# safe-autonomous-systems/fluidgym

Measured on AMD Instinct MI355X. Metric: env-steps/sec (batched) + pressure-Poisson HBM GB/s vs roofline, 1/2/4/8 GPUs, higher is better.
Workload: dtype f32; 1 GPU; ChannelJet2D-v0 (2D channel stand-in for 'cylinder Re=100 256x128'), 64 envs/GPU, 25 PISO steps/env step, random jets, stirred by a body force N(0,2.0) redrawn every env step; global_batch=64, parallelism=env-sharded x1, 1 bcast + 1 all_gather per step (RCCL), lanes_per_gpu=2, workload_modified=True, capped_solves=0, floor_released_solves=0, advection_solver_form=two-brick, velocity_solver=on-chip Jacobi sweeps (policy advection_jacobi; 11972 solves settled by

## Files before the change

### fluidgym_amd/_lib.py

```python
from __future__ import annotations

import ctypes
import os
from ctypes import POINTER, Structure, c_char_p, c_float, c_int, c_int32, c_int64, c_void_p

_HERE = os.path.dirname(os.path.abspath(__file__))
LIB_PATH = os.environ.get("FLUIDGYM_AMD_LIB") or os.path.join(_HERE, "libfluidgym_hip.so")
LIB_F64_PATH = os.environ.get("FLUIDGYM_AMD_LIB_F64") or os.path.join(_HERE, "libfluidgym_hip_f64.so")

FG_MAX_SCALARS = 4
FG_FIELD_SUMMARY_WORK_BYTES = 128
FG_OK = 0
FG_ERR_NOT_CONVERGED = -5
FG_ERR_NOT_FINITE = -6
FG_ERR_FLUX_BALANCE = -7
FG_PERIODIC, FG_FIXED = 0, 1
FG_DIRICHLET, FG_NEUMANN = 0, 1
FG_VELOCITY, FG_PRESSURE, FG_SCALAR, FG_VELOCITY_SOURCE, FG_VISCOSITY_FIELD = 0, 1, 2, 3, 4
FG_BOUND_VELOCITY, FG_BOUND_SCALAR = 8, 16
FG_SOLVER_CG, FG_SOLVER_JACOBI, FG_SOLVER_RBGS, FG_SOLVER_MGCG, FG_SOLVER_FDCG = 0, 1, 2, 3, 4
(FG_BUF_A, FG_BUF_C_OFF, FG_BUF_ADV_RHS, FG_BUF_VEL_RESULT, FG_BUF_H, FG_BUF_DIV, FG_BUF_P_RESULT,
 FG_BUF_SCALAR_RESULT) = range(8)
FG_ERR_UNSUPPORTED = -4
FG_ERR_INVALID_ARG = -1
# ... 79 lines not shown
        ("pressure_use_bicgstab", c_int32),
        ("pressure_warm_start", c_int32),
        ("pressure_project_mean", c_int32),
        ("pressure_stall_accept", c_float),
        ("solver_double_fallback", c_int32),
        ("bicg_precondition_fallback", c_int32),
    ]


class FgMbSimOptions(Structure):
    _fields_ = [
        ("step", FgMbStepOptions),
        ("time_step", c_float),
        ("cfl", c_float),
        ("adaptive", c_int32),
        ("substeps", c_int32),
        ("flux_balance_tol", c_float),
        ("outflow_slot0", c_int32),
        ("outflow_count", c_int32),
        ("outflow_velm", c_float * 3),
        ("outflow_tol", c_float),
        ("max_substeps", c_int32),
        ("outflow_slot0_b", c_int32),
        ("outflow_count_b", c_int32),
    ]


(FG_MB_BUF_A, FG_MB_BUF_C_OFF, FG_MB_BUF_RHS, FG_MB_BUF_H, FG_MB_BUF_DIV, FG_MB_BUF_P_DIAG, FG_MB_BUF_P_OFF,
 FG_MB_BUF_VELOCITY_RESULT) = range(8)
FG_MB_BUF_KRYLOV0 = 8


class FgSimOptions(Structure):
    _fields_ = [
        ("step", FgStepOptions),
        ("time_step", c_float),
        ("cfl", c_float),
        ("adaptive", c_int32),
        ("substeps", c_int32),
        ("flux_balance_tol", c_float),
        ("outflow_mask", c_int32),
        ("outflow_velm", c_float * 3),
        ("outflow_tol", c_float),
        ("max_substeps", c_int32),
    ]


SIGNATURES = {
    "fg_abi_version": (c_int, []),
    "fg_last_error": (c_char_p, []),
    "fg_create": (c_int, [POINTER(FgConfig), POINTER(c_float), POINTER(c_float), POINTER(c_float), POINTER(c_void_p)]),
    "fg_destroy": (c_int, [c_void_p]),
    "fg_bind": (c_int, [c_void_p, c_int, c_void_p]),
    "fg_set_viscosity": (c_int, [c_void_p, c_float]),
    "fg_set_scalar_viscosity": (c_int, [c_void_p, c_int, c_float]),
    "fg_set_viscosity_batch": (c_int, [c_void_p, c_void_p]),
    "fg_set_scalar_viscosity_batch": (c_int, [c_void_p, c_int, c_void_p]),
    "fg_set_fd_preconditioner": (c_int, [c_void_p] + [POINTER(c_float)] * 7),
    "fg_max_velocity": (c_int, [c_void_p, c_void_p, c_void_p]),
    "fg_set_fd_fast_transform": (c_int, [c_void_p, c_int, c_float]),
    "fg_set_return_best": (c_int, [c_void_p, c_int]),
    "fg_set_cg_reset_steps": (c_int, [c_void_p, c_int]),
    "fg_set_advection_start": (c_int, [c_void_p, c_int]),
    "fg_set_wall_stress_forcing": (c_int, [c_void_p, c_int, c_float, c_float]),
    "fg_boundary_flux_balance": (c_int, [c_void_p, c_void_p, c_void_p]),
    "fg_step_diagnostics": (c_int, [c_void_p, POINTER(c_float), c_void_p]),
    "fg_update_advective_boundary": (c_int, [c_void_p, c_int, POINTER(c_float), c_void_p, c_void_p]),
    "fg_balance_boundary_fluxes": (c_int, [c_void_p, c_int, c_float, c_void_p, c_void_p]),
    "fg_setup_advection": (c_int, [c_void_p, c_void_p, c_int, c_int, c_void_p]),
    "fg_solve_advection": (c_int, [c_void_p, c_int, c_int, c_float, c_int, POINTER(FgSolveInfo), c_void_p]),
    "fg_copy_scalar_result_to_blocks": (c_int, [c_void_p, c_int, c_void_p]),
    "fg_setup_pressure_matrix": (c_int, [c_void_p, c_void_p]),
    "fg_setup_pressure_rhs": (c_int, [c_void_p, c_void_p, c_void_p]),
    "fg_solve_pressure": (c_int, [c_void_p, c_int, c_float, c_int, c_int, POINTER(FgSolveInfo), c_void_p]),
    "fg_correct_velocity": (c_int, [c_void_p, c_void_p]),
    "fg_copy_velocity_result_to_blocks": (c_int, [c_void_p, c_void_p]),
    "fg_copy_velocity_result_from_blocks": (c_int, [c_void_p, c_void_p]),
    "fg_piso_step": (c_int, [c_void_p, c_void_p, POINTER(FgStepOptions), POINTER(c_int32), c_void_p]),
    "fg_single_step": (c_int, [c_void_p, POINTER(FgSimOptions), POINTER(c_int32), POINTER(c_float), c_void_p]),
    "fg_multi_step": (c_int, [c_void_p, POINTER(FgSimOptions), c_int32, POINTER(c_void_p), POINTER(c_int32), POINTER(c_float), POINTER(c_int32), c_void_p]),
    "fg_make_divergence_free": (c_int, [c_void_p, c_float, c_int, POINTER(FgSolveInfo), c_void_p]),
    "fg_reset_solver_state": (c_int, [c_void_p, c_void_p]),
    "fg_solver_hints": (c_int, [c_void_p, POINTER(c_int32), c_int32]),
    "fg_env_restore_field": (c_int, [c_void_p, c_int, c_void_p, c_int32, POINTER(FgEnvSel), c_int32, c_int32, c_void_p]),
    "fg_env_reset_solver_state": (c_int, [c_void_p, POINTER(FgEnvSel), c_int32, c_void_p]),
    "fg_mb_env_restore_field": (c_int, [c_void_p, c_int, c_void_p, c_int32, POINTER(FgEnvSel), c_int32, c_int32, c_void_p]),
    "fg_mb_env_reset_solver_state": (c_int, [c_void_p, POINTER(FgEnvSel), c_int32, c_void_p]),
    "fg_set_pressure_refinement": (c_int, [c_void_p, c_int32, c_float, c_float]),
    "fg_get_buffer": (c_int, [c_void_p, c_int, POINTER(c_void_p), POINTER(c_int64)]),
    "fg_read_buffer": (c_int, [c_void_p, c_int, c_void_p, c_void_p]),
    "fg_poisson_apply": (c_int, [c_void_p, c_void_p, c_void_p, c_void_p, c_void_p]),
    "fg_poisson_jacobi": (c_int, [c_void_p, c_void_p, c_void_p, c_void_p, c_int, c_float, c_void_p]),
    "fg_poisson_rbgs": (c_int, [c_void_p, c_void_p, c_void_p, c_void_p, c_int, c_float, c_void_p]),
    "fg_poisson_cg": (c_int, [c_void_p, c_void_p, c_void_p, c_void_p, c_float, c_int, c_int, POINTER(FgSolveInfo),
                              c_void_p]),
    "fg_poisson_fdcg": (c_int, [c_void_p, c_void_p, c_void_p, c_void_p, c_float, c_int, c_int, POINTER(FgSolveInfo),
                                c_void_p]),
    "fg_sparse_apply_ell": (c_int, [c_void_p, c_void_p, c_int32, c_int32, c_void_p, c_int64, c_int32, c_void_p, c_void_p]),
    "fg_sparse_apply_csr": (c_int, [c_void_p, c_void_p, c_void_p, c_int32, c_void_p, c_int64, c_int32, c_void_p, c_void_p]),
    "fg_stream_triad": (c_int, [c_void_p, c_void_p, c_void_p, c_float, c_int64, c_int32, POINTER(c_float), c_void_p]),
    "fg_mb_multilevel_status": (c_int, [c_void_p, POINTER(c_int32)]),
    "fg_mb_multilevel_apply": (c_int, [c_void_p, c_void_p, c_void_p, c_void_p]),
    "fg_mb_debug_ilu_apply": (c_int, [c_void_p, c_void_p, c_void_p, c_void_p]),
    "fg_mb_debug_pressure_cg": (c_int, [c_void_p, c_float, c_int32, c_int32, POINTER(c_int32), POINTER(c_int32), POINTER(ctypes.c_double), c_void_p]),
    "fg_mb_wall_forces": (c_int, [c_void_p, c_void_p, c_void_p, c_void_p, c_int32, c_int32, c_float, c_float, c_void_p, c_void_p]),
    "fg_mb_wall_forces_batch": (c_int, [c_void_p, c_void_p, c_void_p, c_void_p, c_int32, c_int32, c_float, c_float, c_void_p, c_void_p, c_void_p]),
    "fg_mb_debug_bicgstab": (c_int, [c_void_p, c_float, c_int32, c_int32, POINTER(c_int64), POINTER(ctypes.c_double), POINTER(c_float), c_void_p]),
    "fg_dacc_host_sum": (c_int, [POINTER(ctypes.c_double), c_int64, ctypes.c_double, POINTER(ctypes.c_double)]),
    "fg_dacc_device_sum": (c_int, [POINTER(ctypes.c_double), c_int64, ctypes.c_double, c_int32, POINTER(ctypes.c_double), c_void_p]),
    "fg_field_summary": (c_int, [c_void_p, c_int32, c_int32, c_int64, c_int32, c_void_p, c_void_p, c_void_p, ctypes.c_double, ctypes.c_double,
                                 c_int32, c_void_p, c_void_p]),
    "fg_plane_moments": (c_int, [POINTER(c_void_p), POINTER(c_int64), c_int32, c_int32, c_int32, c_int32, c_int32, c_int32, c_void_p, c_void_p,
                                 c_void_p, c_void_p, c_void_p]),
    "fg_plane_budgets": (c_int, [POINTER(c_void_p), POINTER(c_int64), c_int32, c_int32, c_int32, c_int32, c_int32, c_void_p, c_void_p, c_void_p,
                                 c_int32, c_int32, c_void_p, c_void_p, c_void_p, c_void_p, c_void_p]),
    "fg_plane_timecorr": (c_int, [POINTER(c_void_p), POINTER(c_int64), c_int32, c_int32, c_int32, c_int32, c_int32, c_int32, c_int32,
                                  POINTER(c_int32), c_void_p, c_void_p, c_void_p, c_void_p]),
    "fg_mb_cell_moments": (c_int, [c_void_p, c_void_p, c_int32, c_int32, c_int64, POINTER(c_int64), c_int32, c_int64, c_void_p, c_void_p,
                                   c_void_p]),
    "fg_mb_cell_moments_widths": (c_int, [c_void_p, c_void_p, c_int64, POINTER(c_int64), c_int32, c_void_p, c_void_p, POINTER(c_int32)]),
    "fg_plane_spectra": (c_int, [POINTER(c_void_p), POINTER(c_int64), c_int32, c_int32, c_int32, c_int32, c_int32, POINTER(c_int32), c_int32,
                                 c_void_p, c_void_p, c_void_p]),
    "fg_coherence_litmus": (c_int, [c_int32, c_int32, c_int32, c_int32, POINTER(c_int64), POINTER(ctypes.c_double), c_void_p]),
    "fg_profile_enable": (c_int, [c_void_p, c_int]),
    "fg_profile_kinds": (c_int, []),
    "fg_profile_kind_name": (ctypes.c_char_p, [c_int]),
    "fg_profile_read": (c_int, [c_void_p, c_int, POINTER(ctypes.c_double), POINTER(c_int64), POINTER(ctypes.c_double),
                                POINTER(ctypes.c_double), POINTER(ctypes.c_double), POINTER(ctypes.c_double),
                                POINTER(c_int64), POINTER(c_int64), POINTER(ctypes.c_double), POINTER(c_int64)]),
    "fg_coords_to_transforms": (c_int, [c_void_p, c_void_p, c_int, c_int, c_int, c_int, c_void_p]),
    "fg_resampler_create": (c_int, [c_int, POINTER(ctypes.c_int32), POINTER(ctypes.c_int32), POINTER(ctypes.c_int32),
                                    POINTER(ctypes.c_float), c_int, c_int, POINTER(c_void_p)]),
    "fg_resampler_destroy": (c_int, [c_void_p]),
    "fg_resample": (c_int, [c_void_p, c_void_p, c_int, c_int, c_void_p, c_int, c_void_p]),
    "fg_envglue_jet_schedule": (c_int, [c_void_p, c_void_p, c_void_p, c_void_p, c_int32, c_int32, c_int32, c_void_p, c_void_p, c_void_p]),
    "fg_envglue_channel_observe": (c_int, [c_void_p, c_void_p, c_void_p, c_int32, c_int32, c_int32, c_int32, c_float, c_float, c_void_p,
                                           c_void_p, c_void_p, c_void_p, c_void_p, c_void_p]),
    "fg_envglue_channel_observe_batch": (c_int, [c_void_p, c_void_p, c_void_p, c_int32, c_int32, c_int32, c_int32, c_void_p, c_float, c_void_p,
                                                 c_void_p, c_void_p, c_void_p, c_void_p, c_void_p]),
    "fg_mb_create": (c_int, [c_int32, c_int32, c_int32, POINTER(c_void_p)]),
    "fg_mb_destroy": (c_int, [c_void_p]),
    "fg_config_dump": (c_int, [c_void_p, ctypes.c_char_p, c_int]),
    "fg_mb_config_dump": (c_int, [c_void_p, ctypes.c_char_p, c_int]),
    "fg_mb_add_block": (c_int, [c_void_p, POINTER(c_float), c_int32, c_int32, c_int32, POINTER(c_int32)]),
    "fg_mb_connect": (c_int, [c_void_p, c_int32, c_int32, c_int32, c_int32, c_int32, c_int32]),
    "fg_mb_make_periodic": (c_int, [c_void_p, c_int32, c_int32]),
    "fg_mb_set_reference_quirks": (c_int, [c_void_p, c_int32, c_int32]),
    "fg_mb_set_nonortho_flags": (c_int, [c_void_p, c_int32]),
    "fg_mb_finalize": (c_int, [c_void_p]),
    "fg_mb_sizes": (c_int, [c_void_p, POINTER(c_int32), POINTER(c_int32)]),
    "fg_mb_block_info": (c_int, [c_void_p, c_int32, POINTER(c_int32), POINTER(c_int32)]),
    "fg_mb_get_host_table": (c_int, [c_void_p, c_int32, c_void_p, POINTER(c_int64)]),
    "fg_mb_get_neighbors": (c_int, [c_void_p, POINTER(c_int32)]),
    "fg_mb_bind": (c_int, [c_void_p, c_void_p, c_void_p, c_void_p, c_void_p]),
    "fg_mb_set_viscosity": (c_int, [c_void_p, c_float]),
    "fg_mb_set_viscosity_batch": (c_int, [c_void_p, c_void_p]),
    "fg_mb_piso_step": (c_int, [c_void_p, c_void_p, POINTER(FgMbStepOptions), POINTER(c_int32), c_void_p]),
    "fg_mb_max_velocity": (c_int, [c_void_p, POINTER(c_float), c_void_p]),
    "fg_mb_set_residual_projection": (c_int, [c_void_p, POINTER(c_float)]),
    "fg_mb_set_stall_limit": (c_int, [c_void_p, c_int32]),
    "fg_mb_set_advection_start": (c_int, [c_void_p, c_int]),
    "fg_mb_set_advection_jacobi": (c_int, [c_void_p, c_int]),
    "fg_mb_advection_jacobi_counts": (c_int, [c_void_p, POINTER(c_int64)]),
    "fg_mb_set_multilevel": (c_int, [c_void_p, c_int32, c_int32, POINTER(c_int32), POINTER(c_int32), POINTER(c_int32), POINTER(c_float),
                                     POINTER(c_float), c_float, c_int32]),
    "fg_mb_env_status": (c_int, [c_void_p, POINTER(c_int32)]),
# ... 133 lines not shown
```

### fluidgym_amd/csrc/fg_api.hip

```cpp
#include <stdio.h>
#include <string.h>

#include <cmath>
#include <string>
#include <vector>

#include <stdlib.h>

#include "fg_internal.h"

static thread_local std::string g_last_error;
void fg_set_error(const std::string& msg) { g_last_error = msg; }

extern "C" int fg_abi_version(void) { return FG_ABI_VERSION; }
extern "C" const char* fg_last_error(void) { return g_last_error.c_str(); }

static FgBounds make_bounds(const fg_state* s, int channel) {
    FgBounds b;
    for (int f = 0; f < 6; ++f) {
        b.vel[f] = s->bvel[f];
        b.scal[f] = s->bscal[f];
        b.scalar_bc[f] = s->cfg.scalar_bc[f][channel < 0 ? 0 : channel];
    }
    return b;
}

static int check_bound(const fg_state* s, bool need_scalar) {
    FG_REQUIRE(s->velocity && s->pressure, FG_ERR_NOT_BOUND, "velocity/pressure not bound (fg_bind)");
    for (int f = 0; f < 2 * s->grid.dims; ++f) {
        if (!s->grid.fixed[f]) continue;
        FG_REQUIRE(s->bvel[f], FG_ERR_NOT_BOUND, "boundary velocity of a FIXED face not bound");
        if (need_scalar) FG_REQUIRE(s->bscal[f], FG_ERR_NOT_BOUND, "boundary scalar of a FIXED face not bound");
    }
    if (need_scalar) FG_REQUIRE(s->scalar, FG_ERR_NOT_BOUND, "passive scalar not bound");
    return FG_OK;
}

extern "C" int fg_create(const fg_config* cfg, const fg_real* hx, const fg_real* hy, const fg_real* hz, fg_handle* out) {
    FG_REQUIRE(cfg && out && hx && hy, FG_ERR_INVALID_ARG, "fg_create: null argument");
    FG_REQUIRE(cfg->dims == 2 || cfg->dims == 3, FG_ERR_INVALID_ARG, "dims must be 2 or 3");
    FG_REQUIRE(cfg->dims == 2 || hz, FG_ERR_INVALID_ARG, "hz required in 3-D");
    FG_REQUIRE(cfg->nx >= 3 && cfg->ny >= 3 && (cfg->dims == 2 ? cfg->nz == 1 : cfg->nz >= 3), FG_ERR_INVALID_ARG,
               "block needs >= 3 cells per axis (nz = 1 in 2-D)");
    FG_REQUIRE(cfg->batch >= 1, FG_ERR_INVALID_ARG, "batch must be >= 1");
    FG_REQUIRE(cfg->n_scalars >= 0 && cfg->n_scalars <= FG_MAX_SCALARS, FG_ERR_INVALID_ARG, "bad n_scalars");
    for (int a = 0; a < cfg->dims; ++a)
        FG_REQUIRE(cfg->face_type[2 * a] == cfg->face_type[2 * a + 1], FG_ERR_INVALID_ARG,
                   "a FIXED face needs a FIXED partner (CloseBoundary closes both, domain_structs.cpp:1981-2002)");
    FG_REQUIRE((long long)cfg->nx * cfg->ny * cfg->nz * cfg->batch * 6 < (1LL << 31), FG_ERR_UNSUPPORTED,
               "index space exceeds int32 (reference index_t is int32 as well)");
    FG_HIP_CHECK(hipSetDevice(cfg->device));

    fg_state* s = new fg_state();
    memset(s, 0, sizeof(*s));
    s->cfg = *cfg;
    FgGrid& g = s->grid;
    g.dims = cfg->dims; g.nx = cfg->nx; g.ny = cfg->ny; g.nz = cfg->nz;
    g.n = cfg->nx * cfg->ny * cfg->nz; g.B = cfg->batch;
    for (int f = 0; f < 6; ++f) g.fixed[f] = (f < 2 * cfg->dims) ? (cfg->face_type[f] == FG_FIXED) : 0;
    s->vec = (!FG_F64 && cfg->nx % 4 == 0) ? 4 : 1;
    s->viscosity = 0.f;

    const fg_real* hsrc[3] = {hx, hy, hz};
    const int hn[3] = {cfg->nx, cfg->ny, cfg->nz};
    for (int a = 0; a < 3; ++a) {
        std::vector<fg_real> h(hn[a], 1.f), rh(hn[a], 1.f);
        if (a < cfg->dims)
            for (int i = 0; i < hn[a]; ++i) {
                if (!(hsrc[a][i] > 0.f)) { delete s; fg_set_error("cell widths must be positive"); return FG_ERR_INVALID_ARG; }
                h[i] = hsrc[a][i]; rh[i] = 1.f / hsrc[a][i];
            }
        FG_HIP_CHECK(hipMalloc(&s->d_h[a], sizeof(fg_real) * hn[a]));
        FG_HIP_CHECK(hipMalloc(&s->d_rh[a], sizeof(fg_real) * hn[a]));
        FG_HIP_CHECK(hipMemcpy(s->d_h[a], h.data(), sizeof(fg_real) * hn[a], hipMemcpyHostToDevice));
        FG_HIP_CHECK(hipMemcpy(s->d_rh[a], rh.data(), sizeof(fg_real) * hn[a], hipMemcpyHostToDevice));
        g.h[a] = s->d_h[a]; g.rh[a] = s->d_rh[a];
    }
    const size_t BN = (size_t)g.B * g.n, d = g.dims;
    auto alloc = [&](fg_real** p, size_t count) -> hipError_t {
        hipError_t e = hipMalloc(p, sizeof(fg_real) * count);
        if (e == hipSuccess) e = hipMemset(*p, 0, sizeof(fg_real) * count);
        return e;
    };
    FG_HIP_CHECK(alloc(&s->A, BN));
    FG_HIP_CHECK(alloc(&s->rA, BN));
    FG_HIP_CHECK(alloc(&s->Coff, BN * 2 * d));
    FG_HIP_CHECK(alloc(&s->adv_rhs, BN * d));
    FG_HIP_CHECK(alloc(&s->vel_result, BN * d));
    FG_HIP_CHECK(alloc(&s->hvec, BN * d));
    FG_HIP_CHECK(alloc(&s->div, BN));
    FG_HIP_CHECK(alloc(&s->p_result, BN));
    FG_HIP_CHECK(alloc(&s->scal_result, BN));
    for (int i = 0; i < 8; ++i) FG_HIP_CHECK(alloc(&s->w[i], BN * d));
    const size_t nsys = (size_t)g.B * d;
    FG_HIP_CHECK(hipMalloc(&s->acc, sizeof(FgDacc) * nsys * FG_ACC_DOUBLES));
    FG_HIP_CHECK(hipMemset(s->acc, 0, sizeof(FgDacc) * nsys * FG_ACC_DOUBLES));
    FG_HIP_CHECK(hipMalloc(&s->flags, sizeof(int32_t) * nsys));
    FG_HIP_CHECK(hipMalloc(&s->info_dev, sizeof(fg_solve_info) * nsys));
    FG_HIP_CHECK(hipHostMalloc(&s->info_pinned, sizeof(fg_solve_info) * nsys));
    FG_HIP_CHECK(hipHostMalloc(&s->flags_pinned, sizeof(int32_t) * nsys));
    FG_HIP_CHECK(alloc(&s->scratch_B, (size_t)g.B * (4 + 2 * d)));
    FG_HIP_CHECK(hipMalloc(&s->d_bvel_ptrs, sizeof(fg_real*) * 6));
    FG_HIP_CHECK(hipMemset(s->d_bvel_ptrs, 0, sizeof(fg_real*) * 6));
    FG_HIP_CHECK(hipHostMalloc(&s->diag_pinned, sizeof(fg_real) * 2 * g.B));
    FG_HIP_CHECK(hipHostMalloc(&s->dt_pinned, sizeof(fg_real) * g.B));
    FG_HIP_CHECK(alloc(&s->dt_dev, g.B));
    FG_HIP_CHECK(hipMalloc(&s->env_sel_dev, sizeof(fg_env_sel) * g.B));
    s->t_rem_dev = nullptr;
#if !FG_F64
    FG_HIP_CHECK(hipMalloc(&s->t_rem_dev, sizeof(double) * g.B));
    FG_HIP_CHECK(hipMemset(s->t_rem_dev, 0, sizeof(double) * g.B));
#endif
    if (int rc = fg_poll_create(&s->poll, (int)(nsys > 2 * (size_t)g.B ? nsys : 2 * (size_t)g.B))) return rc;
    for (int k = 0; k < 4; ++k) { s->pred_bicg[k] = 2; s->pred_cg[k] = 1; }
    s->wall_forcing_axis = -1;
    s->ref64_inner = 1e-4f;
    s->cg_wgs_per_slot = 256;
    { const char* ev = getenv("FG_BICG3"); s->bicg3_force = ev ? atoi(ev) : -1; }
    { const char* ev = getenv("FG_BICG3_BXL"); s->bicg3_bxl = ev ? atoi(ev) : 0; }
    { const char* ev = getenv("FG_BICG_SUB"); s->bicg_sub = ev ? atoi(ev) : -1; }
    { const char* ev = getenv("FG_REDUCE_WGS"); s->reduce_wgs = ev ? atoi(ev) : 0; }
    { const char* ev = getenv("FG_BICG3_MIX"); s->bicg3_mix = ev ? atoi(ev) : 3; }
    { const char* ev = getenv("FG_BICG_FUSED"); s->bicg_fused = ev ? atoi(ev) : 1; }
    s->tridiag_cb = 64;
    s->helm_cb_pref = 32;
    { const char* ev = getenv("FG_HELM_ROWFORM"); s->helm_rowform_off = (ev && atoi(ev) == 0) ? 1 : 0; }
    { const char* ev = getenv("FG_FD_FACFUSE"); s->fd_facfuse = ev ? atoi(ev) : 1; }
    { const char* ev = getenv("FG_DEV_DT"); s->dev_dt = ev ? atoi(ev) : 1; }
    { const char* ev = getenv("FG_ADV_LINESWEEP"); s->adv_linesweep = ev ? atoi(ev) : 0; }
    { const char* ev = getenv("FG_FD_ROWMEAN"); s->fd_rowmean = ev ? atoi(ev) : 1; }
    s->fd_row_epoch = -1; s->rA_epoch = 0; s->fd_row_part_epoch = -1;
    { const char* ev = getenv("FG_CG_FUSED"); s->cg_fused = ev ? atoi(ev) : 1; }
    { const char* ev = getenv("FG_BICG_PFUSED"); s->bicg_pfused = ev ? atoi(ev) : 1; }
    { const char* ev = getenv("FG_ADV_JACOBI"); s->adv_jacobi = ev ? atoi(ev) : 0; s->adv_jacobi_env = ev ? 1 : 0; }
    for (int k = 0; k < 4; ++k) s->jac_hist[k] = FgJacHist{0, 0, 0};
    s->jac_solves = s->jac_fallbacks = 0;
    FG_HIP_CHECK(hipHostMalloc(&s->jac_prev, sizeof(float) * 4 * nsys));
    s->jac_rA_epoch = -1;
    FG_HIP_CHECK(hipMalloc(&s->fcg_alpha, sizeof(double) * 2 * (size_t)g.B));
    FG_HIP_CHECK(hipMemset(s->fcg_alpha, 0, sizeof(double) * 2 * (size_t)g.B));
    FG_HIP_CHECK(hipMalloc(&s->fcg_xsum, sizeof(FgDacc) * 2 * (size_t)g.B));
    FG_HIP_CHECK(hipMemset(s->fcg_xsum, 0, sizeof(FgDacc) * 2 * (size_t)g.B));
    FG_HIP_CHECK(hipMalloc(&s->fcg_lazy, sizeof(int32_t) * (size_t)g.B));
    FG_HIP_CHECK(hipMemset(s->fcg_lazy, 0, sizeof(int32_t) * (size_t)g.B));
    { const char* e = getenv("FG_FCG_FIRST"); s->fcg_first = (e && atoi(e) == 0) ? 0 : 1; }
    { const char* e = getenv("FG_JAC_SPEC"); s->jac_spec = (e && atoi(e) == 0) ? 0 : 1; }
    { const char* e = getenv("FG_FCG_SPEC"); s->fcg_spec = (e && atoi(e) == 0) ? 0 : 1; }
    { const char* e = getenv("FG_JAC_PREFACTOR"); s->jac_prefactor = (e && atoi(e) == 0) ? 0 : 1; }
    { const char* e = getenv("FG_JAC_WARM"); s->jac_warm = e ? (atoi(e) != 0 ? 1 : 0) : -1; }
    s->cg_return_best = 1;
    s->cg_reset_steps = 100;
    s->adv_from_result = 1;
    FG_HIP_CHECK(hipMalloc(&s->cg_acc, sizeof(FgDacc) * (size_t)g.B * 8 * 64));
    FG_HIP_CHECK(hipMemset(s->cg_acc, 0, sizeof(FgDacc) * (size_t)g.B * 8 * 64));
    FG_HIP_CHECK(hipMalloc(&s->cg_best.best_crit, sizeof(fg_real) * g.B));
    FG_HIP_CHECK(hipMalloc(&s->cg_best.saved_crit, sizeof(fg_real) * g.B));
    FG_HIP_CHECK(hipMalloc(&s->cg_best.save_at, sizeof(int32_t) * g.B));
    FG_HIP_CHECK(alloc(&s->cg_best.best_x, BN));
    *out = s;
    return FG_OK;
}

extern "C" int fg_destroy(fg_handle s) {
    if (!s) return FG_OK;
    for (int a = 0; a < 3; ++a) { (void)hipFree(s->d_h[a]); (void)hipFree(s->d_rh[a]); }
    fg_real* owned[] = {s->A, s->rA, s->Coff, s->adv_rhs, s->vel_result, s->hvec, s->div, s->p_result, s->scal_result,
                      s->scratch_B};
    for (fg_real* p : owned) (void)hipFree(p);
    for (int i = 0; i < 8; ++i) (void)hipFree(s->w[i]);
    (void)hipFree(s->acc); (void)hipFree(s->flags); (void)hipFree(s->info_dev);
    (void)hipHostFree(s->info_pinned); (void)hipHostFree(s->flags_pinned);
    fg_prof_destroy(s);
    fg_poll_destroy(&s->poll);
    (void)hipFree(s->d_bvel_ptrs); (void)hipHostFree(s->diag_pinned); (void)hipHostFree(s->dt_pinned); (void)hipFree(s->dt_dev); (void)hipFree(s->t_rem_dev); (void)hipFree(s->env_sel_dev);
    float* fd[] = {s->fd_Qx, s->fd_QxT, s->fd_Qz, s->fd_QzT, s->fd_lower, s->fd_inv, s->fd_cp};
    for (float* p : fd) if (p) (void)hipFree(p);
    if (s->fd_dct_tw) { (void)hipFree(s->fd_dct_tw); (void)hipFree(s->fd_dct_rot); }
    (void)hipFree(s->cg_acc); (void)hipFree(s->fcg_alpha); (void)hipFree(s->fcg_xsum); (void)hipFree(s->fcg_lazy);
    if (s->jac_prev) (void)hipHostFree(s->jac_prev);
    (void)hipFree(s->fd_row_part); (void)hipFree(s->fd_lam_x); (void)hipFree(s->fd_row_inv); (void)hipFree(s->fd_row_cp); (void)hipFree(s->fd_row_lower);
    (void)hipFree(s->line_inv); (void)hipFree(s->line_cp); (void)hipFree(s->ilu_d);
    (void)hipFree(s->r64_buf); (void)hipFree(s->r64_acc); (void)hipFree(s->ref64_x); (void)hipFree(s->force_uniform);
    (void)hipFree(s->fd_lam); (void)hipFree(s->helm_diag); (void)hipFree(s->helm_lower); (void)hipFree(s->helm_upper); (void)hipFree(s->helm_tmp); (void)hipFree(s->helm_lower_row); (void)hipFree(s->helm_lower_row2); (void)hipFree(s->line_inv2); (void)hipFree(s->line_cp2);
    (void)hipFree(s->cg_best.best_crit); (void)hipFree(s->cg_best.saved_crit); (void)hipFree(s->cg_best.save_at); (void)hipFree(s->cg_best.best_x);
    delete s;
    return FG_OK;
}

static int sync_bvel_ptrs(fg_state* s);
extern "C" int fg_bind(fg_handle s, int field, fg_real* ptr) {
    FG_REQUIRE(s, FG_ERR_INVALID_ARG, "null handle");
    if (field == FG_VELOCITY) s->velocity = ptr;
    else if (field == FG_PRESSURE) s->pressure = ptr;
    else if (field == FG_SCALAR) s->scalar = ptr;
    else if (field == FG_VELOCITY_SOURCE) s->velocity_source = ptr;
    else if (field == FG_VISCOSITY_FIELD) s->visc_field = ptr;
    else if (field >= FG_BOUND_VELOCITY && field < FG_BOUND_VELOCITY + 6) {
        s->bvel[field - FG_BOUND_VELOCITY] = ptr;
        return sync_bvel_ptrs(s);
    }
    else if (field >= FG_BOUND_SCALAR && field < FG_BOUND_SCALAR + 6) s->bscal[field - FG_BOUND_SCALAR] = ptr;
    else FG_REQUIRE(false, FG_ERR_INVALID_ARG, "fg_bind: unknown field id");
    return FG_OK;
}

extern "C" int fg_set_viscosity(fg_handle s, fg_real v) {
    FG_REQUIRE(s, FG_ERR_INVALID_ARG, "null handle");
    s->viscosity = v;
    return FG_OK;
}
extern "C" int fg_set_scalar_viscosity(fg_handle s, int ch, fg_real v) {
    FG_REQUIRE(s && ch >= 0 && ch < FG_MAX_SCALARS, FG_ERR_INVALID_ARG, "bad channel");
    s->scalar_viscosity[ch] = v;
    s->scalar_viscosity_set = true;
    return FG_OK;
}
extern "C" int fg_set_viscosity_batch(fg_handle s, const fg_real* nu_B) {
    FG_REQUIRE(s, FG_ERR_INVALID_ARG, "null handle");
    s->viscosity_B = nu_B;
    s->helm_pre_mask = 0;
    return FG_OK;
}
extern "C" int fg_set_scalar_viscosity_batch(fg_handle s, int ch, const fg_real* k_B) {
    FG_REQUIRE(s && ch >= 0 && ch < FG_MAX_SCALARS, FG_ERR_INVALID_ARG, "bad channel");
    s->scalar_viscosity_B[ch] = k_B;
    s->helm_pre_mask = 0;
    return FG_OK;
}

extern "C" int fg_set_fd_preconditioner(fg_handle s, const float* Qx, const float* QxT, const float* Qz, const float* QzT,
// ... 267 lines not shown
    if (for_scalar) {
        a.scal = s->scalar + (size_t)channel * s->grid.n;
        a.scal_env_stride = (long)s->cfg.n_scalars * s->grid.n;
        a.nu = fg_nu(s, 1, channel);
    } else {
        a.source = s->velocity_source;
        if (s->wall_forcing_axis >= 0)
            if (int rc = fg_launch_wall_forcing(s, (hipStream_t)stream)) return rc;
        a.force = s->wall_forcing_axis >= 0 ? s->force_uniform : nullptr;
        a.visc = s->visc_field;
        a.nu = fg_nu(s);
        a.rA = s->rA;
        s->adv_last_dt = dt_B;
        s->rA_epoch++;
        s->jac_rA_epoch = s->rA_epoch;
#if !FG_F64
        if (fg_fd_rowmean_ok(s) && s->vec == 4 && (s->grid.nx & 63) == 0) {
            if (!s->fd_row_part) FG_HIP_CHECK(hipMalloc(&s->fd_row_part, sizeof(float) * (size_t)s->grid.B * s->grid.ny * (s->grid.nx / 64)));
            a.row_part = s->fd_row_part;
            s->fd_row_part_epoch = s->rA_epoch;
        }
#endif
        if (buoy_axis >= 0) {
            a.buoy_T = s->scalar; a.buoy_stride = (long)s->cfg.n_scalars * s->grid.n; a.buoy_axis = buoy_axis; a.buoy_factor = buoy_factor;
            a.source_w = s->velocity_source;
        }
    }
    return fg_launch_adv_build(s, make_bounds(s, channel), a, (hipStream_t)stream);
}

static int advection_solve(fg_state* s, FgBicgArgs a, fg_solve_info* info, hipStream_t st, int for_scalar = 0, int channel = 0, bool* spec_ran = nullptr);

extern "C" int fg_solve_advection(fg_handle s, int for_scalar, int channel, fg_real tol, int max_iterations,
                                  fg_solve_info* info_host, void* stream) {
    FG_REQUIRE(s, FG_ERR_INVALID_ARG, "null handle");
    FgBicgArgs a;
    a.diag = s->A; a.off = s->Coff; a.rhs = s->adv_rhs;
    a.dt = s->cur_dt;
    a.tol = tol; a.max_iterations = max_iterations;
    if (for_scalar) { a.x = s->scal_result; a.nc = 1; a.use_x0 = 0; a.kind = 0; }
    else { a.x = s->vel_result; a.nc = s->grid.dims; a.use_x0 = s->adv_from_result; }
    return advection_solve(s, a, info_host, (hipStream_t)stream, for_scalar, channel);
}

extern "C" int fg_copy_scalar_result_to_blocks(fg_handle s, int channel, void* stream) {
    FG_REQUIRE(s && s->scalar, FG_ERR_NOT_BOUND, "scalar not bound");
    const int n = s->grid.n;
    if (s->cfg.n_scalars == 1) return fg_launch_copy_active(s, s->cur_dt, s->scal_result, s->scalar, 1, (hipStream_t)stream);
    FG_HIP_CHECK(hipMemcpy2DAsync(s->scalar + (size_t)channel * n, sizeof(fg_real) * n * s->cfg.n_scalars, s->scal_result,
                                  sizeof(fg_real) * n, sizeof(fg_real) * n, s->grid.B, hipMemcpyDeviceToDevice,
                                  (hipStream_t)stream));
    return FG_OK;
}

extern "C" int fg_setup_pressure_matrix(fg_handle s, void* stream) {
    FG_REQUIRE(s, FG_ERR_INVALID_ARG, "null handle");
    s->rA_epoch++;
    return fg_launch_pressure_setup(s, s->cur_dt, (hipStream_t)stream);
}

extern "C" int fg_setup_pressure_rhs(fg_handle s, const fg_real* dt_B, void* stream) {
    FG_REQUIRE(s && dt_B, FG_ERR_INVALID_ARG, "null argument");
    if (int rc = check_bound(s, false)) return rc;
    hipStream_t st = (hipStream_t)stream;
    if (int rc = fg_launch_h(s, dt_B, s->vel_result, st)) return rc;
    return fg_launch_div(s, make_bounds(s, 0), dt_B, s->hvec, s->div, st);
}

struct SpecH { fg_state* s; const fg_real* dt; const fg_step_options* opt; hipStream_t st; };
static int spec_h(void* p) {
    const SpecH* c = static_cast<const SpecH*>(p);
    fg_state* s = c->s;
    if (int rc = fg_launch_h(s, c->dt, s->vel_result, c->st)) return rc;
    return fg_launch_div(s, make_bounds(s, 0), c->dt, s->hvec, s->div, c->st, !c->opt->pressure_warm_start,
                         c->opt->pressure_method == FG_SOLVER_FDCG && s->fd_Qx != nullptr);
}

static int launch_corrector(fg_state* s, const fg_real* dt, const FgCgOutcome& o, bool last, hipStream_t st) {
    const bool mean_folded = last && o.mean_ready;
    FG_REQUIRE(!o.lazy_z || !last || mean_folded, FG_ERR_UNSUPPORTED, "fg_piso_step: an unmaterialised pressure without its folded mean");
    if (last && !mean_folded)
        if (int rc = fg_launch_mean_sub(s, dt, s->p_result, s->pressure, st)) return rc;
    const FgMeanRef mean = {s->fcg_xsum, s->info_dev, s->pressure, o.marks_valid ? s->fcg_lazy : nullptr, s->fcg_alpha};
    const FgLazyRef lazy = {s->fcg_lazy, s->fcg_alpha, last ? s->p_result : nullptr};
    const fg_real* p = o.lazy_z ? o.lazy_z : ((last && !mean_folded) ? s->pressure : s->p_result);
    return fg_launch_correct(s, dt, s->rA, s->hvec, p, s->vel_result, st, last ? s->velocity : nullptr, mean_folded ? &mean : nullptr, o.lazy_z ? &lazy : nullptr);
}

struct SpecCorrect { fg_state* s; const fg_real* dt; bool last; hipStream_t st; };
static int spec_correct(void* p, const FgCgOutcome& o) {
    const SpecCorrect* c = static_cast<const SpecCorrect*>(p);
    return launch_corrector(c->s, c->dt, o, c->last, c->st);
}

static int solve_pressure(fg_state* s, const fg_real* dt, int method, fg_real tol, int max_iterations, int use_previous,
                          fg_solve_info* info_host, hipStream_t st, bool finalize = true, int kind = 2, FgCgOutcome* out = nullptr,
                          FgCgSpec spec = FgCgSpec{}) {
    int rc = FG_OK;
    FgCgOutcome own;
    if (!out) out = &own;
    if (method == FG_SOLVER_CG || method == FG_SOLVER_FDCG) {
        FgCgArgs a;
        a.rA = s->rA; a.b = s->div; a.x = s->p_result;
        a.r = s->w[0]; a.p = s->w[1]; a.Ap = s->w[2];
        a.dt = dt; a.tol = tol; a.max_iterations = max_iterations; a.use_x0 = use_previous;
        a.reset_steps = s->cg_reset_steps;
        a.precond = (method == FG_SOLVER_FDCG);
        a.kind = kind;
        a.check_every = a.precond ? 2 : 16;
        a.lazy_ok = finalize ? 0 : 1;
        a.spec = spec;
#if !FG_F64
        if (s->ref64_outer > 0) a.lazy_ok = 0;
#endif
        rc = fg_cg_solve(s, a, info_host, st, out);
#if !FG_F64
        if (s->ref64_outer > 0 && (rc == FG_OK || rc == FG_ERR_NOT_CONVERGED)) rc = fg_refine64_pressure(s, a, info_host, st, out);
        if (s->double_fallback && (rc == FG_ERR_NOT_FINITE || (s->ladder_force & 2))) {
            std::vector<fg_solve_info> tmp;
            fg_solve_info* info = info_host;
            if (!info) { tmp.assign(s->info_pinned, s->info_pinned + s->grid.B); info = tmp.data(); }
            s->rung_count[2] += 1;
            rc = fg_rung64_cg(s, a, info, (s->ladder_force & 2) != 0, st, out);
        }
#endif
    } else {
        fg_set_error("fg_solve_pressure: only FG_SOLVER_CG drives the PISO step (Jacobi/RBGS are smoothers)");
        return FG_ERR_UNSUPPORTED;
    }
    if (rc != FG_OK && rc != FG_ERR_NOT_CONVERGED) return rc;
    if (finalize)
        if (int rc2 = fg_launch_mean_sub(s, dt, s->p_result, s->pressure, st)) return rc2;
    return rc;
}

extern "C" int fg_solve_pressure(fg_handle s, int method, fg_real tol, int max_iterations, int use_previous,
                                 fg_solve_info* info_host, void* stream) {
    FG_REQUIRE(s, FG_ERR_INVALID_ARG, "null handle");
    if (int rc = check_bound(s, false)) return rc;
    return solve_pressure(s, s->cur_dt, method, tol, max_iterations, use_previous, info_host, (hipStream_t)stream);
}

extern "C" int fg_set_pressure_refinement(fg_handle s, int32_t max_corrections, fg_real target_tol, fg_real inner_relative_tol) {
    FG_REQUIRE(s, FG_ERR_INVALID_ARG, "null handle");
    FG_REQUIRE(!FG_F64 || max_corrections <= 0, FG_ERR_UNSUPPORTED, "fg_set_pressure_refinement: the fp64 build solves in fp64 already");
    FG_REQUIRE(max_corrections <= 0 || (target_tol > 0 && inner_relative_tol > 0 && inner_relative_tol < 1), FG_ERR_INVALID_ARG,
               "fg_set_pressure_refinement: tolerances must be positive, the relative one below 1");
    s->ref64_outer = max_corrections > 0 ? max_corrections : 0;
    s->ref64_tol = (float)target_tol; s->ref64_inner = (float)inner_relative_tol;
    return FG_OK;
}

extern "C" int fg_correct_velocity(fg_handle s, void* stream) {
    FG_REQUIRE(s, FG_ERR_INVALID_ARG, "null handle");
    if (int rc = check_bound(s, false)) return rc;
    return fg_launch_correct(s, s->cur_dt, s->rA, s->hvec, s->pressure, s->vel_result, (hipStream_t)stream);
}

extern "C" int fg_copy_velocity_result_to_blocks(fg_handle s, void* stream) {
    FG_REQUIRE(s && s->velocity, FG_ERR_NOT_BOUND, "velocity not bound");
    return fg_launch_copy_active(s, s->cur_dt, s->vel_result, s->velocity, s->grid.dims, (hipStream_t)stream);
}
extern "C" int fg_copy_velocity_result_from_blocks(fg_handle s, void* stream) {
    FG_REQUIRE(s && s->velocity, FG_ERR_NOT_BOUND, "velocity not bound");
    return fg_launch_copy_active(s, nullptr, s->velocity, s->vel_result, s->grid.dims, (hipStream_t)stream);
}

static int max_iters(const fg_solve_info* info, int n) {
    int m = -1;
    for (int i = 0; i < n; ++i) m = info[i].used_iterations > m ? info[i].used_iterations : m;
    return m;
}

static int advection_solve(fg_state* s, FgBicgArgs a, fg_solve_info* info, hipStream_t st, int for_scalar, int channel, bool* spec_ran) {
    a.precond = (s->adv_precond == 1) ? 1 : (s->adv_precond == 3 ? 2 : (s->adv_precond == 4 ? 3 : 0));
    if (a.precond == 2 && !for_scalar && s->visc_field) a.precond = 0;
    if (a.precond == 2) {
        a.nu = fg_nu(s, for_scalar, channel);
        a.wall_lo = for_scalar ? (s->cfg.scalar_bc[2][channel] == FG_DIRICHLET) : 1;
        a.wall_hi = for_scalar ? (s->cfg.scalar_bc[3][channel] == FG_DIRICHLET) : 1;
    }
    const int nsys = s->grid.B * a.nc;
    std::vector<fg_solve_info> info_own;
    if (!info) { info_own.resize(nsys); info = info_own.data(); }
    int rc = fg_bicgstab_solve(s, a, info, st, spec_ran);
    bool failed = (rc == FG_ERR_NOT_CONVERGED || rc == FG_ERR_NOT_FINITE) || (s->ladder_force & 1);
#if !FG_F64
    if (failed && s->double_fallback && rc != FG_ERR_HIP) {
        s->rung_count[0] += 1;
        rc = fg_rung64_bicgstab(s, a, info, (s->ladder_force & 1) != 0, st);
        if (rc != FG_OK && rc != FG_ERR_NOT_CONVERGED && rc != FG_ERR_NOT_FINITE) return rc;
        failed = (rc != FG_OK) || (s->ladder_force & 4);
    }
#endif
    if (failed && (s->adv_precond == 2 || s->adv_precond == 5)) {
        s->line_retries += 1;
        s->rung_count[1] += 1;
        a.precond = s->adv_precond == 5 ? 3 : 1; a.use_x0 = 0;
        rc = fg_bicgstab_solve(s, a, info, st);
    }
    (void)nsys;
    return rc;
}

extern "C" int fg_piso_step(fg_handle s, const fg_real* dt_B, const fg_step_options* opt, int32_t* stats_host,
                            void* stream) {
    FG_REQUIRE(s && dt_B && opt, FG_ERR_INVALID_ARG, "null argument");
    const bool scalar = opt->advect_scalar && s->cfg.n_scalars > 0;
    if (int rc = check_bound(s, scalar)) return rc;
    FG_REQUIRE(opt->buoyancy_axis < s->grid.dims, FG_ERR_INVALID_ARG, "bad buoyancy axis");
    FG_REQUIRE(opt->buoyancy_axis < 0 || (s->velocity_source && s->scalar), FG_ERR_NOT_BOUND,
               "buoyancy needs velocity source and scalar bound");
    hipStream_t st = (hipStream_t)stream;
    const int B = s->grid.B, d = s->grid.dims;
    std::vector<fg_solve_info> info((size_t)B * d);
    int32_t stats[4] = {-1, -1, -1, -1};
    struct DropHelmRecord { fg_state* s; ~DropHelmRecord() { s->helm_pre_mask = 0; } } drop_helm_record{s};
    int status = FG_OK;
    auto soft = [&](int rc) {
        if (rc == FG_ERR_NOT_CONVERGED) { status = rc; return FG_OK; }
        return rc;
    };
#if !FG_F64
    const bool sweeps_first = s->adv_linesweep && s->grid.dims == 2 && s->jac_hist[0].skip == 0 && s->jac_hist[1].skip == 0;
    if (scalar && s->cfg.n_scalars == 1 && s->adv_precond == 3 && s->fd_lam && !s->visc_field && !sweeps_first) {
        const FgNu nu2[2] = {fg_nu(s, 1, 0), fg_nu(s)};
        const int wlo[2] = {s->cfg.scalar_bc[2][0] == FG_DIRICHLET, 1}, whi[2] = {s->cfg.scalar_bc[3][0] == FG_DIRICHLET, 1};
        if (int rc = fg_helm_factor_pair(s, dt_B, nu2, wlo, whi, st)) return rc;
    }
#endif
    if (scalar) {
        FgRange range_scalar("scalar_advection");
        for (int ch = 0; ch < s->cfg.n_scalars; ++ch) {
            if (int rc = fg_setup_advection(s, dt_B, 1, ch, stream)) return rc;
            FgBicgArgs a;
            a.diag = s->A; a.off = s->Coff; a.rhs = s->adv_rhs; a.x = s->scal_result; a.nc = 1;
            a.dt = dt_B; a.tol = opt->advection_tol; a.max_iterations = opt->max_iterations; a.use_x0 = 0; a.kind = 0;
            if (int rc = soft(advection_solve(s, a, info.data(), st, 1, ch))) return rc;
            const int m = max_iters(info.data(), B);
            stats[0] = m > stats[0] ? m : stats[0];
            s->ctr.add(0, info.data(), B);
            const int n = s->grid.n;
            if (s->cfg.n_scalars == 1) {
                if (int rc = fg_launch_copy_active(s, dt_B, s->scal_result, s->scalar, 1, st)) return rc;
            } else {
                (void)n;
                fg_set_error("multi-channel scalar copy with inactive envs not implemented");
                return FG_ERR_UNSUPPORTED;
            }
        }
    }
    fg_range_push("velocity_assembly_and_solve");
    struct PopOnce { bool armed = true; void fire() { if (armed) { fg_range_pop(); armed = false; } } ~PopOnce() { fire(); } } range_velocity;
    if (int rc = setup_advection(s, dt_B, 0, 0, stream, opt->buoyancy_axis, opt->buoyancy_factor)) return rc;
    bool h_div_ran = false;
    {
        FgBicgArgs a;
        a.diag = s->A; a.off = s->Coff; a.rhs = s->adv_rhs; a.x = s->vel_result; a.nc = d;
        a.dt = dt_B; a.tol = opt->advection_tol; a.max_iterations = opt->max_iterations; a.use_x0 = s->adv_from_result;
        SpecH spec_h_ctx = {s, dt_B, opt, st};
        if (opt->corrector_steps > 0) a.spec = FgSpecHook{spec_h, &spec_h_ctx};
        if (int rc = soft(advection_solve(s, a, info.data(), st, 0, 0, &h_div_ran))) return rc;
        stats[1] = max_iters(info.data(), B * d);
        s->ctr.add(1, info.data(), B * d);
    }
    range_velocity.fire();
    for (int c = 0; c < opt->corrector_steps; ++c) {
        FgRange range_corr(c == 0 ? "pressure_corrector_0" : "pressure_corrector_1+");
        const bool last = (c + 1 == opt->corrector_steps);
        if (!(c == 0 && h_div_ran)) {
            if (int rc = fg_launch_h(s, dt_B, s->vel_result, st)) return rc;
            if (int rc = fg_launch_div(s, make_bounds(s, 0), dt_B, s->hvec, s->div, st, !opt->pressure_warm_start,
                                       opt->pressure_method == FG_SOLVER_FDCG && s->fd_Qx != nullptr))
                return rc;
        }
        SpecCorrect spec_ctx = {s, dt_B, last, st};
        FgCgOutcome outcome;
        if (int rc = soft(solve_pressure(s, dt_B, opt->pressure_method, opt->pressure_tol, opt->max_iterations, opt->pressure_warm_start ? 1 : 0,
                                         info.data(), st, false, c == 0 ? 0 : 1, &outcome, FgCgSpec{spec_correct, &spec_ctx})))
            return rc;
        if (c < 2) { stats[2 + c] = max_iters(info.data(), B); s->ctr.add(2 + c, info.data(), B); }
        if (!outcome.spec_done)
            if (int rc = launch_corrector(s, dt_B, outcome, last, st)) return rc;
    }
    if (opt->corrector_steps <= 0)
        if (int rc = fg_launch_copy_active(s, dt_B, s->vel_result, s->velocity, d, st)) return rc;
    if (stats_host) memcpy(stats_host, stats, sizeof(stats));
    s->ctr.piso_steps += 1;
    return status;
}

extern "C" int fg_config_dump(fg_handle s, char* buf, int n) {
    FG_REQUIRE(s && buf && n > 0, FG_ERR_INVALID_ARG, "fg_config_dump: bad argument");
    char tmp[3072];
    const int len = snprintf(tmp, sizeof(tmp),
        "{\"build\": \"%s\", \"FG_CG_FUSED\": %d, \"FG_BICG_PFUSED\": %d, \"FG_BICG_FUSED\": %d, \"FG_BICG_SUB\": %d, \"FG_BICG3\": %d, "
        "\"FG_BICG3_BXL\": %d, \"FG_BICG3_MIX\": %d, \"FG_REDUCE_WGS\": %d, \"FG_CG_WGS_PER_SLOT\": %d, \"FG_TRIDIAG_CB\": %d, \"FG_HELM_CB\": %d, "
        "\"FG_HELM_ROWFORM\": %d, \"FG_FD_ROWMEAN\": %d, \"FG_POLL_SPIN\": %d, \"FG_PROF_PERIOD\": %d, \"fast_transform_x\": %d, \"fd_preconditioner\": %d, "
        "\"helmholtz\": %d, \"advection_preconditioner\": %d, \"advection_from_result\": %d, \"return_best\": %d, \"cg_reset_steps\": %d, "
        "\"double_fallback\": %d, \"wall_forcing_axis\": %d, \"FG_ADV_JACOBI\": %d, \"FG_FCG_FIRST\": %d, \"FG_JAC_WARM\": %d, \"first_iterate_polls\": %ld, \"unstored_pressure_solves\": %ld, \"FG_JAC_SPEC\": %d, \"FG_FCG_SPEC\": %d, \"jacobi_speculation_misses\": %ld, \"jacobi_floor_released\": %ld, \"pressure_refinement_corrections\": %ld}",
        FG_F64 ? "f64" : "f32", s->cg_fused, s->bicg_pfused, s->bicg_fused, s->bicg_sub, s->bicg3_force, s->bicg3_bxl, s->bicg3_mix, s->reduce_wgs,
        s->cg_wgs_per_slot, s->tridiag_cb, s->helm_cb_pref, s->helm_rowform_off ? 0 : 1, s->fd_rowmean, s->poll.spin, s->prof.period, s->fd_dct_x, s->fd_Qx ? 1 : 0,
        s->fd_lam ? 1 : 0, s->adv_precond, s->adv_from_result, s->cg_return_best, s->cg_reset_steps, s->double_fallback, s->wall_forcing_axis, s->adv_jacobi, s->fcg_first, s->jac_warm,
        s->fcg_first_polls, s->fcg_unstored, s->jac_spec, s->fcg_spec, s->jac_spec_missed, s->jac_floor_released, s->ref64_corrections);
    if (len >= n) return len + 1;
    memcpy(buf, tmp, (size_t)len + 1);
    return FG_OK;
}

extern "C" int fg_solver_unconverged(fg_handle s, int64_t* out4) {
    FG_REQUIRE(s != nullptr && out4 != nullptr, FG_ERR_INVALID_ARG, "fg_solver_unconverged: bad argument");
    for (int k = 0; k < 4; ++k) out4[k] = s->ctr.unconv[k];
    return FG_OK;
}

extern "C" int fg_solver_counters(fg_handle s, int64_t* out13, int32_t reset) {
    FG_REQUIRE(s != nullptr, FG_ERR_INVALID_ARG, "fg_solver_counters: null handle");
    if (out13) s->ctr.write(out13);
    if (reset) s->ctr.reset();
    return FG_OK;
}

extern "C" int fg_single_step(fg_handle s, const fg_sim_options* o, int32_t* out, fg_real* flux_host, void* stream);
extern "C" int fg_multi_step(fg_handle s, const fg_sim_options* o, int32_t n, const fg_real* const* bvel_schedule, int32_t* out_6n,
                             fg_real* flux_host, int32_t* steps_done, void* stream) {
    FG_REQUIRE(s && o && out_6n && n >= 0, FG_ERR_INVALID_ARG, "fg_multi_step: bad argument");
    if (steps_done) *steps_done = 0;
    for (int k = 0; k < n; ++k) {
        if (bvel_schedule)
            for (int f = 0; f < 2 * s->grid.dims; ++f)
                if (const fg_real* p = bvel_schedule[(size_t)k * 6 + f])
                    if (int rc = fg_bind(s, FG_BOUND_VELOCITY + f, const_cast<fg_real*>(p))) return rc;
        if (int rc = fg_single_step(s, o, out_6n + 6 * (size_t)k, flux_host, stream)) return rc;
        if (steps_done) *steps_done = k + 1;
        if (out_6n[6 * (size_t)k + 5] == 0 && !s->cg_return_best) break;
    }
    return FG_OK;
}

static inline bool is_close_zero(double a) { return std::fabs(a) <= 1e-8; }

extern "C" int fg_single_step(fg_handle s, const fg_sim_options* o, int32_t* out, fg_real* flux_host, void* stream) {
    fg_htrace("single_step_in");
    FgRange range_sim("fg_single_step");
    FG_REQUIRE(s && o && out, FG_ERR_INVALID_ARG, "null argument");
    if (int rc = check_bound(s, o->step.advect_scalar && s->cfg.n_scalars > 0)) return rc;
    hipStream_t st = (hipStream_t)stream;
    const int B = s->grid.B;
    const FgBounds bnd = make_bounds(s, 0);
    std::vector<double> t_rem(B, (double)o->time_step);
    int32_t stats[4] = {-1, -1, -1, -1};
    int substeps = 0, all_ok = 1;
    bool first = true;
    int fixed_left = o->adaptive ? 0 : (o->substeps > 0 ? o->substeps : 1);
    for (;;) {
        bool any = false;
        if (o->adaptive) {
            for (int b = 0; b < B; ++b) any = any || (t_rem[b] > 0 && !is_close_zero(t_rem[b]));
        } else {
            any = fixed_left > 0;
        }
        if (!any) break;
        auto advance = [&](int b, fg_real max_vel) -> fg_real {
            fg_real ts = 0.f;
            if (!o->adaptive) {
                ts = o->time_step;
            } else if (t_rem[b] > 0 && !is_close_zero(t_rem[b])) {
                const double mv = (double)max_vel;
                const double max_ts = is_close_zero(mv) ? t_rem[b] : (double)o->cfl / mv;
                double tsd;
                if (max_ts >= t_rem[b]) tsd = t_rem[b];
                else tsd = t_rem[b] / (double)(long long)std::ceil(t_rem[b] / max_ts);
                t_rem[b] -= tsd;
                ts = (fg_real)tsd;
            }
            return ts;
        };
        auto flux_guard = [&]() -> int {
            fg_real worst = 0.f;
            for (int b = 0; b < B; ++b) {
                if (flux_host) flux_host[b] = s->diag_pinned[b];
                const fg_real a = std::fabs(s->diag_pinned[b]);
                worst = (a > worst || a != a) ? a : worst;
            }
            if (!(worst <= o->flux_balance_tol)) {
                fg_set_error("Domain boundary fluxes not balanced, cannot proceed with simulation step.");
                return FG_ERR_FLUX_BALANCE;
// ... 11 lines not shown
                const FgDtRule rule = deferred ? FgDtRule{s->t_rem_dev, s->dt_dev, (float)o->cfl, (double)o->time_step, first ? 1 : 0}
                                               : FgDtRule{nullptr, nullptr, 0.f, 0.0, 0};
                if (int rc = fg_launch_max_velocity(s, bnd, s->scratch_B + B, st, s->diag_pinned + B, po.seq ? FgPollOut{po.seq + B, po.value, po.gran} : po,
                                                    first ? s->scratch_B : nullptr, first ? s->diag_pinned : nullptr, rule))
                    return rc;
            }
            fg_htrace("maxvel_launched");
            if (!deferred) {
                if (o->adaptive && po.gran) {
                    if (int rc = fg_poll_wait_words(&s->poll, po, 12 * B, first ? 2 * B : B, st)) return rc;
                    for (int b = 0; b < B; ++b) {
                        s->diag_pinned[B + b] = fg_poll_word_float(&s->poll, 12 * B + b);
                        if (first) s->diag_pinned[b] = fg_poll_word_float(&s->poll, 13 * B + b);
                    }
                } else if (int rc = fg_poll_wait(&s->poll, po, o->adaptive ? B : 0, o->adaptive ? 1 : B, st)) return rc;
                fg_htrace("maxvel_poll_done");
                if (first) if (int rc = flux_guard()) return rc;
            }
        }
        if (!deferred)
            for (int b = 0; b < B; ++b) s->dt_pinned[b] = advance(b, o->adaptive ? s->diag_pinned[B + b] : (fg_real)0);
        const bool folded = o->outflow_mask && fg_outflow_folds(s, o->outflow_mask);
        const bool dt_by_value = folded && B <= 64 && !deferred;
        if (!dt_by_value && !deferred) FG_HIP_CHECK(hipMemcpyAsync(s->dt_dev, s->dt_pinned, sizeof(fg_real) * B, hipMemcpyHostToDevice, st));
        if (o->outflow_mask) {
            for (int f = 0; f < 2 * s->grid.dims; ++f)
                if ((o->outflow_mask >> f) & 1) FG_REQUIRE(s->grid.fixed[f], FG_ERR_INVALID_ARG, "outflow face is not FIXED");
            if (!folded)
                for (int f = 0; f < 2 * s->grid.dims; ++f)
                    if ((o->outflow_mask >> f) & 1)
                        if (int rc = fg_launch_outflow(s, f, o->outflow_velm[f >> 1], s->dt_dev, st)) return rc;
            fg_real velm3[3] = {o->outflow_velm[0], o->outflow_velm[1], o->outflow_velm[2]};
            if (int rc = fg_launch_balance(s, bnd, o->outflow_mask, (fg_real)0.01 * o->outflow_tol, s->dt_dev, st, folded ? o->outflow_mask : 0, velm3,
                                           dt_by_value ? s->dt_pinned : nullptr))
                return rc;
        }
        int rc = fg_piso_step(s, s->dt_dev, &o->step, stats, stream);
        if (rc == FG_ERR_NOT_CONVERGED) all_ok = 0;
        else if (rc != FG_OK) return rc;
        if (deferred) {
            if (int rc2 = fg_poll_wait_words(&s->poll, po_cfl, 12 * B, first ? 2 * B : B, st)) return rc2;
            for (int b = 0; b < B; ++b) {
                s->diag_pinned[B + b] = fg_poll_word_float(&s->poll, 12 * B + b);
                if (first) s->diag_pinned[b] = fg_poll_word_float(&s->poll, 13 * B + b);
            }
            if (first) if (int rc2 = flux_guard()) return rc2;
            for (int b = 0; b < B; ++b) s->dt_pinned[b] = advance(b, s->diag_pinned[B + b]);
        }
        ++substeps;
        first = false;
        if (!o->adaptive) --fixed_left;
        if (substeps >= (o->max_substeps > 0 ? o->max_substeps : 100000)) break;
    }
    fg_htrace("single_step_out");
    for (int i = 0; i < 4; ++i) out[i] = stats[i];
    out[4] = substeps;
    out[5] = all_ok;
    return FG_OK;
}

extern "C" int fg_make_divergence_free(fg_handle s, fg_real tol, int max_iterations, fg_solve_info* info_host,
                                       void* stream) {
    FG_REQUIRE(s, FG_ERR_INVALID_ARG, "null handle");
    if (int rc = check_bound(s, false)) return rc;
    s->cur_dt = nullptr;
    hipStream_t st = (hipStream_t)stream;
    const size_t BN = (size_t)s->grid.B * s->grid.n;
    std::vector<fg_real> ones(BN, 1.f);
    FG_HIP_CHECK(hipMemcpyAsync(s->rA, ones.data(), sizeof(fg_real) * BN, hipMemcpyHostToDevice, st));
    s->rA_epoch++;
    FG_HIP_CHECK(hipStreamSynchronize(st));
    if (int rc = fg_launch_copy_active(s, nullptr, s->velocity, s->hvec, s->grid.dims, st)) return rc;
    if (int rc = fg_launch_div(s, make_bounds(s, 0), nullptr, s->hvec, s->div, st)) return rc;
    int rc = solve_pressure(s, nullptr, FG_SOLVER_CG, tol, max_iterations, 0, info_host, st);
    if (rc != FG_OK && rc != FG_ERR_NOT_CONVERGED) return rc;
    if (int rc2 = fg_launch_correct(s, nullptr, s->rA, s->hvec, s->pressure, s->vel_result, st)) return rc2;
    if (int rc2 = fg_launch_copy_active(s, nullptr, s->vel_result, s->velocity, s->grid.dims, st)) return rc2;
    return rc;
}

extern "C" int fg_reset_solver_state(fg_handle s, void* stream) {
    FG_REQUIRE(s && s->velocity, FG_ERR_NOT_BOUND, "velocity not bound");
    for (int k = 0; k < 4; ++k) s->jac_hist[k] = FgJacHist{0, 0, 0};
    FG_HIP_CHECK(hipMemsetAsync(s->p_result, 0, sizeof(fg_real) * (size_t)s->grid.B * s->grid.n, (hipStream_t)stream));
    return fg_launch_copy_active(s, nullptr, s->velocity, s->vel_result, s->grid.dims, (hipStream_t)stream);
}

extern "C" int fg_solver_hints(fg_handle s, int32_t* hints12, int32_t set) {
    FG_REQUIRE(s != nullptr && hints12 != nullptr, FG_ERR_INVALID_ARG, "fg_solver_hints: bad argument");
    for (int k = 0; k < 4; ++k) {
        FgJacHist& H = s->jac_hist[k];
        if (set) { H.sweeps = hints12[3 * k]; H.skip = hints12[3 * k + 1]; H.fails = hints12[3 * k + 2]; }
        else { hints12[3 * k] = H.sweeps; hints12[3 * k + 1] = H.skip; hints12[3 * k + 2] = H.fails; }
    }
    return FG_OK;
}

extern "C" int fg_get_buffer(fg_handle s, int which, fg_real** out_ptr, int64_t* out_count) {
    FG_REQUIRE(s && out_ptr && out_count, FG_ERR_INVALID_ARG, "null argument");
    const int64_t BN = (int64_t)s->grid.B * s->grid.n, d = s->grid.dims;
    switch (which) {
        case FG_BUF_A: *out_ptr = s->A; *out_count = BN; break;
        case FG_BUF_C_OFF: *out_ptr = s->Coff; *out_count = BN * 2 * d; break;
        case FG_BUF_ADV_RHS: *out_ptr = s->adv_rhs; *out_count = BN * d; break;
        case FG_BUF_VEL_RESULT: *out_ptr = s->vel_result; *out_count = BN * d; break;
        case FG_BUF_H: *out_ptr = s->hvec; *out_count = BN * d; break;
        case FG_BUF_DIV: *out_ptr = s->div; *out_count = BN; break;
        case FG_BUF_P_RESULT: *out_ptr = s->p_result; *out_count = BN; break;
        case FG_BUF_SCALAR_RESULT: *out_ptr = s->scal_result; *out_count = BN; break;
        default:
            if (which >= 100 && which < 108) { *out_ptr = s->w[which - 100]; *out_count = BN * d; break; }
            FG_REQUIRE(false, FG_ERR_INVALID_ARG, "unknown buffer id");
    }
    return FG_OK;
}

extern "C" int fg_read_buffer(fg_handle s, int which, fg_real* dst, void* stream) {
    fg_real* src = nullptr;
    int64_t count = 0;
    if (int rc = fg_get_buffer(s, which, &src, &count)) return rc;
    FG_REQUIRE(dst, FG_ERR_INVALID_ARG, "null destination");
    FG_HIP_CHECK(hipMemcpyAsync(dst, src, sizeof(fg_real) * count, hipMemcpyDeviceToDevice, (hipStream_t)stream));
    return FG_OK;
}

extern "C" int fg_poisson_apply(fg_handle s, const fg_real* rA, const fg_real* x, fg_real* y, void* stream) {
    FG_REQUIRE(s && rA && x && y, FG_ERR_INVALID_ARG, "null argument");
    return fg_poisson_apply_launch(s, rA, x, y, (hipStream_t)stream);
}

extern "C" int fg_poisson_jacobi(fg_handle s, const fg_real* rA, const fg_real* b, fg_real* x, int n_sweeps, fg_real omega,
                                 void* stream) {
    FG_REQUIRE(s && rA && b && x && n_sweeps >= 0, FG_ERR_INVALID_ARG, "bad argument");
    hipStream_t st = (hipStream_t)stream;
    fg_real* buf[2] = {x, s->w[5]};
    for (int i = 0; i < n_sweeps; ++i)
        if (int rc = fg_poisson_jacobi_launch(s, rA, b, buf[i & 1], buf[(i + 1) & 1], omega, st)) return rc;
    if (n_sweeps & 1)
        FG_HIP_CHECK(hipMemcpyAsync(x, s->w[5], sizeof(fg_real) * (size_t)s->grid.B * s->grid.n, hipMemcpyDeviceToDevice, st));
    return FG_OK;
}

extern "C" int fg_poisson_rbgs(fg_handle s, const fg_real* rA, const fg_real* b, fg_real* x, int n_sweeps, fg_real omega,
                               void* stream) {
    FG_REQUIRE(s && rA && b && x && n_sweeps >= 0, FG_ERR_INVALID_ARG, "bad argument");
    hipStream_t st = (hipStream_t)stream;
    for (int i = 0; i < n_sweeps; ++i) {
        if (int rc = fg_poisson_rbgs_launch(s, rA, b, x, omega, 0, st)) return rc;
        if (int rc = fg_poisson_rbgs_launch(s, rA, b, x, omega, 1, st)) return rc;
    }
    return FG_OK;
}

extern "C" int fg_poisson_cg(fg_handle s, const fg_real* rA, const fg_real* b, fg_real* x, fg_real tol, int max_iterations,
                             int use_x0, fg_solve_info* info_host, void* stream) {
    FG_REQUIRE(s && rA && b && x, FG_ERR_INVALID_ARG, "null argument");
    FgCgArgs a;
    a.rA = rA; a.b = b; a.x = x;
    a.r = s->w[0]; a.p = s->w[1]; a.Ap = s->w[2];
    a.dt = nullptr; a.tol = tol; a.max_iterations = max_iterations; a.use_x0 = use_x0;
    a.reset_steps = 100;
    a.precond = 0;
    a.check_every = (tol > 0.f) ? 16 : (1 << 30);
    return fg_cg_solve(s, a, info_host, (hipStream_t)stream);
}

// ... 24 lines not shown
```

### fluidgym_amd/csrc/fg_fftcg.h

```cpp
#pragma once
#include "fg_internal.h"
#include "fg_cg.h"

constexpr int FCG_DELTA = 3, FCG_GAMMA = 5;

struct FcgVectors {
    fg_real* z; fg_real* w;
    fg_real* p; fg_real* s;
    fg_real* x; fg_real* r; fg_real* t1;
};

struct FcgUpdArgs {
    const float* z; const float* w; float* p; float* s; float* x; float* r; float* t1;
    const float2* tw; const float2* rot; float fs0, fs;
    const int32_t* flags; FgDacc* acc; double* alpha; FgDacc* xsum; FgBest best;
    int ns, rows, it, first; long env_stride;
    const float* r0; int x_zero;
    const int32_t* lazy;
};
struct FcgInvArgs {
    const float* u; const float* r; const float* rA; float* z; float* w;
    const float2* tw; const float2* rot; float is0, is;
    const int32_t* flags; FgDacc* acc; int ns, rows, it; long env_stride;
    const float* hy; const float* rhy; const float* hx; const float* rhx; int fixed_x;
    FgDacc* xsum; int extras;
};

struct FcgDivArgs {
    const float* h; float* div; float* r; float* x; float* t1;
    const float* bvel[4];
    const float2* tw; const float2* rot; float fs0, fs;
    const float* dt; FgDacc* acc; int ns, rows; long n;
    const float* hx; const float* hy; int fixed_x;
};

#if !FG_F64
int fg_fcg_div_fwd(fg_state* s, const FgBounds& bnd, const fg_real* dt, const fg_real* hvec, fg_real* div, int ns, hipStream_t st);
bool fg_fcg_ok(const fg_state* s);
int fg_fcg_update_fwd(fg_state* s, const FcgVectors& v, int it, int first, int ns, hipStream_t st, bool marks_valid, const fg_real* r0 = nullptr);
int fg_fcg_inv_apply(fg_state* s, const FcgVectors& v, const fg_real* rA, int it, int ns, hipStream_t st, int extras = 0);
int fg_fcg_check0(fg_state* s, fg_real tol, int ns, hipStream_t st, FgPollOut poll, bool* marks_valid);
#endif
```

### fluidgym_amd/csrc/fg_fftcg.hip

```cpp
#include "fg_internal.h"
#include "fg_cg.h"
#include "fg_fftrow.h"
#include "fg_fftcg.h"

#if !FG_F64
namespace {

using fgfft::Map;

template <int N, bool PERIODIC>
__global__ __launch_bounds__(256) void k_fcg_update_fwd(FcgUpdArgs a) {
    constexpr int EPL = N / 64;
    __shared__ __attribute__((aligned(16))) float2 buf[2][4][N];
    __shared__ __attribute__((aligned(16))) float2 twl[N];
    __shared__ float red[8];
    const int b = blockIdx.y;
    const int lane = threadIdx.x & 63, wave = threadIdx.x >> 6;
    if (a.flags[b] != 0) {
        if (a.lazy && a.lazy[b] == 1) {
            const float alpha = (float)a.alpha[b * 2];
            const int row0 = 2 * (blockIdx.x * 4 + wave);
#pragma unroll
            for (int half = 0; half < 2; ++half) {
                const int row = row0 + half;
                if (row >= a.rows) continue;
                const size_t o = (size_t)b * a.env_stride + (size_t)row * N;
                float zv[EPL], xv[EPL];
                fgfft::load_row<N>(a.z + o, lane, zv);
                if (a.x_zero) {
#pragma unroll
                    for (int e = 0; e < EPL; ++e) xv[e] = 0.f;
                } else {
                    fgfft::load_row<N>(a.x + o, lane, xv);
                }
#pragma unroll
                for (int e = 0; e < EPL; ++e) xv[e] += alpha * zv[e];
                fgfft::store_row<N>(a.x + o, lane, xv);
            }
        } else if (a.x_zero && (a.flags[b] == 1 || a.flags[b] == 2)) {
            float z0[EPL];
#pragma unroll
            for (int e = 0; e < EPL; ++e) z0[e] = 0.f;
            const int r0 = 2 * (blockIdx.x * 4 + wave);
            if (r0 < a.rows) fgfft::store_row<N>(a.x + (size_t)b * a.env_stride + (size_t)r0 * N, lane, z0);
            if (r0 + 1 < a.rows) fgfft::store_row<N>(a.x + (size_t)b * a.env_stride + (size_t)(r0 + 1) * N, lane, z0);
        }
        return;
    }
    for (int k = threadIdx.x; k < N; k += 256) twl[k] = a.tw[k];
    const int it = a.it;
    const double g_new = fg_acc_total(fg_acc_ptr(a.acc, b, FCG_GAMMA + it % 3), a.ns);
    const double d_new = fg_acc_total(fg_acc_ptr(a.acc, b, FCG_DELTA + (it & 1)), a.ns);
    double beta = 0.0, denom = d_new;
    if (!a.first) {
        const double g_old = fg_acc_total(fg_acc_ptr(a.acc, b, FCG_GAMMA + (it + 2) % 3), a.ns);
        const double al_old = a.alpha[b * 2 + ((it + 1) & 1)];
        beta = g_new / g_old;
        denom = d_new - beta * g_new / al_old;
    }
    const double alpha_d = g_new / denom;
    const float alpha = (float)alpha_d, betaf = (float)beta;
    const bool save = a.best.save_at[b] == it;
    if (blockIdx.x == 0 && threadIdx.x < 64) {
        fg_acc_zero(fg_acc_ptr(a.acc, b, FCG_GAMMA + (it + 1) % 3), a.ns);
        fg_acc_zero(fg_acc_ptr(a.acc, b, FCG_DELTA + ((it + 1) & 1)), a.ns);
        if (threadIdx.x == 0) {
            a.alpha[b * 2 + (it & 1)] = alpha_d;
            acc_st(a.xsum + (b * 2 + ((it + 1) & 1)), 0.0);
        }
    }
    const int row0 = 2 * (blockIdx.x * 4 + wave), row1 = row0 + 1;
    const bool live0 = row0 < a.rows, live1 = row1 < a.rows;
    const size_t o0 = (size_t)b * a.env_stride + (size_t)(live0 ? row0 : 0) * N;
    const size_t o1 = (size_t)b * a.env_stride + (size_t)(live1 ? row1 : 0) * N;
    float pa[EPL], pb[EPL], sa[EPL], sb[EPL], xa[EPL], xb[EPL], ra[EPL], rb[EPL];
    {
        float za[EPL], zb[EPL], wa[EPL], wb[EPL];
        fgfft::load_row<N>(a.z + o0, lane, za); fgfft::load_row<N>(a.z + o1, lane, zb);
        fgfft::load_row<N>(a.w + o0, lane, wa); fgfft::load_row<N>(a.w + o1, lane, wb);
        if (!a.first) {
            fgfft::load_row<N>(a.p + o0, lane, pa); fgfft::load_row<N>(a.p + o1, lane, pb);
            fgfft::load_row<N>(a.s + o0, lane, sa); fgfft::load_row<N>(a.s + o1, lane, sb);
        }
        if (a.x_zero) {
#pragma unroll
            for (int e = 0; e < EPL; ++e) { xa[e] = 0.f; xb[e] = 0.f; }
        } else {
            fgfft::load_row<N>(a.x + o0, lane, xa); fgfft::load_row<N>(a.x + o1, lane, xb);
        }
        const float* rsrc = a.r0 ? a.r0 : a.r;
        fgfft::load_row<N>(rsrc + o0, lane, ra); fgfft::load_row<N>(rsrc + o1, lane, rb);
        if (save) {
            if (live0) fgfft::store_row<N>(a.best.best_x + o0, lane, xa);
            if (live1) fgfft::store_row<N>(a.best.best_x + o1, lane, xb);
        }
        if (a.first) {
#pragma unroll
            for (int e = 0; e < EPL; ++e) { pa[e] = za[e]; pb[e] = zb[e]; sa[e] = wa[e]; sb[e] = wb[e]; }
        } else {
#pragma unroll
            for (int e = 0; e < EPL; ++e) {
                pa[e] = za[e] + betaf * pa[e]; pb[e] = zb[e] + betaf * pb[e];
                sa[e] = wa[e] + betaf * sa[e]; sb[e] = wb[e] + betaf * sb[e];
            }
        }
    }
    float part[2] = {0.f, 0.f};
#pragma unroll
    for (int e = 0; e < EPL; ++e) {
        xa[e] += alpha * pa[e]; ra[e] -= alpha * sa[e];
        xb[e] += alpha * pb[e]; rb[e] -= alpha * sb[e];
        if (!live0) { xa[e] = 0.f; ra[e] = 0.f; }
        if (!live1) { xb[e] = 0.f; rb[e] = 0.f; }
        part[0] += ra[e] * ra[e] + rb[e] * rb[e];
        part[1] += xa[e] + xb[e];
    }
    if (live0) {
        if (!a.first) { fgfft::store_row<N>(a.p + o0, lane, pa); fgfft::store_row<N>(a.s + o0, lane, sa); }
        fgfft::store_row<N>(a.x + o0, lane, xa); fgfft::store_row<N>(a.r + o0, lane, ra);
    }
    if (live1) {
        if (!a.first) { fgfft::store_row<N>(a.p + o1, lane, pb); fgfft::store_row<N>(a.s + o1, lane, sb); }
// ... 229 lines not shown
            if (at_lo) fgfft::ldv<VW>(a.bvel[2] + ((size_t)b * 2 + 1) * N + i0, bl);
            if (at_hi) fgfft::ldv<VW>(a.bvel[3] + ((size_t)b * 2 + 1) * N + i0, bh);
            const float hl = sr[(i0 == 0) ? N - 1 : i0 - 1], hr = sr[(i0 + VW == N) ? 0 : i0 + VW];
            const bool xlo = (i0 == 0) && a.fixed_x, xhi = (i0 + VW == N) && a.fixed_x;
#pragma unroll
            for (int e = 0; e < VW; ++e) {
                const float h_l = (e == 0) ? hl : hc[e > 0 ? e - 1 : 0], h_r = (e == VW - 1) ? hr : hc[e < VW - 1 ? e + 1 : VW - 1];
                float acc = 0.f;
                {
                    const float area = hy;
                    const float F_hi = (e == VW - 1 && xhi) ? a.bvel[1][((size_t)b * 2 + 0) * a.rows + jc] * area : 0.5f * (hc[e] + h_r) * area;
                    const float F_lo = (e == 0 && xlo) ? a.bvel[0][((size_t)b * 2 + 0) * a.rows + jc] * area : 0.5f * (hc[e] + h_l) * area;
                    acc += F_hi - F_lo;
                }
                {
                    const float area = hx[e];
                    const float F_hi = at_hi ? bh[e] * area : 0.5f * (v1[e] + vd[e]) * area;
                    const float F_lo = at_lo ? bl[e] * area : 0.5f * (v1[e] + vu[e]) * area;
                    acc += F_hi - F_lo;
                }
                out[q * VW + e] = live ? acc : 0.f;
            }
        }
        if (live) {
#pragma unroll
            for (int e = 0; e < EPL; ++e) part[0] += out[e] * out[e];
            const size_t o = (size_t)b * a.n + (size_t)j * N;
            fgfft::store_row<N>(a.div + o, lane, half ? db : da);
        }
    }
    __syncthreads();
    float oa[EPL], ob[EPL];
    fgfft::forward_rows<N, PERIODIC>(da, db, oa, ob, buf[0][wave], buf[1][wave], twl, a.rot, fgfft::Scales{a.fs0, a.fs}, lane);
    if (row0 < a.rows) fgfft::store_row<N>(a.t1 + (size_t)b * a.n + (size_t)row0 * N, lane, oa);
    if (row0 + 1 < a.rows) fgfft::store_row<N>(a.t1 + (size_t)b * a.n + (size_t)(row0 + 1) * N, lane, ob);
    fg_block_sum<1>(part, red);
    if (threadIdx.x == 0) fg_acc_add(fg_acc_ptr(a.acc, b, 0), a.ns, blockIdx.x, (double)part[0]);
}

template <bool PERIODIC>
int launch_upd(const fg_state* s, int slot, int n, const FcgUpdArgs& a, dim3 grid, hipStream_t st) {
    switch (n) {
        case 64: FG_LAUNCH_P(s, slot, (k_fcg_update_fwd<64, PERIODIC>), grid, dim3(256), 0, st, a); break;
        case 128: FG_LAUNCH_P(s, slot, (k_fcg_update_fwd<128, PERIODIC>), grid, dim3(256), 0, st, a); break;
        case 256: FG_LAUNCH_P(s, slot, (k_fcg_update_fwd<256, PERIODIC>), grid, dim3(256), 0, st, a); break;
        case 512: FG_LAUNCH_P(s, slot, (k_fcg_update_fwd<512, PERIODIC>), grid, dim3(256), 0, st, a); break;
        default: fg_set_error("fused CG: unsupported row length"); return FG_ERR_UNSUPPORTED;
    }
    return FG_OK;
}
template <bool PERIODIC>
int launch_inv(const fg_state* s, int slot, int n, const FcgInvArgs& a, dim3 grid, hipStream_t st) {
    switch (n) {
        case 64: FG_LAUNCH_P(s, slot, (k_fcg_inv_apply<64, PERIODIC>), grid, dim3(320), 0, st, a); break;
        case 128: FG_LAUNCH_P(s, slot, (k_fcg_inv_apply<128, PERIODIC>), grid, dim3(320), 0, st, a); break;
        case 256: FG_LAUNCH_P(s, slot, (k_fcg_inv_apply<256, PERIODIC>), grid, dim3(320), 0, st, a); break;
        case 512: FG_LAUNCH_P(s, slot, (k_fcg_inv_apply<512, PERIODIC>), grid, dim3(320), 0, st, a); break;
        default: fg_set_error("fused CG: unsupported row length"); return FG_ERR_UNSUPPORTED;
    }
    return FG_OK;
}

template <bool PERIODIC>
int launch_div(const fg_state* s, int n, const FcgDivArgs& a, dim3 grid, hipStream_t st) {
    const int slot = fg_prof_slot(s, FG_PK_DIV, nullptr, s->grid.B, 28.0 * (double)s->grid.n, (8.0 + 5.0 * log2((double)n)) * (double)s->grid.n, st);
    switch (n) {
        case 64: FG_LAUNCH_P(s, slot, (k_fcg_div_fwd<64, PERIODIC>), grid, dim3(256), 0, st, a); break;
        case 128: FG_LAUNCH_P(s, slot, (k_fcg_div_fwd<128, PERIODIC>), grid, dim3(256), 0, st, a); break;
        case 256: FG_LAUNCH_P(s, slot, (k_fcg_div_fwd<256, PERIODIC>), grid, dim3(256), 0, st, a); break;
        case 512: FG_LAUNCH_P(s, slot, (k_fcg_div_fwd<512, PERIODIC>), grid, dim3(256), 0, st, a); break;
        default: fg_set_error("fused CG: unsupported row length"); return FG_ERR_UNSUPPORTED;
    }
    return FG_OK;
}

}

bool fg_fcg_ok(const fg_state* s) {
    const FgGrid& G = s->grid;
    return s->cg_fused && s->fd_dct_x != 0 && G.dims == 2 && fg_fd_dct_supported(G.nx) && G.fixed[2] && G.fixed[3] && G.ny >= 3 &&
           s->fcg_alpha != nullptr;
}

int fg_fcg_update_fwd(fg_state* s, const FcgVectors& v, int it, int first, int ns, hipStream_t st, bool marks_valid, const fg_real* r0) {
    const FgGrid& G = s->grid;
    FcgUpdArgs a = {};
    a.r0 = r0; a.x_zero = r0 ? 1 : 0;
    a.lazy = (it == 0 && marks_valid) ? s->fcg_lazy : nullptr;
    a.z = v.z; a.w = v.w; a.p = v.p; a.s = v.s; a.x = v.x; a.r = v.r; a.t1 = v.t1;
    a.tw = s->fd_dct_tw; a.rot = s->fd_dct_rot; a.fs0 = s->fd_dct_fwd[0]; a.fs = s->fd_dct_fwd[1];
    a.flags = s->flags; a.acc = s->cg_acc; a.alpha = s->fcg_alpha; a.xsum = s->fcg_xsum; a.best = s->cg_best;
    a.ns = ns; a.rows = G.ny; a.it = it; a.first = first; a.env_stride = G.n;
    const dim3 grid((G.ny + 7) / 8, G.B);
    const int slot = fg_prof_slot(s, FG_PK_FCG_UPD, s->flags, G.B, (first ? (r0 ? 24.0 : 28.0) : 44.0) * G.n, (10.0 + 5.0 * log2((double)G.nx)) * G.n, st);
    if (int rc = (s->fd_dct_x == 2 ? launch_upd<true>(s, slot, G.nx, a, grid, st) : launch_upd<false>(s, slot, G.nx, a, grid, st))) return rc;
    FG_HIP_CHECK(hipGetLastError());
    return FG_OK;
}

int fg_fcg_inv_apply(fg_state* s, const FcgVectors& v, const fg_real* rA, int it, int ns, hipStream_t st, int extras) {
    const FgGrid& G = s->grid;
    FcgInvArgs a = {};
    a.u = v.t1; a.r = v.r; a.rA = rA; a.z = v.z; a.w = v.w;
    a.tw = s->fd_dct_tw; a.rot = s->fd_dct_rot; a.is0 = s->fd_dct_inv[0]; a.is = s->fd_dct_inv[1];
    a.flags = s->flags; a.acc = s->cg_acc; a.ns = ns; a.rows = G.ny; a.it = it; a.env_stride = G.n;
    a.xsum = s->fcg_xsum; a.extras = (extras && it == 0) ? 1 : 0;
    a.hy = G.h[1]; a.rhy = G.rh[1]; a.hx = G.h[0]; a.rhx = G.rh[0]; a.fixed_x = G.fixed[0];
    const dim3 grid((G.ny + 7) / 8, G.B);
    const int slot = fg_prof_slot(s, FG_PK_FCG_INV, s->flags, G.B, 20.0 * G.n, (14.0 + 5.0 * log2((double)G.nx)) * G.n, st);
    if (int rc = (s->fd_dct_x == 2 ? launch_inv<true>(s, slot, G.nx, a, grid, st) : launch_inv<false>(s, slot, G.nx, a, grid, st))) return rc;
    FG_HIP_CHECK(hipGetLastError());
    return FG_OK;
}
int fg_fcg_check0(fg_state* s, fg_real tol, int ns, hipStream_t st, FgPollOut poll, bool* marks_valid) {
    const FgGrid& G = s->grid;
    hipLaunchKernelGGL(k_fcg_check0, dim3((G.B + CHECK_WAVES - 1) / CHECK_WAVES), dim3(64 * CHECK_WAVES), 0, st, s->cg_acc, s->flags, s->info_dev, s->info_pinned, s->fcg_alpha, s->fcg_lazy,
                       tol, G.n, G.B, ns, poll);
    FG_HIP_CHECK(hipGetLastError());
    *marks_valid = true;
    return FG_OK;
}
int fg_fcg_div_fwd(fg_state* s, const FgBounds& bnd, const fg_real* dt, const fg_real* hvec, fg_real* div, int ns, hipStream_t st) {
    const FgGrid& G = s->grid;
    FcgDivArgs a = {};
    a.h = hvec; a.div = div; a.r = s->w[0]; a.x = s->p_result; a.t1 = s->w[3];
    for (int f = 0; f < 4; ++f) a.bvel[f] = bnd.vel[f];
    a.tw = s->fd_dct_tw; a.rot = s->fd_dct_rot; a.fs0 = s->fd_dct_fwd[0]; a.fs = s->fd_dct_fwd[1];
    a.dt = dt; a.acc = s->cg_acc; a.ns = ns; a.rows = G.ny; a.n = G.n;
    a.hx = G.h[0]; a.hy = G.h[1]; a.fixed_x = G.fixed[0];
    const dim3 grid((G.ny + 7) / 8, G.B);
    if (int rc = (s->fd_dct_x == 2 ? launch_div<true>(s, G.nx, a, grid, st) : launch_div<false>(s, G.nx, a, grid, st))) return rc;
    FG_HIP_CHECK(hipGetLastError());
    return FG_OK;
}
#endif
```

### fluidgym_amd/csrc/fg_internal.h

```cpp
#pragma once
#include <hip/hip_runtime.h>
#include <hip/hip_ext.h>
#include <math.h>
#include <stdint.h>
#include <cstring>
#include <string>
#include <type_traits>

#include "../../include/fluidgym_hip.h"

#ifdef FG_REAL_DOUBLE
struct alignas(16) fg_real4 { double x, y, z, w; };
__host__ __device__ __forceinline__ fg_real4 make_fg_real4(double x, double y, double z, double w) { fg_real4 r; r.x = x; r.y = y; r.z = z; r.w = w; return r; }
#define FG_F64 1
#define FG_FMAX fmax
#define FG_FABS fabs
#define FG_SQRT sqrt
#else
typedef float4 fg_real4;
#define make_fg_real4 make_float4
#define FG_F64 0
#define FG_FMAX fmaxf
#define FG_FABS fabsf
#define FG_SQRT sqrtf
// ... 533 lines not shown
            if (!info[i].converged) unconv[kind] += 1;
        }
    }
    void reset() { *this = FgCounters(); }
    void write(int64_t* out) const {
        for (int k = 0; k < 4; ++k) { out[k] = sum[k]; out[4 + k] = n[k]; out[8 + k] = max[k]; }
        out[12] = piso_steps;
    }
};

struct FgPrepared {
    int bicg_nc; const fg_real* bicg_dt;
    int cg_ns, cg_best; const fg_real* cg_dt;
    int cg_start;
    void clear() { *this = FgPrepared{}; }
    void set_bicg(int nc, const fg_real* dt) { clear(); bicg_nc = nc; bicg_dt = dt; }
    void set_cg(int ns, int best, const fg_real* dt) { clear(); cg_ns = ns; cg_best = best; cg_dt = dt; }
    bool cg_for(const fg_real* dt) const { return cg_ns > 0 && cg_dt == dt; }
    void set_cg_start(int form) { cg_start = form; }
    bool take_bicg(int nc, const fg_real* dt) { const bool ready = bicg_nc == nc && bicg_dt == dt; clear(); return ready; }
    int take_cg(int ns, int best, const fg_real* dt) {
        const int got = (cg_ns == ns && cg_best == best && cg_dt == dt) ? cg_start : -1; clear(); return got;
    }
};

struct FgNu {
    fg_real v = 0; const fg_real* per_env = nullptr;
#ifdef __HIPCC__
    __device__ __forceinline__ fg_real at(int b) const { return per_env ? per_env[b] : v; }
#endif
    bool same(const FgNu& o) const { return v == o.v && per_env == o.per_env; }
};

struct fg_state {
    fg_config cfg;
    FgGrid grid;
    int vec;
    fg_real viscosity;
    fg_real scalar_viscosity[FG_MAX_SCALARS];
    bool scalar_viscosity_set;
    const fg_real* viscosity_B;
    const fg_real* scalar_viscosity_B[FG_MAX_SCALARS];
    fg_real* d_h[3];
    fg_real* d_rh[3];
    fg_real* velocity;
    fg_real* pressure;
    fg_real* scalar;
    fg_real* velocity_source;
    fg_real* visc_field;
    fg_real* bvel[6];
    fg_real* bscal[6];
    fg_real* A;
    fg_real* rA;
    fg_real* Coff;
    fg_real* adv_rhs;
    fg_real* vel_result;
    fg_real* hvec;
    fg_real* div;
    fg_real* p_result;
    fg_real* scal_result;
    fg_real* w[8];
    FgDacc* acc;
    int32_t* flags;
    fg_solve_info* info_dev;
    fg_solve_info* info_pinned;
    int32_t* flags_pinned;
    fg_real* scratch_B;
    FgProf prof;
    FgDacc* cg_acc;
    FgBest cg_best;
    int cg_return_best;
    int cg_reset_steps;
    int adv_from_result;
    int adv_precond; long long line_retries;
    int cg_wgs_per_slot;
    int wall_forcing_axis; fg_real wall_forcing_coef[2]; fg_real* force_uniform;
    int reduce_wgs;
    int bicg_sub;
    int bicg3_force, bicg3_bxl, bicg3_mix;
    int bicg_fused;
    int cg_fused, bicg_pfused; double* fcg_alpha; FgDacc* fcg_xsum;
    int32_t* fcg_lazy; int fcg_first;
    int fcg_spec;
    int jac_spec; long jac_spec_missed;
    long jac_floor_released = 0;
    int jac_prefactor;
    int jac_warm;
    long fcg_unstored, fcg_first_polls;
    fg_real* line_inv; fg_real* line_cp;
    fg_real* ilu_d;
    int double_fallback; int ladder_force; long long rung_count[4];
    double* r64_buf; FgDacc* r64_acc;
    int ref64_outer; float ref64_tol, ref64_inner; double* ref64_x; long ref64_corrections;
    float* fd_Qx; float* fd_QxT; float* fd_Qz; float* fd_QzT; float* fd_lower; float* fd_inv; float* fd_cp;
    float* fd_lam; float* helm_diag; float* helm_lower; float* helm_upper; float* helm_tmp;
    float* helm_lower_row; float helm_rs; int helm_cb, helm_rowform_off, helm_cb_pref;
    float* line_inv2; float* line_cp2; float* helm_lower_row2; int helm_pre_mask; const fg_real* helm_pre_dt; FgNu helm_pre_nu[2]; int helm_pre_walls[2][2]; int helm_set;
    int tridiag_cb;
    int fd_dct_x; float2* fd_dct_tw; float2* fd_dct_rot; float fd_dct_fwd[2]; float fd_dct_inv[2];
    float* fd_lam_x; float* fd_row_inv; float* fd_row_cp; float* fd_row_lower; int fd_rowmean; long fd_row_epoch; mutable long rA_epoch;
    int fd_facfuse;
    float* fd_row_part; long fd_row_part_epoch;
    int32_t* forms_rec;
    const fg_real* adv_last_dt;
    fg_real** d_bvel_ptrs;
    fg_real* diag_pinned;
    fg_real* dt_pinned;
    fg_real* dt_dev;
    double* t_rem_dev;
    int dev_dt;
    int pred_bicg[4], pred_cg[4];
    int adv_jacobi, adv_jacobi_env; FgJacHist jac_hist[4]; float* jac_prev;
    int adv_linesweep;
    long long jac_solves, jac_fallbacks;
    long jac_rA_epoch;
    FgCounters ctr;
    const fg_real* cur_dt;
    FgPoll poll;
    mutable int maxvel_clean;
    FgPrepared prepared;
    fg_env_sel* env_sel_dev;
    size_t n_cells() const { return (size_t)grid.n; }
};
inline FgNu fg_nu(const fg_state* s, int for_scalar = 0, int channel = 0) {
    FgNu n;
    if (for_scalar && s->scalar_viscosity_B[channel]) { n.v = s->scalar_viscosity[channel]; n.per_env = s->scalar_viscosity_B[channel]; }
    else if (for_scalar && s->scalar_viscosity_set) n.v = s->scalar_viscosity[channel];
    else { n.v = s->viscosity; n.per_env = s->viscosity_B; }
    return n;
}

void fg_set_error(const std::string& msg);
#define FG_REQUIRE(cond, code, msg)  \
    do {                             \
        if (!(cond)) {               \
            fg_set_error(msg);       \
            return code;             \
        }                            \
    } while (0)
#define FG_HIP_CHECK(expr)                                                                        \
    do {                                                                                          \
        hipError_t _e = (expr);                                                                   \
        if (_e != hipSuccess) {                                                                   \
            fg_set_error(std::string(#expr) + ": " + hipGetErrorString(_e));                      \
            return FG_ERR_HIP;                                                                    \
        }                                                                                         \
    } while (0)

#if FG_F64
#define FG_DISPATCH(s, ...)                                                       \
    do {                                                                          \
        if ((s)->grid.dims == 2) { constexpr int DIMS = 2, VEC = 1; __VA_ARGS__; } \
        else { constexpr int DIMS = 3, VEC = 1; __VA_ARGS__; }                    \
    } while (0)
#else
#define FG_DISPATCH(s, ...)                                                       \
    do {                                                                          \
        if ((s)->grid.dims == 2) {                                                \
            if ((s)->vec == 4) { constexpr int DIMS = 2, VEC = 4; __VA_ARGS__; }  \
            else { constexpr int DIMS = 2, VEC = 1; __VA_ARGS__; }                \
        } else {                                                                  \
            if ((s)->vec == 4) { constexpr int DIMS = 3, VEC = 4; __VA_ARGS__; }  \
            else { constexpr int DIMS = 3, VEC = 1; __VA_ARGS__; }                \
        }                                                                         \
    } while (0)
#endif

struct FgBicgBegin { FgDacc* acc; fg_real* sc; int32_t* flags; fg_solve_info* info; int nc; };
#ifdef __HIPCC__
__device__ __forceinline__ void fg_bicg_begin_sys(const FgBicgBegin& q, const fg_real* __restrict__ dt, int sys) {
    for (int k = 0; k < FG_ACC_DOUBLES; ++k) acc_st(q.acc + ((size_t)sys * FG_ACC_DOUBLES + k), 0.0);
    sc_st(q.sc + (sys * 2), 1.f); sc_st(q.sc + (sys * 2 + 1), 1.f);
    const bool active = (dt == nullptr) || (dt[sys / q.nc] > 0.f);
    flag_st(q.flags + (sys), active ? 0 : 3);
    q.info[sys].final_residual = 0.f;
    q.info[sys].used_iterations = -1;
    q.info[sys].converged = active ? 0 : 1;
    q.info[sys].is_finite = 1;
}
#endif
struct FgAdvArgs {
    const fg_real* vel;
    const fg_real* scal;
    long scal_env_stride;
    const fg_real* source;
    const fg_real* force;
    const fg_real* dt;
    FgNu nu;
    const fg_real* visc;
    int for_scalar;
    int channel, n_scalars;
    fg_real* A; fg_real* Coff; fg_real* rhs;
    fg_real* rA;
    FgBicgBegin begin;
    const fg_real* buoy_T; long buoy_stride; int buoy_axis; fg_real buoy_factor; fg_real* source_w;
    fg_real* row_part;
};
int fg_launch_adv_build(fg_state* s, const FgBounds& bnd, const FgAdvArgs& a, hipStream_t st);
int fg_launch_wall_forcing(const fg_state* s, hipStream_t st);
int fg_launch_sgs(const fg_state* s, const FgBounds& bnd, fg_real coefficient, fg_real* out, hipStream_t st);
int fg_launch_pressure_setup(const fg_state* s, const fg_real* dt, hipStream_t st);
int fg_launch_h(fg_state* s, const fg_real* dt, const fg_real* vel_result, hipStream_t st);
int fg_launch_div(fg_state* s, const FgBounds& bnd, const fg_real* dt, const fg_real* hvec, fg_real* div, hipStream_t st,
                  bool cg_from_zero = false,
                  bool fused_fwd = false);
struct FgMeanRef { const FgDacc* sums; const fg_solve_info* info; fg_real* p_copy; const int32_t* lazy; const double* alpha; };
struct FgLazyRef { const int32_t* lazy; const double* alpha; fg_real* p_res; };
int fg_launch_correct(const fg_state* s, const fg_real* dt, const fg_real* rA, const fg_real* hvec, const fg_real* p,
                      fg_real* vel_out, hipStream_t st, fg_real* vel_copy = nullptr, const FgMeanRef* mean = nullptr, const FgLazyRef* lazy = nullptr);
struct FgDtRule { double* t_rem; fg_real* dt_out; float cfl; double time_step; int reset; };
int fg_launch_max_velocity(const fg_state* s, const FgBounds& bnd, fg_real* out_B, hipStream_t st, fg_real* mirror_B = nullptr,
                           FgPollOut poll = FgPollOut{nullptr, 0}, fg_real* flux_B = nullptr, fg_real* flux_mirror = nullptr,
                           FgDtRule rule = FgDtRule{nullptr, nullptr, 0.f, 0.0, 0});
int fg_launch_flux_balance(const fg_state* s, const FgBounds& bnd, fg_real* out_B, hipStream_t st, FgPollOut poll = FgPollOut{nullptr, 0});
int fg_launch_copy_active(const fg_state* s, const fg_real* dt, const fg_real* src, fg_real* dst, int comps, hipStream_t st);
int fg_launch_buoyancy(const fg_state* s, const fg_real* dt, const fg_real* T, long t_env_stride, fg_real* source, int axis,
                       fg_real factor, hipStream_t st);
int fg_launch_outflow(const fg_state* s, int face, fg_real velm_axis, const fg_real* dt, hipStream_t st);
int fg_launch_balance(const fg_state* s, const FgBounds& bnd, int free_mask, fg_real atol, const fg_real* dt, hipStream_t st,
                      int outflow_mask = 0, const fg_real* outflow_velm = nullptr,
                      const fg_real* dt_host_values = nullptr);
bool fg_outflow_folds(const fg_state* s, int outflow_mask);
int fg_launch_mean_sub(const fg_state* s, const fg_real* active_dt, fg_real* p, fg_real* p_copy, hipStream_t st);

int fg_poisson_apply_launch(const fg_state* s, const fg_real* rA, const fg_real* x, fg_real* y, hipStream_t st);
int fg_poisson_jacobi_launch(const fg_state* s, const fg_real* rA, const fg_real* b, const fg_real* x, fg_real* xnew,
                             fg_real omega, hipStream_t st);
int fg_poisson_rbgs_launch(const fg_state* s, const fg_real* rA, const fg_real* b, fg_real* x, fg_real omega, int color,
                           hipStream_t st);
struct FgCgOutcome {
    const fg_real* lazy_z = nullptr;
    bool mean_ready = false;
    bool marks_valid = false;
    bool spec_done = false;
};
struct FgCgSpec { int (*fn)(void* ctx, const FgCgOutcome& o) = nullptr; void* ctx = nullptr; };
struct FgCgArgs {
    const fg_real* rA; const fg_real* b; fg_real* x;
    fg_real* r; fg_real* p; fg_real* Ap;
    const fg_real* dt;
    fg_real tol; int max_iterations; int use_x0; int reset_steps;
    int check_every;
    int precond;
    int kind = 2;
    int lazy_ok = 0;
    FgCgSpec spec;
};
int fg_cg_solve(fg_state* s, const FgCgArgs& a, fg_solve_info* info_host, hipStream_t st, FgCgOutcome* out = nullptr);

struct FgSpecHook { int (*fn)(void* ctx) = nullptr; void* ctx = nullptr; };
struct FgBicgArgs {
    const fg_real* diag; const fg_real* off;
    const fg_real* rhs; fg_real* x;
    int nc;
    const fg_real* dt;
    fg_real tol; int max_iterations; int use_x0;
    int precond = 0;
    FgNu nu; int wall_lo = 1, wall_hi = 1;
    int kind = 1;
    FgSpecHook spec;
};
int fg_bicgstab_solve(fg_state* s, const FgBicgArgs& a, fg_solve_info* info_host, hipStream_t st, bool* spec_ran = nullptr);
#if !FG_F64
enum FgSweepOutcome {
    FG_SWEEP_NOT_TRIED,
    FG_SWEEP_SOLVED,
    FG_SWEEP_SOLVED_SPEC,
    FG_SWEEP_GAVE_UP,
    FG_SWEEP_SPEC_MISSED,
};
bool fg_jacobi_ok(const fg_state* s, const FgBicgArgs& a);
bool fg_linesweep_ok(const fg_state* s, const FgBicgArgs& a);
int fg_linesweep_solve(fg_state* s, const FgBicgArgs& a, fg_solve_info* info_host, hipStream_t st, FgSweepOutcome* outcome);
int fg_jacobi_solve(fg_state* s, const FgBicgArgs& a, fg_solve_info* info_host, hipStream_t st, FgSweepOutcome* outcome);
#endif
int fg_rung64_bicgstab(fg_state* s, const FgBicgArgs& a, fg_solve_info* info_host, bool all_systems, hipStream_t st);
int fg_rung64_cg(fg_state* s, const FgCgArgs& a, fg_solve_info* info_host, bool all_envs, hipStream_t st, FgCgOutcome* out);

bool fg_zmarch_ok(const fg_state* s, int* zc_out);
int fg_zmarch_apply(const fg_state* s, const fg_real* rA, const fg_real* x, fg_real* y, int zc, hipStream_t st);
int fg_zmarch_relax(const fg_state* s, const fg_real* rA, const fg_real* b, const fg_real* x, fg_real* xnew, fg_real omega,
                    int color, int zc, hipStream_t st);
int fg_zmarch_cg_ap(const fg_state* s, const fg_real* rA, const fg_real* z, const fg_real* p_in, fg_real* p_out, fg_real* Ap,
                    FgDacc* acc, int32_t* flags, fg_solve_info* info, int prof_slot, fg_real tol, int it, int first,
                    int ns, int num_base, int zc, hipStream_t st);
#define FG_PROF_SELF ((const int32_t*)(uintptr_t)1)
int fg_prof_slot(const fg_state* s, int kind, const int32_t* flags, int nsys, double bytes_per_sys,
                 double flops_per_sys, hipStream_t st);
int fg_prof_collect(fg_state* s, hipStream_t st);
void fg_prof_prefetch(fg_state* s, hipStream_t st);
void fg_prof_destroy(fg_state* s);
bool fg_fd_dct_supported(int n);
struct FgCgJudge;
int fg_fd_dct_forward(fg_state* s, const fg_real* r, fg_real* out, hipStream_t st, int batch = 0, const FgCgJudge* judge = nullptr);
int fg_fd_dct_inverse(fg_state* s, const fg_real* u, fg_real* z, const fg_real* dot_with, FgDacc* dot_acc, int dot_stride,
                      int dot_ns, hipStream_t st, int batch = 0);
#define FG_LAUNCH_P(s, slot, kernel, grid, block, shmem, st, ...)                                              \
    do {                                                                                                       \
        const int slot__ = (slot);                                                                             \
        if (slot__ >= 0)                                                                                       \
            hipExtLaunchKernelGGL(kernel, grid, block, shmem, st, (s)->prof.ev[2 * slot__],                    \
                                  (s)->prof.ev[2 * slot__ + 1], 0, __VA_ARGS__);                               \
        else                                                                                                   \
            hipLaunchKernelGGL(kernel, grid, block, shmem, st, __VA_ARGS__);                                   \
    } while (0)
int fg_fd_apply(fg_state* s, const fg_real* r, fg_real* z, FgDacc* rz_acc, int rz_stride, int rz_ns, int expect_active,
                hipStream_t st, const FgCgJudge* judge = nullptr);
struct FgCgLead;
int fg_fd_tridiag(fg_state* s, float* cur, hipStream_t st, const FgCgLead* lead, bool use_rowmean = false, const float* factor_from = nullptr, const float* factor_dt = nullptr);
bool fg_fd_tridiag_can_factor(const fg_state* s);
bool fg_fd_rowmean_ok(const fg_state* s);
int fg_refine64_pressure(fg_state* s, const FgCgArgs& a0, fg_solve_info* info_host, hipStream_t st, FgCgOutcome* out);
int fg_fd_rowmean_factor(fg_state* s, const float* rA, const float* dt, hipStream_t st, const float* row_part = nullptr, int tiles_x = 0);
int fg_fd_rowmean_prefactor(fg_state* s, const fg_real* dt, hipStream_t st);
int fg_line_alloc(fg_state* s);
int fg_ilu_alloc(fg_state* s);
int fg_ilu_factor(fg_state* s, const fg_real* diag, const fg_real* off, hipStream_t st);
int fg_ilu_apply(fg_state* s, const fg_real* diag, const fg_real* off, int nc, const fg_real* r, fg_real* z, hipStream_t st);
int fg_helm_alloc(fg_state* s);
int fg_helm_factor(fg_state* s, const fg_real* dt, FgNu nu, int wall_lo, int wall_hi, int nc, hipStream_t st, int kind = -1);
int fg_helm_factor_pair(fg_state* s, const float* dt, const FgNu nu[2], const int wall_lo[2], const int wall_hi[2], hipStream_t st);
int fg_helm_apply(fg_state* s, int nc, const float* r, float* z, hipStream_t st);
int fg_fd_helmholtz_apply(fg_state* s, int nc, const fg_real* r, fg_real* z, hipStream_t st);
int fg_line_factor(fg_state* s, const fg_real* diag, const fg_real* off, int nc, hipStream_t st);
int fg_line_apply(fg_state* s, const fg_real* diag, const fg_real* off, int nc, const fg_real* r, fg_real* z, hipStream_t st);
int fg_metrics_launch(const float* coords, float* transforms, int dims, int nx, int ny, int nz, hipStream_t st);
```

### fluidgym_amd/csrc/fg_piso.hip

```cpp
#include "fg_internal.h"
#include "fg_cg.h"
#include "fg_fftcg.h"

namespace {

template <int VEC>
__device__ __forceinline__ fg_real fg_elem_mask(int e, fg_real lo_mask_or_hi, bool is_edge_elem) {
    return is_edge_elem ? lo_mask_or_hi : 1.f;
}

template <int DIMS, int VEC>
__device__ __forceinline__ int fg_slab_index(const FgGrid& g, const FgCtx<DIMS, VEC>& c, int a) {
    if (a == 0) return c.k * g.ny + c.j;
    if (a == 1) return c.k * g.nx + c.i0;
    return c.j * g.nx + c.i0;
}
__device__ __forceinline__ int fg_slab_size(const FgGrid& g, int a) {
    return (a == 0) ? g.ny * g.nz : (a == 1) ? g.nx * g.nz : g.nx * g.ny;
}

template <int DIMS, int VEC, bool SCALAR, bool VISC = false>
__global__ __launch_bounds__(FG_BLOCK) void k_adv_build(FgGrid g, FgBounds bnd, FgAdvArgs a, int tiles_x,
                                                         int tiles_y, int tiles) {
    const FgCtx<DIMS, VEC> c = fg_make_ctx<DIMS, VEC>(g, tiles_x, tiles_y, tiles);
// ... 193 lines not shown
    const FgVec<VEC> rA = fg_load<VEC>(rA_ + (size_t)c.b * N + c.idx);
    FgVec<VEC> off[2 * DIMS];
#pragma unroll
    for (int f = 0; f < 2 * DIMS; ++f) off[f] = fg_load<VEC>(Coff + ((size_t)c.b * 2 * DIMS + f) * N + c.idx);
#pragma unroll
    for (int q = 0; q < DIMS; ++q) {
        const size_t base = ((size_t)c.b * DIMS + q) * N;
        const FgNbr<DIMS, VEC> u = fg_gather<DIMS, VEC>(velr + base, c);
        const FgVec<VEC> r = fg_load<VEC>(rhs + base + c.idx);
        FgVec<VEC> out;
#pragma unroll
        for (int e = 0; e < VEC; ++e) {
            fg_real H = off[0].v[e] * u.xm.v[e] + off[1].v[e] * u.xp.v[e] + off[2].v[e] * u.ym.v[e] +
                      off[3].v[e] * u.yp.v[e];
            if constexpr (DIMS == 3) H += off[4].v[e] * u.zm.v[e] + off[5].v[e] * u.zp.v[e];
            out.v[e] = rA.v[e] * (r.v[e] - H);
        }
        fg_store<VEC>(hvec + base + c.idx, out);
    }
}

template <int DIMS, int VEC>
__global__ __launch_bounds__(FG_BLOCK) void k_div(FgGrid g, FgBounds bnd, const fg_real* __restrict__ dt,
                                                   const fg_real* __restrict__ hvec, fg_real* __restrict__ div, FgCgStart start,
                                                   int tiles_x, int tiles_y, int tiles) {
    const FgCtx<DIMS, VEC> c = fg_make_ctx<DIMS, VEC>(g, tiles_x, tiles_y, tiles);
    if (dt && !(dt[c.b] > 0.f)) return;
    if (!c.valid && !start.acc) return;
    const size_t N = g.n;
    const FgMetric<DIMS, VEC> m = fg_metrics<DIMS, VEC>(g, c);
    fg_real acc[VEC];
#pragma unroll
    for (int e = 0; e < VEC; ++e) acc[e] = 0.f;
#pragma unroll
    for (int ax = 0; ax < DIMS; ++ax) {
        FgVec<VEC> ctr, lo, hi;
        fg_gather_axis<DIMS, VEC>(hvec + ((size_t)c.b * DIMS + ax) * N, c, ax, ctr, lo, hi);
        const int slab = fg_slab_index<DIMS, VEC>(g, c, ax);
        const int slab_n = fg_slab_size(g, ax);
#pragma unroll
        for (int e = 0; e < VEC; ++e) {
            fg_real area, mask_lo, mask_hi;
            if (ax == 0) { area = m.hy * m.hz; mask_lo = (e == 0) ? c.mxm : 1.f; mask_hi = (e == VEC - 1) ? c.mxp : 1.f; }
            else if (ax == 1) { area = m.hx[e] * m.hz; mask_lo = c.mym; mask_hi = c.myp; }
            else { area = m.hx[e] * m.hy; mask_lo = c.mzm; mask_hi = c.mzp; }
            const int bi = slab + ((ax == 0) ? 0 : e);
            fg_real F_hi, F_lo;
            if (mask_hi != 0.f) F_hi = 0.5f * (ctr.v[e] + hi.v[e]) * area;
            else F_hi = bnd.vel[2 * ax + 1][((size_t)c.b * DIMS + ax) * slab_n + bi] * area;
            if (mask_lo != 0.f) F_lo = 0.5f * (ctr.v[e] + lo.v[e]) * area;
            else F_lo = bnd.vel[2 * ax][((size_t)c.b * DIMS + ax) * slab_n + bi] * area;
            acc[e] += F_hi - F_lo;
        }
    }
    FgVec<VEC> out;
#pragma unroll
    for (int e = 0; e < VEC; ++e) out.v[e] = acc[e];
    if (c.valid) fg_store<VEC>(div + (size_t)c.b * N + c.idx, out);
    if (start.acc) {
        __shared__ fg_real lds[4];
        fg_real part[1] = {0.f};
        if (c.valid) {
            FgVec<VEC> z;
#pragma unroll
            for (int e = 0; e < VEC; ++e) { z.v[e] = 0.f; part[0] += out.v[e] * out.v[e]; }
            fg_store<VEC>(start.x + (size_t)c.b * N + c.idx, z);
            fg_store<VEC>(start.r + (size_t)c.b * N + c.idx, out);
        }
        fg_block_sum<1>(part, lds);
        if (threadIdx.x == 0) {
            const unsigned tile = fg_xcd_remap(blockIdx.x, gridDim.x) % tiles;
            fg_acc_add(fg_acc_ptr(start.acc, c.b, 0), start.ns, tile, (double)part[0]);
        }
    }
}

template <int DIMS, int VEC>
__global__ __launch_bounds__(FG_BLOCK) void k_correct(FgGrid g, const fg_real* __restrict__ dt,
                                                       const fg_real* __restrict__ rA_, const fg_real* __restrict__ hvec,
                                                       const fg_real* __restrict__ p, fg_real* __restrict__ vel_out,
                                                       fg_real* __restrict__ vel_copy, FgMeanRef mean, FgLazyRef lazy, int tiles_x, int tiles_y, int tiles) {
    const FgCtx<DIMS, VEC> c = fg_make_ctx<DIMS, VEC>(g, tiles_x, tiles_y, tiles);
    if ((dt && !(dt[c.b] > 0.f)) || !c.valid) return;
    const size_t N = g.n;
    const FgMetric<DIMS, VEC> m = fg_metrics<DIMS, VEC>(g, c);
    const FgVec<VEC> rA = fg_load<VEC>(rA_ + (size_t)c.b * N + c.idx);
    FgNbr<DIMS, VEC> P = fg_gather<DIMS, VEC>(p + (size_t)c.b * N, c);
    if (lazy.lazy) {
        const bool on = lazy.lazy[c.b] == 1;
        const fg_real sc = on ? (fg_real)lazy.alpha[2 * c.b] : (fg_real)0;
        auto scale = [&](FgVec<VEC>& v) {
#pragma unroll
            for (int e = 0; e < VEC; ++e) v.v[e] = on ? sc * v.v[e] : (fg_real)0;
        };
        scale(P.c); scale(P.xm); scale(P.xp); scale(P.ym); scale(P.yp);
        if constexpr (DIMS == 3) { scale(P.zm); scale(P.zp); }
        if (lazy.p_res) fg_store<VEC>(lazy.p_res + (size_t)c.b * N + c.idx, P.c);
    }
    if (mean.sums) {
        const int used = mean.info[c.b].used_iterations;
        const bool first_only = mean.lazy && mean.lazy[c.b] == 1;
        const fg_real mu = first_only ? (fg_real)(mean.alpha[2 * c.b] * acc_ld(mean.sums + (2 * c.b + 1)) / (double)g.n)
                           : used < 0 ? (fg_real)0 : (fg_real)(acc_ld(mean.sums + (2 * c.b + (used & 1))) / (double)g.n);
        FgVec<VEC> pc;
#pragma unroll
        for (int e = 0; e < VEC; ++e) pc.v[e] = P.c.v[e] - mu;
        fg_store<VEC>(mean.p_copy + (size_t)c.b * N + c.idx, pc);
    }
#pragma unroll
    for (int q = 0; q < DIMS; ++q) {
        const size_t base = ((size_t)c.b * DIMS + q) * N;
        const FgVec<VEC> h = fg_load<VEC>(hvec + base + c.idx);
        FgVec<VEC> out;
#pragma unroll
        for (int e = 0; e < VEC; ++e) {
            fg_real lo, hi, fac, rh;
            if (q == 0) {
                lo = P.xm.v[e]; hi = P.xp.v[e]; rh = m.rhx[e];
                const fg_real ml = (e == 0) ? c.mxm : 1.f, mh = (e == VEC - 1) ? c.mxp : 1.f;
                fac = (ml == 0.f || mh == 0.f) ? 1.f : 0.5f;
            } else if (q == 1) {
                lo = P.ym.v[e]; hi = P.yp.v[e]; rh = m.rhy;
                fac = (c.mym == 0.f || c.myp == 0.f) ? 1.f : 0.5f;
            } else {
                lo = P.zm.v[e]; hi = P.zp.v[e]; rh = m.rhz;
                fac = (c.mzm == 0.f || c.mzp == 0.f) ? 1.f : 0.5f;
            }
            out.v[e] = h.v[e] - rA.v[e] * ((hi - lo) * fac * rh);
        }
        fg_store<VEC>(vel_out + base + c.idx, out);
        if (vel_copy) fg_store<VEC>(vel_copy + base + c.idx, out);
    }
}

#if FG_F64
typedef long long fg_bits;
__device__ __forceinline__ fg_bits fg_real_bits(fg_real v) { return __double_as_longlong(v); }
__device__ __forceinline__ fg_real fg_bits_real(fg_bits b) { return __longlong_as_double(b); }
#else
typedef int fg_bits;
__device__ __forceinline__ fg_bits fg_real_bits(fg_real v) { return __float_as_int(v); }
__device__ __forceinline__ fg_real fg_bits_real(fg_bits b) { return __int_as_float(b); }
#endif
template <int DIMS>
__device__ __forceinline__ double fg_flux_balance_block(const FgGrid& g, const FgBounds& bnd, int b) {
    double acc = 0.0;
    const int lane = threadIdx.x & 63, wave = threadIdx.x >> 6;
    for (int f = 0; f < 2 * DIMS; ++f) {
        if (!g.fixed[f]) continue;
        const int ax = f >> 1;
        const int slab_n = fg_slab_size(g, ax);
        const double sgn = (f & 1) ? 1.0 : -1.0;
        const int n0 = (ax == 0) ? g.ny : g.nx;
        const int n1 = (DIMS == 3) ? ((ax == 2) ? g.ny : g.nz) : 1;
        const fg_real* __restrict__ h0 = (ax == 0) ? g.h[1] : g.h[0];
        const fg_real* __restrict__ h1 = (DIMS == 3) ? ((ax == 2) ? g.h[1] : g.h[2]) : nullptr;
        const fg_real* __restrict__ v = bnd.vel[f] + ((size_t)b * DIMS + ax) * slab_n;
        constexpr int RU = 4, WV = FG_BLOCK / 64;
        for (int i1b = wave; i1b < n1; i1b += WV * RU) {
            for (int i0 = lane; i0 < n0; i0 += 64) {
                fg_real val[RU], a1[RU];
#pragma unroll
                for (int u = 0; u < RU; ++u) {
                    const int i1 = i1b + u * WV;
                    const bool ok = i1 < n1;
                    a1[u] = ok ? (h1 ? h1[i1] : (fg_real)1) : (fg_real)0;
                    val[u] = ok ? v[(size_t)i1 * n0 + i0] : (fg_real)0;
                }
                const fg_real w0 = h0[i0];
#pragma unroll
                for (int u = 0; u < RU; ++u) acc += sgn * (double)(val[u] * (w0 * a1[u]));
            }
// ... 478 lines not shown
        hi += (double)u[((size_t)k * g.ny + (g.ny - 1)) * g.nx + i];
    }
    __shared__ double lds[2][16];
#pragma unroll
    for (int o = 32; o > 0; o >>= 1) { lo += __shfl_down(lo, o, 64); hi += __shfl_down(hi, o, 64); }
    if ((threadIdx.x & 63) == 0) { lds[0][threadIdx.x >> 6] = lo; lds[1][threadIdx.x >> 6] = hi; }
    __syncthreads();
    if (threadIdx.x == 0) {
        double sl = 0.0, sh = 0.0;
        for (int w = 0; w < (int)(blockDim.x >> 6); ++w) { sl += lds[0][w]; sh += lds[1][w]; }
        const double n = (double)rows * g.nx;
        const fg_real tau_lo = coef_lo * (fg_real)(sl / n), tau_hi = coef_hi * (fg_real)(sh / n);
        for (int q = 0; q < dims; ++q) force[b * dims + q] = (q == axis) ? (fg_real)0.5 * (tau_lo + tau_hi) : (fg_real)0;
    }
}

int fg_launch_wall_forcing(const fg_state* s, hipStream_t st) {
    hipLaunchKernelGGL(k_wall_forcing, dim3(s->grid.B), dim3(1024), 0, st, s->grid, (const fg_real*)s->velocity, s->wall_forcing_axis,
                       s->wall_forcing_coef[0], s->wall_forcing_coef[1], s->force_uniform, s->grid.dims);
    FG_HIP_CHECK(hipGetLastError());
    return FG_OK;
}

int fg_launch_sgs(const fg_state* s, const FgBounds& bnd, fg_real coefficient, fg_real* out, hipStream_t st) {
    const dim3 grid((s->grid.n + FG_BLOCK - 1) / FG_BLOCK, s->grid.B);
    if (s->grid.dims == 2) hipLaunchKernelGGL(k_sgs_smagorinsky<2>, grid, dim3(FG_BLOCK), 0, st, s->grid, bnd, (const fg_real*)s->velocity, coefficient, out);
    else hipLaunchKernelGGL(k_sgs_smagorinsky<3>, grid, dim3(FG_BLOCK), 0, st, s->grid, bnd, (const fg_real*)s->velocity, coefficient, out);
    FG_HIP_CHECK(hipGetLastError());
    return FG_OK;
}

int fg_launch_pressure_setup(const fg_state* s, const fg_real* dt, hipStream_t st) {
    const int n = s->grid.n;
    hipLaunchKernelGGL(k_reciprocal, stride_grid(s, n), dim3(FG_BLOCK), 0, st, s->A, s->rA, dt, n, (n % 4 == 0) ? n / 4 : 0);
    FG_HIP_CHECK(hipGetLastError());
    return FG_OK;
}

int fg_launch_h(fg_state* s, const fg_real* dt, const fg_real* vel_result, hipStream_t st) {
    fg_htrace("h_launch_in");
    FgCgBegin begin;
    begin.acc = s->cg_acc; begin.flags = s->flags; begin.info = s->info_dev; begin.mean_sums = s->acc; begin.best = s->cg_best;
    begin.track_best = s->cg_return_best; begin.ns = fg_cg_slots(s); begin.xsum = s->fcg_xsum;
    s->prepared.set_cg(begin.ns, begin.track_best, dt);
    const int slot_h = fg_prof_slot(s, FG_PK_H, nullptr, s->grid.B, (s->grid.dims == 3 ? 68.0 : 52.0) * (double)s->grid.n, 6.0 * s->grid.dims * s->grid.dims * (double)s->grid.n, st);
    FG_DISPATCH(s, {
        const FgLaunch L = fg_launch_geometry<DIMS, VEC>(s->grid);
        FG_LAUNCH_P(s, slot_h, (k_h<DIMS, VEC>), L.grid, dim3(FG_BLOCK), 0, st, s->grid, dt, s->rA, s->Coff, s->adv_rhs,
                    vel_result, s->hvec, begin, L.tiles_x, L.tiles_y, L.tiles);
    });
    FG_HIP_CHECK(hipGetLastError());
    fg_htrace("h_launch_out");
    return FG_OK;
}

int fg_launch_div(fg_state* s, const FgBounds& bnd, const fg_real* dt, const fg_real* hvec, fg_real* div,
                  hipStream_t st, bool cg_from_zero, bool fused_fwd) {
    FgCgStart start = {nullptr, nullptr, nullptr, 1};
    s->prepared.set_cg_start(0);
    if (cg_from_zero && dt != nullptr && s->prepared.cg_for(dt) && div == s->div) {
#if !FG_F64
        if (fused_fwd && fg_fcg_ok(s)) {
            s->prepared.set_cg_start(2);
            return fg_fcg_div_fwd(s, bnd, dt, hvec, div, s->prepared.cg_ns, st);
        }
#endif
        start.acc = s->cg_acc; start.r = s->w[0]; start.x = s->p_result; start.ns = s->prepared.cg_ns;
        s->prepared.set_cg_start(1);
    }
    const int slot_d = fg_prof_slot(s, FG_PK_DIV, nullptr, s->grid.B, 28.0 * (double)s->grid.n, 4.0 * s->grid.dims * (double)s->grid.n, st);
    FG_DISPATCH(s, {
        const FgLaunch L = fg_launch_geometry<DIMS, VEC>(s->grid);
        FG_LAUNCH_P(s, slot_d, (k_div<DIMS, VEC>), L.grid, dim3(FG_BLOCK), 0, st, s->grid, bnd, dt, hvec, div, start, L.tiles_x,
                    L.tiles_y, L.tiles);
    });
    FG_HIP_CHECK(hipGetLastError());
    return FG_OK;
}

int fg_launch_correct(const fg_state* s, const fg_real* dt, const fg_real* rA, const fg_real* hvec, const fg_real* p,
                      fg_real* vel_out, hipStream_t st, fg_real* vel_copy, const FgMeanRef* mean, const FgLazyRef* lazy) {
    fg_htrace("correct_in");
    const FgMeanRef mr = mean ? *mean : FgMeanRef{nullptr, nullptr, nullptr, nullptr, nullptr};
    const FgLazyRef lz = lazy ? *lazy : FgLazyRef{nullptr, nullptr, nullptr};
    const double cb = (s->grid.dims == 3 ? 36.0 : 28.0) + (vel_copy ? 4.0 * s->grid.dims : 0.0) + ((mean && mean->sums) || (lazy && lazy->p_res) ? 4.0 : 0.0);
    const int slot_c = fg_prof_slot(s, FG_PK_CORRECT, nullptr, s->grid.B, cb * (double)s->grid.n, 5.0 * s->grid.dims * (double)s->grid.n, st);
    FG_DISPATCH(s, {
        const FgLaunch L = fg_launch_geometry<DIMS, VEC>(s->grid);
        FG_LAUNCH_P(s, slot_c, (k_correct<DIMS, VEC>), L.grid, dim3(FG_BLOCK), 0, st, s->grid, dt, rA, hvec, p, vel_out, vel_copy, mr, lz,
                    L.tiles_x, L.tiles_y, L.tiles);
    });
    FG_HIP_CHECK(hipGetLastError());
    fg_htrace("correct_out");
    return FG_OK;
}

int fg_launch_max_velocity(const fg_state* s, const FgBounds& bnd, fg_real* out_B, hipStream_t st, fg_real* mirror_B, FgPollOut poll,
                           fg_real* flux_B, fg_real* flux_mirror, FgDtRule rule) {
    FG_REQUIRE(!rule.t_rem || (poll.gran && mirror_B && !FG_F64), FG_ERR_INVALID_ARG, "the device-side sub-step rule needs the result-word form");
    FG_REQUIRE(!flux_B || (mirror_B && flux_mirror), FG_ERR_INVALID_ARG, "the flux balance rides in the mirrored form only");
    int32_t* done_B = reinterpret_cast<int32_t*>(out_B + s->grid.B);
    FG_REQUIRE(!mirror_B || out_B == s->scratch_B + s->grid.B, FG_ERR_INVALID_ARG, "mirror needs the scratch row as out_B");
    if (!mirror_B || !s->maxvel_clean)
        FG_HIP_CHECK(hipMemsetAsync(out_B, 0, mirror_B ? sizeof(fg_real) * s->grid.B + sizeof(int32_t) * (s->grid.B + 1) : sizeof(fg_real) * s->grid.B, st));
    s->maxvel_clean = mirror_B ? 1 : 0;
    if ((s->grid.nx & 3) == 0) {
        const int rows = s->grid.ny * s->grid.nz;
        int rpb = 4;
        while ((long)((rows + 2 * rpb - 1) / (2 * rpb)) * s->grid.B >= 2048) rpb *= 2;
        while ((rows + rpb - 1) / rpb > (int)fg_reduce_wgs(s)) rpb *= 2;
        dim3 grid((rows + rpb - 1) / rpb, s->grid.B);
        const int slot_m = fg_prof_slot(s, FG_PK_MAXVEL, nullptr, s->grid.B, 4.0 * s->grid.dims * (double)s->grid.n, 2.0 * s->grid.dims * (double)s->grid.n, st);
        if (s->grid.dims == 2)
            FG_LAUNCH_P(s, slot_m, k_max_velocity_rows<2>, grid, dim3(FG_BLOCK), 0, st, s->grid, bnd, s->velocity, out_B, done_B,
                        mirror_B, rpb, poll, flux_B, flux_mirror, rule);
        else
            FG_LAUNCH_P(s, slot_m, k_max_velocity_rows<3>, grid, dim3(FG_BLOCK), 0, st, s->grid, bnd, s->velocity, out_B, done_B,
                        mirror_B, rpb, poll, flux_B, flux_mirror, rule);
        FG_HIP_CHECK(hipGetLastError());
        return FG_OK;
    }
    dim3 grid = stride_grid(s, (long)s->grid.n * 4);
    if (s->grid.dims == 2)
        hipLaunchKernelGGL(k_max_velocity<2>, grid, dim3(FG_BLOCK), 0, st, s->grid, bnd, s->velocity, out_B, done_B, mirror_B, poll, flux_B, flux_mirror, rule);
    else
        hipLaunchKernelGGL(k_max_velocity<3>, grid, dim3(FG_BLOCK), 0, st, s->grid, bnd, s->velocity, out_B, done_B, mirror_B, poll, flux_B, flux_mirror, rule);
    FG_HIP_CHECK(hipGetLastError());
    return FG_OK;
}

int fg_launch_flux_balance(const fg_state* s, const FgBounds& bnd, fg_real* out_B, hipStream_t st, FgPollOut poll) {
    if (s->grid.dims == 2)
        hipLaunchKernelGGL(k_flux_balance<2>, dim3(s->grid.B), dim3(FG_BLOCK), 0, st, s->grid, bnd, out_B, poll);
    else
        hipLaunchKernelGGL(k_flux_balance<3>, dim3(s->grid.B), dim3(FG_BLOCK), 0, st, s->grid, bnd, out_B, poll);
    FG_HIP_CHECK(hipGetLastError());
    return FG_OK;
}

int fg_launch_copy_active(const fg_state* s, const fg_real* dt, const fg_real* src, fg_real* dst, int comps,
                          hipStream_t st) {
    const long per_env = (long)comps * s->grid.n;
    hipLaunchKernelGGL(k_copy_active, stride_grid(s, per_env), dim3(FG_BLOCK), 0, st, dt, src, dst, per_env);
    FG_HIP_CHECK(hipGetLastError());
    return FG_OK;
}

int fg_launch_buoyancy(const fg_state* s, const fg_real* dt, const fg_real* T, long t_env_stride, fg_real* source, int axis,
                       fg_real factor, hipStream_t st) {
    hipLaunchKernelGGL(k_buoyancy, stride_grid(s, (long)s->grid.n * 4), dim3(FG_BLOCK), 0, st, dt, T, t_env_stride,
                       source, s->grid.dims, s->grid.n, axis, factor);
    FG_HIP_CHECK(hipGetLastError());
    return FG_OK;
}

int fg_launch_mean_sub(const fg_state* s, const fg_real* dt, fg_real* p, fg_real* p_copy, hipStream_t st) {
    FgDacc* sums = s->acc;
    dim3 grid = stride_grid(s, (long)s->grid.n * 4);
    dim3 rgrid(grid.x > fg_reduce_wgs(s) ? fg_reduce_wgs(s) : grid.x, grid.y);
    hipLaunchKernelGGL(k_sum_env, rgrid, dim3(FG_BLOCK), 0, st, dt, p, sums, s->grid.n);
    hipLaunchKernelGGL(k_sub_mean, grid, dim3(FG_BLOCK), 0, st, dt, p, p_copy, sums, s->grid.n);
    FG_HIP_CHECK(hipGetLastError());
    return FG_OK;
}

int fg_launch_outflow(const fg_state* s, int face, fg_real velm_axis, const fg_real* dt, hipStream_t st) {
    const int slab_n = (face >> 1) == 0 ? s->grid.ny * s->grid.nz : (face >> 1) == 1 ? s->grid.nx * s->grid.nz : s->grid.nx * s->grid.ny;
// ... 45 lines not shown
```

### fluidgym_amd/csrc/fg_poisson.hip

```cpp
#include <math.h>
#include <cmath>
#include <vector>

#include "fg_internal.h"
#include "fg_cg.h"
#include "fg_rung64.h"
#include "fg_fftcg.h"

namespace {

template <int DIMS, int VEC>
struct FgCoef {
    fg_real xm[VEC], xp[VEC], ym[VEC], yp[VEC], zm[VEC], zp[VEC];
};

template <int DIMS, int VEC>
__device__ __forceinline__ FgCoef<DIMS, VEC> fg_poisson_coef(const FgCtx<DIMS, VEC>& c, const FgMetric<DIMS, VEC>& m,
                                                             const FgNbr<DIMS, VEC>& rA) {
    FgCoef<DIMS, VEC> k;
    const fg_real ayz = m.hy * m.hz;
#pragma unroll
    for (int e = 0; e < VEC; ++e) {
        const fg_real rh_lo = (e == 0) ? m.rhx_m : m.rhx[e > 0 ? e - 1 : 0];
        const fg_real rh_hi = (e == VEC - 1) ? m.rhx_p : m.rhx[e < VEC - 1 ? e + 1 : VEC - 1];
// ... 280 lines not shown
    const fg_real have = best.saved_crit[b];
    const bool worse = !(I.final_residual <= have);
    if (I.converged || !worse || !isfinite(have)) return;
    for (int i = blockIdx.x * blockDim.x + threadIdx.x; i < n; i += gridDim.x * blockDim.x)
        x[(size_t)b * n + i] = best.best_x[(size_t)b * n + i];
    if (blockIdx.x == 0 && threadIdx.x == 0) {
        mirror[b].final_residual = have;
        mirror[b].is_finite = 1;
    }
}

}


int fg_poisson_apply_launch(const fg_state* s, const fg_real* rA, const fg_real* x, fg_real* y, hipStream_t st) {
    int zc;
    if (fg_zmarch_ok(s, &zc)) return fg_zmarch_apply(s, rA, x, y, zc, st);
    FG_DISPATCH(s, {
        const FgLaunch L = fg_launch_geometry<DIMS, VEC>(s->grid);
        hipLaunchKernelGGL((k_poisson_apply<DIMS, VEC>), L.grid, dim3(FG_BLOCK), 0, st, s->grid, rA, x, y, L.tiles_x,
                           L.tiles_y, L.tiles);
    });
    FG_HIP_CHECK(hipGetLastError());
    return FG_OK;
}

int fg_poisson_jacobi_launch(const fg_state* s, const fg_real* rA, const fg_real* b, const fg_real* x, fg_real* xnew,
                             fg_real omega, hipStream_t st) {
    int zc;
    if (fg_zmarch_ok(s, &zc)) return fg_zmarch_relax(s, rA, b, x, xnew, omega, -1, zc, st);
    FG_DISPATCH(s, {
        const FgLaunch L = fg_launch_geometry<DIMS, VEC>(s->grid);
        hipLaunchKernelGGL((k_poisson_relax<DIMS, VEC, false>), L.grid, dim3(FG_BLOCK), 0, st, s->grid, rA, b, x, xnew,
                           omega, 0, L.tiles_x, L.tiles_y, L.tiles);
    });
    FG_HIP_CHECK(hipGetLastError());
    return FG_OK;
}

int fg_poisson_rbgs_launch(const fg_state* s, const fg_real* rA, const fg_real* b, fg_real* x, fg_real omega, int color,
                           hipStream_t st) {
    int zc;
    if (fg_zmarch_ok(s, &zc)) return fg_zmarch_relax(s, rA, b, x, x, omega, color, zc, st);
    FG_DISPATCH(s, {
        const FgLaunch L = fg_launch_geometry<DIMS, VEC>(s->grid);
        hipLaunchKernelGGL((k_poisson_relax<DIMS, VEC, true>), L.grid, dim3(FG_BLOCK), 0, st, s->grid, rA, b, x, x,
                           omega, color, L.tiles_x, L.tiles_y, L.tiles);
    });
    FG_HIP_CHECK(hipGetLastError());
    return FG_OK;
}

int fg_fd_rowmean_prefactor(fg_state* s, const fg_real* dt, hipStream_t st) {
#if !FG_F64
    if (!(s->fd_Qx && fg_fcg_ok(s) && fg_fd_rowmean_ok(s)) || s->fd_row_epoch == s->rA_epoch || dt == nullptr) return FG_OK;
    const bool parts = s->fd_row_part && s->fd_row_part_epoch == s->rA_epoch;
    if (parts && fg_fd_tridiag_can_factor(s)) return FG_OK;
    if (int rc = fg_fd_rowmean_factor(s, s->rA, dt, st, parts ? s->fd_row_part : nullptr, (s->grid.nx + 63) / 64)) return rc;
    s->fd_row_epoch = s->rA_epoch;
#else
    (void)s; (void)dt; (void)st;
#endif
    return FG_OK;
}

int fg_cg_slots(const fg_state* s) {
    int tiles_per_env = 1;
    FG_DISPATCH(s, { tiles_per_env = fg_launch_geometry<DIMS, VEC>(s->grid).tiles; });
    int ns = 1;
    while (ns < FG_CG_SLOTS && tiles_per_env / ns > s->cg_wgs_per_slot) ns *= 2;
    return ns;
}

namespace {
struct CgRun {
    int ns, nb, check_every, next_poll;
    fg_real* zvec;
    FgDacc* mean_sums;
    FgCgJudge judge;
    bool fused;
    bool start_ready = false;
    bool start_fwd = false;
    bool done = false, info_fresh = false;
};
}

static int cg_begin(fg_state* s, const FgCgArgs& a, CgRun& c, hipStream_t st) {
    const int B = s->grid.B, n = s->grid.n;
    const int ns = c.ns = fg_cg_slots(s);
    {
        const int prep = s->prepared.take_cg(ns, s->cg_return_best, a.dt);
        c.start_ready = prep > 0 && !a.use_x0 && a.b == s->div && a.r == s->w[0] && a.x == s->p_result;
        c.start_fwd = c.start_ready && prep == 2;
        if (prep < 0) {
            FgCgBegin q;
            q.acc = s->cg_acc; q.flags = s->flags; q.info = s->info_dev; q.mean_sums = s->acc; q.best = s->cg_best;
            q.track_best = s->cg_return_best; q.ns = ns; q.xsum = s->fcg_xsum;
            hipLaunchKernelGGL(k_cg_begin, dim3(B), dim3(64), 0, st, a.dt, q, B);
        }
    }
    if (!c.start_ready)
    FG_DISPATCH(s, {
        const FgLaunch L = fg_launch_geometry<DIMS, VEC>(s->grid);
        hipLaunchKernelGGL((k_cg_residual<DIMS, VEC>), L.grid, dim3(FG_BLOCK), 0, st, s->grid, a.rA, a.b, a.x, a.r,
                           s->cg_acc, s->flags, a.use_x0, 0, ns, L.tiles_x, L.tiles_y, L.tiles);
    });
    c.check_every = a.check_every > 0 ? a.check_every : 16;
    c.nb = a.precond ? 5 : 0;
    c.zvec = a.precond ? s->w[5] : a.r;
    c.judge.acc = s->cg_acc; c.judge.flags = s->flags; c.judge.info = s->info_dev; c.judge.tol = a.tol; c.judge.it = -1; c.judge.n = n; c.judge.ns = ns;
#if !FG_F64
    c.fused = a.precond && s->fd_Qx && fg_fcg_ok(s);
#else
    c.fused = false;
#endif
    if (a.precond && !c.fused) {
        if (!s->fd_Qx) { fg_set_error("preconditioned CG requested but fg_set_fd_preconditioner was not called"); return FG_ERR_INVALID_ARG; }
        if (int rc = fg_fd_apply(s, a.r, c.zvec, s->cg_acc + (size_t)(c.nb + 0) * FG_CG_SLOTS, FG_CG_NAMES * FG_CG_SLOTS, ns, B, st, &c.judge)) return rc;
    }
    c.next_poll = a.precond ? (s->pred_cg[a.kind & 3] + 1 > 1 ? s->pred_cg[a.kind & 3] + 1 : 1) : c.check_every;
    c.mean_sums = (!a.use_x0 && a.x == s->p_result && s->fcg_xsum) ? s->fcg_xsum : nullptr;
    return FG_OK;
}

#if !FG_F64
static int cg_iterate_fused(fg_state* s, const FgCgArgs& a, CgRun& c, FgCgOutcome& o, hipStream_t st) {
    const int B = s->grid.B, n = s->grid.n, ns = c.ns;
    FgCgJudge& judge = c.judge;
    FcgVectors v;
    v.x = a.x; v.r = a.r; v.t1 = s->w[3]; v.z = c.zvec; v.w = s->w[4]; v.p = a.p; v.s = a.Ap;
    FgCgLead lead;
    lead.best = s->cg_best;
    const bool rowm = fg_fd_rowmean_ok(s);
    const float* factor_from = nullptr;
    if (rowm && !(a.rA == s->rA && s->fd_row_epoch == s->rA_epoch)) {
        const bool parts = a.rA == s->rA && s->fd_row_part && s->fd_row_part_epoch == s->rA_epoch;
        if (parts && fg_fd_tridiag_can_factor(s)) factor_from = s->fd_row_part;
        else if (int rc = fg_fd_rowmean_factor(s, a.rA, a.dt, st, parts ? s->fd_row_part : nullptr, (s->grid.nx + 63) / 64)) return rc;
        s->fd_row_epoch = (a.rA == s->rA) ? s->rA_epoch : -1;
    }
    judge.it = -1;
    if (!c.start_fwd)
        if (int rc = fg_fd_dct_forward(s, a.r, v.t1, st, 0, &judge)) return rc;
    lead.judge = judge;
    if (int rc = fg_fd_tridiag(s, v.t1, st, &lead, rowm, factor_from, a.dt)) return rc;
    const fg_real* r0 = c.start_fwd ? a.b : nullptr;
    {
        FcgVectors v0 = v;
        if (r0) v0.r = const_cast<fg_real*>(r0);
        if (int rc = fg_fcg_inv_apply(s, v0, a.rA, 0, ns, st, s->fcg_first)) return rc;
    }
    if (s->fcg_first && a.max_iterations >= 1) {
        const bool poll0 = c.next_poll <= 1;
        const FgPollOut po = poll0 ? fg_poll_next(&s->poll) : FgPollOut{nullptr, 0};
        if (poll0) fg_prof_prefetch(s, st);
        if (int rc = fg_fcg_check0(s, a.tol, ns, st, po, &o.marks_valid)) return rc;
        bool spec = false;
        if (poll0 && s->fcg_spec && a.spec.fn && a.lazy_ok && r0 && c.mean_sums) {
            FgCgOutcome ahead;
            ahead.lazy_z = v.z; ahead.mean_ready = true; ahead.marks_valid = true;
            if (int rc = a.spec.fn(a.spec.ctx, ahead)) return rc;
            spec = true;
        }
        if (poll0) {
            fg_htrace("cg_check_launched");
            if (int rc = fg_poll_wait_infos(&s->poll, po, 0, B, s->info_pinned, st)) return rc;
            fg_htrace("cg_poll_done");
            c.info_fresh = true;
            s->fcg_first_polls += 1;
            bool all = true, all_ok = true;
            for (int b = 0; b < B; ++b) {
                all = all && (s->info_pinned[b].converged || !s->info_pinned[b].is_finite);
                all_ok = all_ok && s->info_pinned[b].converged && s->info_pinned[b].is_finite;
            }
            if (all) {
                if (a.lazy_ok && r0 && all_ok && c.mean_sums) {
                    o.lazy_z = v.z; s->fcg_unstored += 1; o.spec_done = spec;
                } else {
                    if (int rc = fg_fcg_update_fwd(s, v, 0, 1, ns, st, o.marks_valid, r0)) return rc;
                }
                c.done = true;
            } else {
                c.next_poll = 2;
            }
        }
    }
    int first = 1;
    const int fused_reset = (a.reset_steps > 0 && a.reset_steps < 10) ? a.reset_steps : 10;
    for (int it = 0; it < a.max_iterations && !c.done; ++it) {
        if (int rc = fg_fcg_update_fwd(s, v, it, first, ns, st, o.marks_valid, it == 0 ? r0 : nullptr)) return rc;
        if (first) {
            fg_real* t = v.p; v.p = v.z; v.z = t;
            t = v.s; v.s = v.w; v.w = t;
            first = 0;
        }
        const bool poll = (it + 1 >= c.next_poll || it + 1 == a.max_iterations);
        if (poll) {
            c.next_poll = it + 1 + c.check_every;
            const int final_pass = (it + 1 == a.max_iterations);
            fg_prof_prefetch(s, st);
            const FgPollOut po = fg_poll_next(&s->poll);
            hipLaunchKernelGGL(k_cg_check, dim3((B + CG_CHECK_WAVES - 1) / CG_CHECK_WAVES), dim3(64 * CG_CHECK_WAVES), 0, st, s->cg_acc, s->flags, s->info_dev, s->info_pinned, a.tol, it,
                               n, B, final_pass, ns, po);
            fg_htrace("cg_check_launched");
            if (int rc = fg_poll_wait_infos(&s->poll, po, 0, B, s->info_pinned, st)) return rc;
            fg_htrace("cg_poll_done");
            c.info_fresh = true;
            c.done = true;
            for (int b = 0; b < B; ++b) c.done = c.done && (s->info_pinned[b].converged || !s->info_pinned[b].is_finite);
            if (c.done) break;
        }
        if (it + 1 < a.max_iterations) {
            judge.it = it;
            if ((it + 2) % fused_reset == 0) {
                hipLaunchKernelGGL(k_zero_name, dim3(B), dim3(64), 0, st, s->cg_acc, (it + 1) % 3, B);
                FG_DISPATCH(s, {
                    const FgLaunch L = fg_launch_geometry<DIMS, VEC>(s->grid);
                    hipLaunchKernelGGL((k_cg_residual<DIMS, VEC>), L.grid, dim3(FG_BLOCK), 0, st, s->grid, a.rA, a.b, a.x,
                                       a.r, s->cg_acc, s->flags, 1, (it + 1) % 3, ns, L.tiles_x, L.tiles_y, L.tiles);
                });
                if (int rc = fg_fd_dct_forward(s, a.r, v.t1, st, 0, nullptr)) return rc;
                first = 1;
            }
            lead.judge = judge;
            if (int rc = fg_fd_tridiag(s, v.t1, st, &lead, rowm)) return rc;
            if (int rc = fg_fcg_inv_apply(s, v, a.rA, it + 1, ns, st)) return rc;
        }
    }
    o.mean_ready = !a.use_x0;
    return FG_OK;
}
#endif

static int cg_iterate_classic(fg_state* s, const FgCgArgs& a, CgRun& c, FgCgOutcome& o, hipStream_t st) {
    const int B = s->grid.B, n = s->grid.n, ns = c.ns, nb = c.nb;
    fg_real* pbuf[2] = {a.p, s->w[6]};
    int zc = 0;
    const bool zmarch = fg_zmarch_ok(s, &zc);
    int active_est = (B + 3) / 4;
    for (int it = 0; it < a.max_iterations && !c.done; ++it) {
        int first = (it == 0);
        if (a.reset_steps > 0 && it > 0 && (it + 1) % a.reset_steps == 0) {
            hipLaunchKernelGGL(k_zero_name, dim3(B), dim3(64), 0, st, s->cg_acc, it % 3, B);
            FG_DISPATCH(s, {
                const FgLaunch L = fg_launch_geometry<DIMS, VEC>(s->grid);
                hipLaunchKernelGGL((k_cg_residual<DIMS, VEC>), L.grid, dim3(FG_BLOCK), 0, st, s->grid, a.rA, a.b, a.x,
                                   a.r, s->cg_acc, s->flags, 1, it % 3, ns, L.tiles_x, L.tiles_y, L.tiles);
            });
            first = 1;
        }
        const fg_real* p_in = pbuf[(it + 1) & 1];
        fg_real* p_out = pbuf[it & 1];
        const int slot_ap = fg_prof_slot(s, FG_PK_CG_AP, FG_PROF_SELF, B, (double)n * (first ? 16.0 : 20.0),
                                         (double)n * (4.0 * s->grid.dims + 5.0), st);
        if (zmarch) {
            if (int rc = fg_zmarch_cg_ap(s, a.rA, c.zvec, p_in, p_out, a.Ap, s->cg_acc, s->flags, s->info_dev, slot_ap,
                                         a.tol, it, first, ns, nb, zc, st))
                return rc;
        } else {
            FG_DISPATCH(s, {
                const FgLaunch L = fg_launch_geometry<DIMS, VEC>(s->grid);
                FG_LAUNCH_P(s, slot_ap, (k_cg_ap<DIMS, VEC>), L.grid, dim3(FG_BLOCK), 0, st, s->grid, a.rA, c.zvec, p_in,
                            p_out, a.Ap, s->cg_acc, s->flags, s->info_dev,
                            slot_ap >= 0 ? s->prof.active_dev + slot_ap : nullptr, s->cg_best, a.tol, it, first, ns,
                            nb, L.tiles_x, L.tiles_y, L.tiles);
            });
        }
        const int slot_up = fg_prof_slot(s, FG_PK_CG_UPDATE, s->flags, B, (double)n * 24.0, (double)n * 6.0, st);
        FG_DISPATCH(s, {
            const FgLaunch L = fg_launch_geometry<DIMS, VEC>(s->grid);
            FG_LAUNCH_P(s, slot_up, (k_cg_update<DIMS, VEC>), L.grid, dim3(FG_BLOCK), 0, st, s->grid, p_out, a.Ap, a.x,
                        a.r, s->cg_acc, s->flags, s->cg_best, a.tol, it, ns, nb, c.mean_sums, L.tiles_x, L.tiles_y, L.tiles);
        });
        const bool poll = (it + 1 >= c.next_poll || it + 1 == a.max_iterations);
        if (poll) c.next_poll = it + 1 + c.check_every;
        if (poll) {
            const int final_pass = (it + 1 == a.max_iterations);
            fg_prof_prefetch(s, st);
            const FgPollOut po = fg_poll_next(&s->poll);
            hipLaunchKernelGGL(k_cg_check, dim3((B + CG_CHECK_WAVES - 1) / CG_CHECK_WAVES), dim3(64 * CG_CHECK_WAVES), 0, st, s->cg_acc, s->flags, s->info_dev, s->info_pinned, a.tol, it,
                               n, B, final_pass, ns, po);
            if (int rc = fg_poll_wait_infos(&s->poll, po, 0, B, s->info_pinned, st)) return rc;
            c.info_fresh = true;
            c.done = true;
            active_est = 0;
            for (int b = 0; b < B; ++b) {
                const bool fin = s->info_pinned[b].converged || !s->info_pinned[b].is_finite;
                c.done = c.done && fin;
                active_est += !fin;
            }
            if (active_est < 1) active_est = 1;
            if (c.done) break;
        }
        if (a.precond && it + 1 < a.max_iterations) {
            c.judge.it = it;
            if (int rc = fg_fd_apply(s, a.r, c.zvec, s->cg_acc + (size_t)(nb + (it + 1) % 3) * FG_CG_SLOTS, FG_CG_NAMES * FG_CG_SLOTS, ns, active_est, st, &c.judge))
                return rc;
        }
    }
    if (c.mean_sums) o.mean_ready = true;
    return FG_OK;
}

static int cg_finish(fg_state* s, const FgCgArgs& a, const CgRun& c, FgCgOutcome& o, fg_solve_info* info_host, hipStream_t st) {
    const int B = s->grid.B, n = s->grid.n;
    if (!c.info_fresh) {
        FG_HIP_CHECK(hipMemcpyAsync(s->info_pinned, s->info_dev, sizeof(fg_solve_info) * B, hipMemcpyDeviceToHost, st));
        FG_HIP_CHECK(hipStreamSynchronize(st));
    }
    if (int prc = fg_prof_collect(s, st)) return prc;
    bool failed = false;
    for (int b = 0; b < B; ++b) failed = failed || !s->info_pinned[b].converged;
    if (failed) {
        o.mean_ready = false;
        hipLaunchKernelGGL(k_cg_restore_best, dim3(32, B), dim3(FG_BLOCK), 0, st, a.x, s->info_dev, s->info_pinned, s->cg_best, n);
        FG_HIP_CHECK(hipStreamSynchronize(st));
    }
    int rc = FG_OK;
    if (a.precond) {
        int used_max = 0;
        for (int b = 0; b < B; ++b) used_max = s->info_pinned[b].used_iterations > used_max ? s->info_pinned[b].used_iterations : used_max;
        s->pred_cg[a.kind & 3] = used_max;
    }
    for (int b = 0; b < B; ++b) {
        if (info_host) info_host[b] = s->info_pinned[b];
        if (!s->info_pinned[b].is_finite) rc = FG_ERR_NOT_FINITE;
        else if (!s->info_pinned[b].converged && rc == FG_OK) rc = FG_ERR_NOT_CONVERGED;
    }
    FG_HIP_CHECK(hipGetLastError());
    return rc;
}

int fg_cg_solve(fg_state* s, const FgCgArgs& a, fg_solve_info* info_host, hipStream_t st, FgCgOutcome* out) {
    CgRun c;
    FgCgOutcome o;
    if (int rc = cg_begin(s, a, c, st)) return rc;
#if !FG_F64
    if (c.fused) { if (int rc = cg_iterate_fused(s, a, c, o, st)) return rc; }
    else
#endif
    if (int rc = cg_iterate_classic(s, a, c, o, st)) return rc;
    const int rc = cg_finish(s, a, c, o, info_host, st);
    if (out) *out = o;
    return rc;
}

#if !FG_F64
namespace {
template <int DIMS>
__global__ __launch_bounds__(FG_BLOCK) void k64_papply(FgGrid g, const float* __restrict__ rA_, const double* __restrict__ x, double* __restrict__ y,
                                                       int tiles_x, int tiles_y, int tiles) {
    const FgCtx<DIMS, 1> c = fg_make_ctx<DIMS, 1>(g, tiles_x, tiles_y, tiles);
    if (!c.valid) return;
    const FgMetric<DIMS, 1> m = fg_metrics<DIMS, 1>(g, c);
    const FgNbr<DIMS, 1> rA = fg_gather<DIMS, 1>(rA_, c);
    const FgCoef<DIMS, 1> k = fg_poisson_coef<DIMS, 1>(c, m, rA);
    const R64Nbr<DIMS> X = r64_gather<DIMS>(x, c);
    double v = (double)k.xm[0] * (X.xm - X.c) + (double)k.xp[0] * (X.xp - X.c) + (double)k.ym[0] * (X.ym - X.c) + (double)k.yp[0] * (X.yp - X.c);
    if constexpr (DIMS == 3) v += (double)k.zm[0] * (X.zm - X.c) + (double)k.zp[0] * (X.zp - X.c);
    y[c.idx] = v;
}
}

int fg_rung64_cg(fg_state* s, const FgCgArgs& a, fg_solve_info* info, bool all_envs, hipStream_t st, FgCgOutcome* out) {
    R64 w;
    if (int rc = w.init(s, st)) return rc;
    const int B = s->grid.B, n = s->grid.n, d = s->grid.dims;
    FgGrid g1 = s->grid; g1.B = 1;
    double *r = w.v[0], *p = w.v[1], *Ap = w.v[2], *x = w.v[3], *bb = w.v[4];
    auto apply = [&](int b, const double* in, double* out) {
        const float* rA = a.rA + (size_t)b * n;
        if (d == 2) { FgLaunch L = fg_launch_geometry<2, 1>(g1); hipLaunchKernelGGL((k64_papply<2>), L.grid, dim3(FG_BLOCK), 0, st, g1, rA, in, out, L.tiles_x, L.tiles_y, L.tiles); }
        else { FgLaunch L = fg_launch_geometry<3, 1>(g1); hipLaunchKernelGGL((k64_papply<3>), L.grid, dim3(FG_BLOCK), 0, st, g1, rA, in, out, L.tiles_x, L.tiles_y, L.tiles); }
    };
    auto rms = [&](double q) { return sqrt(q / (double)n); };
    std::vector<float> dt_host;
    if (a.dt) { dt_host.resize(B); FG_HIP_CHECK(hipMemcpyAsync(dt_host.data(), a.dt, sizeof(float) * B, hipMemcpyDeviceToHost, st)); FG_HIP_CHECK(hipStreamSynchronize(st)); }
    int rc_all = FG_OK;
    for (int b = 0; b < B; ++b) {
        if (a.dt && !(dt_host[b] > 0.f)) continue;
        fg_solve_info& I = info[b];
        if (!all_envs && I.is_finite) continue;
        w.load(bb, a.b + (size_t)b * n);
        w.zero(x);
        w.axpby(r, 1.0, bb, 0.0, bb);
        w.axpby(p, 1.0, r, 0.0, r);
        double rr = w.dot(r, r);
        I.used_iterations = -1; I.converged = 0; I.is_finite = 1; I.final_residual = (float)rms(rr);
        for (int it = 0; it < a.max_iterations; ++it) {
            if (!(rms(rr) >= (double)a.tol)) { I.converged = std::isfinite(rr) ? 1 : 0; break; }
            if (a.reset_steps > 0 && it > 0 && (it + 1) % a.reset_steps == 0) {
                apply(b, x, Ap);
                w.axpby(r, 1.0, bb, -1.0, Ap);
                w.axpby(p, 1.0, r, 0.0, r);
                rr = w.dot(r, r);
            }
            apply(b, p, Ap);
            const double pAp = w.dot(p, Ap);
            const double alpha = rr / pAp;
            w.axpby(x, 1.0, x, alpha, p);
            w.axpby(r, 1.0, r, -alpha, Ap);
            const double rr_new = w.dot(r, r);
            w.axpby(p, rr_new / rr, p, 1.0, r);
            rr = rr_new;
            I.used_iterations = it; I.final_residual = (float)rms(rr);
// ... 99 lines not shown
```

### include/fluidgym_hip.h

```cpp
#ifndef FLUIDGYM_HIP_H
#define FLUIDGYM_HIP_H

#include <stdint.h>

#ifdef __cplusplus
extern "C" {
#endif

#define FG_ABI_VERSION 1

#ifdef FG_REAL_DOUBLE
typedef double fg_real;
#else
typedef float fg_real;
#endif
#define FG_MAX_SCALARS 4

#define FG_OK 0
#define FG_ERR_INVALID_ARG (-1)
#define FG_ERR_NOT_BOUND (-2)
#define FG_ERR_HIP (-3)
#define FG_ERR_UNSUPPORTED (-4)
#define FG_ERR_NOT_CONVERGED (-5)
#define FG_ERR_NOT_FINITE (-6)
// ... 93 lines not shown
#define FG_FORM_GEMM_T64 2
#define FG_FORM_GEMM_T128 3
#define FG_FORM_GEMM_Z64 4
#define FG_FORM_DCT 5
#define FG_FORM_FFT 6
#define FG_FORM_F64 7
#define FG_FORM_TRI_STREAM 1
#define FG_FORM_TRI_LDS3 2
#define FG_FORM_TRI_LDS2 3
#define FG_FORM_TRI_LDS3_FAC 4
#define FG_FORM_TRI_LDS2_FAC 5
#define FG_FORM_TRI_F64 6
#define FG_FORM_FAC_GRID 1
#define FG_FORM_FAC_ROWMEAN 2
#define FG_FORM_FAC_MADE 3
#define FG_FORM_HELM_ARRAY 1
#define FG_FORM_HELM_ROW32 2
#define FG_FORM_HELM_ROW64 3
#define FG_FORM_LINE_LDS 1
#define FG_FORM_LINE_STREAM 2
int fg_set_fd_helmholtz(fg_handle h, const float* lam_host);
int fg_advection_retries(fg_handle h, int64_t* out, int32_t reset);
int fg_set_double_fallback(fg_handle h, int on);
int fg_set_advection_jacobi(fg_handle h, int on);
int fg_advection_jacobi_counts(fg_handle h, int64_t* out2);
int fg_ladder(fg_handle h, int64_t* out4, int32_t force_mask);
int fg_advection_solver_form(fg_handle h, int nc, int32_t* out);
int fg_copy_scalar_result_to_blocks(fg_handle h, int channel, void* stream);
int fg_setup_pressure_matrix(fg_handle h, void* stream);
int fg_setup_pressure_rhs(fg_handle h, const fg_real* dt_B, void* stream);
int fg_solve_pressure(fg_handle h, int method, fg_real tol, int max_iterations, int use_previous,
                      fg_solve_info* info_host, void* stream);
int fg_set_pressure_refinement(fg_handle h, int32_t max_corrections, fg_real target_tol, fg_real inner_relative_tol);
int fg_correct_velocity(fg_handle h, void* stream);
int fg_copy_velocity_result_to_blocks(fg_handle h, void* stream);
int fg_copy_velocity_result_from_blocks(fg_handle h, void* stream);

typedef struct fg_step_options {
    int32_t corrector_steps;
    int32_t advect_scalar;
    int32_t pressure_method;
    int32_t max_iterations;
    fg_real advection_tol;
    fg_real pressure_tol;
    int32_t buoyancy_axis;
    fg_real buoyancy_factor;
    int32_t pressure_warm_start;
} fg_step_options;
int fg_piso_step(fg_handle h, const fg_real* dt_B, const fg_step_options* opt, int32_t* stats_host,
                 void* stream);
int fg_solver_counters(fg_handle h, int64_t* out13_host, int32_t reset);
int fg_solver_unconverged(fg_handle h, int64_t* out4_host);
typedef struct fg_sim_options {
    fg_step_options step;
    fg_real time_step;
    fg_real cfl;
    int32_t adaptive;
    int32_t substeps;
    fg_real flux_balance_tol;
    int32_t outflow_mask;
    fg_real outflow_velm[3];
    fg_real outflow_tol;
    int32_t max_substeps;
} fg_sim_options;
int fg_single_step(fg_handle h, const fg_sim_options* opt, int32_t* out_host_6, fg_real* flux_balance_host,
                   void* stream);
int fg_multi_step(fg_handle h, const fg_sim_options* opt, int32_t n, const fg_real* const* bvel_schedule, int32_t* out_host_6n,
                  fg_real* flux_balance_host, int32_t* steps_done, void* stream);
int fg_make_divergence_free(fg_handle h, fg_real tol, int max_iterations, fg_solve_info* info_host,
                            void* stream);

enum fg_buffer {
    FG_BUF_A = 0,
    FG_BUF_C_OFF = 1,
    FG_BUF_ADV_RHS = 2,
    FG_BUF_VEL_RESULT = 3,
    FG_BUF_H = 4,
    FG_BUF_DIV = 5,
    FG_BUF_P_RESULT = 6,
    FG_BUF_SCALAR_RESULT = 7
};
int fg_reset_solver_state(fg_handle h, void* stream);
int fg_solver_hints(fg_handle h, int32_t* hints12, int32_t set);

typedef struct fg_env_sel {
    int32_t env, src;
    int32_t flip_x, flip_z;
    int32_t shift_x, shift_z;
} fg_env_sel;
int fg_env_restore_field(fg_handle h, int which_field, const fg_real* bank, int32_t S, const fg_env_sel* sel, int32_t n_sel,
                         int32_t signed_components, void* stream);
int fg_env_reset_solver_state(fg_handle h, const fg_env_sel* sel, int32_t n_sel, void* stream);
int fg_get_buffer(fg_handle h, int which, fg_real** out_ptr, int64_t* out_count);
int fg_read_buffer(fg_handle h, int which, fg_real* dst, void* stream);

int fg_poisson_apply(fg_handle h, const fg_real* rA, const fg_real* x, fg_real* y, void* stream);
int fg_poisson_jacobi(fg_handle h, const fg_real* rA, const fg_real* b, fg_real* x, int n_sweeps, fg_real omega,
                      void* stream);
int fg_poisson_rbgs(fg_handle h, const fg_real* rA, const fg_real* b, fg_real* x, int n_sweeps, fg_real omega,
                    void* stream);
int fg_poisson_cg(fg_handle h, const fg_real* rA, const fg_real* b, fg_real* x, fg_real tol, int max_iterations,
                  int use_x0, fg_solve_info* info_host, void* stream);
int fg_poisson_fdcg(fg_handle h, const fg_real* rA, const fg_real* b, fg_real* x, fg_real tol, int max_iterations,
                    int use_x0, fg_solve_info* info_host, void* stream);

int fg_stream_triad(float* a, const float* b, const float* c, float scalar, int64_t n, int32_t reps, float* ms_per_launch, void* stream);
int fg_coherence_litmus(int32_t atomic_access, int32_t nsys, int32_t cells, int32_t iterations, int64_t* bad_reads, double* bad_value,
                        void* stream);
int fg_dacc_host_sum(const double* values, int64_t n, double plain, double* out_sum);
int fg_dacc_device_sum(const double* values_host, int64_t n, double plain, int32_t reps, double* out_sums_host, void* stream);
#define FG_FIELD_SUMMARY_WORK_BYTES 128
int fg_field_summary(const fg_real* field, int32_t batch, int32_t channels, int64_t n, int32_t channel, void* workspace,
                     double* moments, int64_t* counts, double lo, double width, int32_t nbins, uint64_t* hist, void* stream);
int fg_plane_moments(const fg_real* const* channels, const int64_t* batch_stride, int32_t K, int32_t batch, int32_t nz, int32_t ny,
                     int32_t nx, int32_t order, double* n, double* mean, double* central, uint64_t* tickets, void* stream);
int fg_plane_timecorr(const fg_real* const* channels, const int64_t* batch_stride, int32_t K, int32_t batch, int32_t nz, int32_t ny,
                      int32_t nx, int32_t lags, int32_t n_slots, const int32_t* slot_lag, fg_real* base, double* base_ss, double* acc,
                      void* stream);
int fg_mb_cell_moments(const fg_real* velocity, const fg_real* pressure, int32_t dims, int32_t batch, int64_t n_cells,
                       const int64_t* block_table, int32_t n_blocks, int64_t samples, double* mean, double* central, void* stream);
int fg_mb_cell_moments_widths(const fg_real* velocity, const fg_real* pressure, int64_t n_cells, const int64_t* block_table,
                              int32_t n_blocks, const double* mean, const double* central, int32_t* widths);
int fg_plane_budgets(const fg_real* const* fields, const int64_t* batch_stride, int32_t n_fields, int32_t batch, int32_t nz, int32_t ny,
                     int32_t nx, const double* x, const double* y, const double* z, int32_t wrap_x, int32_t wrap_z, double* n,
                     double* mean, double* central, uint64_t* tickets, void* stream);
int fg_plane_spectra(const fg_real* const* channels, const int64_t* batch_stride, int32_t K, int32_t batch, int32_t nz, int32_t ny,
                     int32_t nx, const int32_t* planes, int32_t n_planes, double* amp, double* power, void* stream);
int fg_profile_enable(fg_handle h, int on);
int fg_profile_kinds(void);
const char* fg_profile_kind_name(int kind);
int fg_profile_read(fg_handle h, int kind, double* ms_sum, int64_t* samples, double* bytes_sum, double* flops_sum,
                    double* full_ms_sum, double* full_bytes_sum, int64_t* full_samples, int64_t* launches,
                    double* all_ms_sum, int64_t* all_samples);

int fg_sparse_apply_ell(const int32_t* idx, const float* w, int32_t rows, int32_t K, const float* x, int64_t n, int32_t m, float* y,
                        void* stream);
int fg_sparse_apply_csr(const int32_t* indptr, const int32_t* col, const float* val, int32_t rows, const float* x, int64_t n, int32_t m,
                        float* y, void* stream);
typedef struct fg_resampler_state* fg_resampler;
int fg_resampler_create(int dims, const int32_t* n_src, const int32_t* n_out, const int32_t* base_cat,
                        const float* frac_cat, int quirk3d, int device, fg_resampler* out);
int fg_resampler_destroy(fg_resampler r);
int fg_resample(fg_resampler r, const float* src, int batch, int channels, float* dst, int fill_max_steps,
                void* stream);

int fg_envglue_jet_schedule(const float* target, const float* current, const float* decay, const float* shape, int32_t n,
                            int32_t batch, int32_t nx, float* jets, float* last, void* stream);
int fg_envglue_channel_observe(const float* velocity, const float* pressure, const int64_t* sensor, int32_t n_sensors,
                               int32_t batch, int32_t ny, int32_t nx, float shear_scale, float penalty, float* obs_velocity,
                               float* obs_pressure, float* cross, float* shear, float* reward, void* stream);
int fg_envglue_channel_observe_batch(const float* velocity, const float* pressure, const int64_t* sensor, int32_t n_sensors,
                                     int32_t batch, int32_t ny, int32_t nx, const float* shear_scale_B, float penalty,
                                     float* obs_velocity, float* obs_pressure, float* cross, float* shear, float* reward,
                                     void* stream);

typedef struct fg_mb_state* fg_mb_handle;
int fg_mb_create(int32_t dims, int32_t batch, int32_t device, fg_mb_handle* out);
int fg_mb_destroy(fg_mb_handle h);
int fg_mb_add_block(fg_mb_handle h, const fg_real* vertex_coords_host, int32_t nx, int32_t ny, int32_t nz, int32_t* block_id);
int fg_mb_connect(fg_mb_handle h, int32_t block1, int32_t face1, int32_t block2, int32_t face2, int32_t axis1, int32_t axis2);
int fg_mb_make_periodic(fg_mb_handle h, int32_t block, int32_t axis);
int fg_mb_set_reference_quirks(fg_mb_handle h, int32_t connected_diagonal_offset, int32_t first_layer_rule);
int fg_mb_set_nonortho_flags(fg_mb_handle h, int32_t flags);
int fg_mb_finalize(fg_mb_handle h);
int fg_mb_sizes(fg_mb_handle h, int32_t* n_cells, int32_t* n_boundary_faces);
int fg_mb_block_info(fg_mb_handle h, int32_t block, int32_t* cell_offset, int32_t* boundary_slot0 );
// ... 100 lines not shown
```

### profiles/gen_switch_table.py

```python
import os
import re
import sys

ROOT = os.path.dirname(os.path.dirname(os.path.abspath(__file__)))

NOTES = {
    "FG_CG_FUSED": ("bits", "1 (default): three-launch preconditioned pressure CG on 2-D fast-transform grids (fg_fftcg.hip); 0: the five kernels"),
    "FG_BICG_PFUSED": ("bits", "1 (default): six-launch Helmholtz-preconditioned BiCGStab (fg_fftbicg.hip); 0: eleven launches per iteration"),
    "FG_BICG_FUSED": ("bits", "1 (default): two-kernel BiCGStab iteration in 2-D; 0: five kernels; 2: two kernels in 3-D bricks too"),
    "FG_BICG_SUB": ("no", "envs per sub-batch of the 2-D two-kernel BiCGStab (unset: by working set; 0: never)"),
    "FG_BICG3": ("bits", "z-marching 3-D BiCGStab: 0 never, N always with z-chunk N (tests), unset by the rule"),
    "FG_BICG3_BXL": ("no", "tile lanes along x of the z-marching BiCGStab (16 / 32)"),
    "FG_BICG3_MIX": ("bits", "debugging: bit 0 kernel a, bit 1 kernel b as z-march, bit 2 keep the init kernel"),
    "FG_REDUCE_WGS": ("no", "workgroups per env of the reduction kernels (0 = rule)"),
    "FG_HELM_ROWFORM": ("bits", "0: Helmholtz factors through k_helm_coeffs + the array-form line kernels (IEEE division instead of v_rcp)"),
    "FG_ADV_LINESWEEP": ("bits", "1: the advection-diffusion systems of the Helmholtz-preconditioned family (wall-refined 2-D grids: RBC) go to line sweeps x <- (D + O_y)^-1 (b - O_x x) first (k_line_sweep_y, fg_linepre.hip), BiCGStab takes what they do not settle; 0 (default): the preconditioned BiCGStab always -- measured on the RBC leg: 16-17 sweeps per velocity solve at the bench state's sub-step, 775 against 793 env-steps/s"),
    "FG_FD_FACFUSE": ("no", "1 (default): the first tridiagonal solve after 1/A changed makes the per-env row-mean factors itself (k_tridiag_y_lds<.., FAC>: same arithmetic, same bits); 0: k_fd_rowmean_factor as a launch of its own (A/B runs)"),
    "FG_FD_ROWMEAN": ("bits", "1 (default): the fused pressure CG is preconditioned by the row-mean operator (per-env factors, one factorisation per PISO step); 0: the grid's A = 1 factors"),
    "FG_ADV_JACOBI": ("bits", "velocity systems of uniform 2-D grids: 1 Jacobi sweeps first (fg_jacobi.hip), 0 BiCGStab always; unset = what fg_set_advection_jacobi says (the Simulation turns it on: policy advection_jacobi)"),
    "FLUIDGYM_AMD_ADVECTION_JACOBI": ("policy", "policy advection_jacobi (default 1): the Simulation asks for the Jacobi sweeps of fg_jacobi.hip on the grids that qualify"),
    "FLUIDGYM_AMD_PRESSURE_REFINEMENT": ("bits", "policy pressure_refinement (default 0 = off): up to N mixed-precision corrections behind every single-block pressure solve (fp64 residual, fp32 corrections: fg_set_pressure_refinement) -- an accuracy mode"),
    "FLUIDGYM_AMD_MULTI_STEP": ("no", "0: the sim steps of an env step are issued one by one from Python instead of through fg_multi_step (A/B runs; same bits)"),
    "FG_FCG_FIRST": ("bits", "1 (default): the fused CG judges its first iterate from I'(0)'s dot products (k_fcg_check0) and stores no pressure when every env ends there; 0: the verdict on the updated residual (A/B runs, tests)"),
    "FG_JAC_WARM": ("bits", "start vector of the Jacobi sweeps of a step's velocity systems: 1 the block velocity, 0 the BiCGStab start vector (zero on the non-orthogonal branch); unset: the block velocity on on-chip grids of 2^17 cells and more (where it saves a pass)"),
    "FG_JAC_PREFACTOR": ("no", "0: the row-mean factors of the pressure preconditioner are made in front of the first tridiagonal solve instead of behind the sweeps' check kernel (A/B runs)"),
    "FG_FCG_SPEC": ("no", "0: the corrector waits for the verdict on the first iterate instead of being launched behind the verdict kernel (A/B runs)"),
    "FG_JAC_SPEC": ("no", "0: k_h and the divergence kernel of the first corrector wait for the verdict on the velocity sweeps instead of being launched behind the check kernel (A/B runs)"),
    "FG_JAC_XCD": ("no", "0: the on-chip Jacobi regions in launch order instead of one XCD per run of an env's regions (A/B runs)"),
    "FG_JAC_SHAPE": ("bits", "A/B runs of the Jacobi sweeps: 1 full-row regions only, 2 bands only (unset: the cheaper of the two for the grid)"),
    "FG_JAC_SWEEPS": ("bits", "A/B runs: sweeps per pass of the Jacobi sweeps (unset: 4 / 6 / 8 for full rows, 8 / 12 for bands, by region depth)"),
    "FG_ROCTX": ("no", "1: named roctx ranges around the phases of a step (fg_single_step, scalar / velocity assembly and solve, pressure correctors; mb_velocity_solve, mb_pressure_solve) for rocprofv3 --marker-trace; the library is dlopen'ed, off by default"),
    "FG_HTRACE": ("no", "1: host time stamps around the polls and the launches behind them (fg_poll.hip), per-pair averages printed at exit"),
    "FG_FORCE_ZMARCH": ("bits", "z-march chunk length of the 3-D Poisson kernels (tests on small grids; -1 = brick kernels)"),
    "FG_ZMARCH_SB": ("no", "single-barrier ring of the z-march kernels: bit per mode, 0 never, unset = rule"),
    "FG_POLL_SPIN": ("no", "0: host polls wait with hipStreamSynchronize instead of spinning on pinned sequence words"),
    "FG_POLL_WORDS": ("no", "0: polled verdicts through the host-pinned mirror + a system-scope release (one L2 write-back per verdict kernel) instead of travelling in the 8-byte result words the host spins on (A/B runs: 8 790 against 9 600 env-steps/s on the headline, one lane)"),
    "FG_DEV_DT": ("no", "0: fg_single_step waits for the CFL maxima and computes the adaptive sub-steps on the host before the PISO step, instead of the CFL kernel's last workgroup taking them on the device (FgDtRule: same doubles, same bits) and the host reading the maxima after the step (A/B runs)"),
    "FLUIDGYM_AMD_F64_FD": ("bits", "0: the fp64 library solves the pressure systems with the reference's plain CG instead of the CG preconditioned by the fast-diagonalisation operator in doubles (csrc/fg_f64_fd.hip; A/B runs: iterations per solve)"),
    "FLUIDGYM_AMD_ENV_GLUE": ("bits", "0: ChannelJet2D's action schedule and reward / observation as elementwise torch launches instead of the two native kernels of fg_envglue.hip (A/B runs; the schedule is bit-identical, the means differ by fp32 rounding of the summation order)"),
    "FLUIDGYM_AMD_LANES": ("no", "default of ParallelFluidEnv(lanes=...): sub-batches of a rank's env batch, each its own solver handle, stepped concurrently by that many host threads on their own HIP streams (1 = one batch; bench.py passes --lanes 2).  Same bits per env as the sub-batches stepped alone"),
    "FG_PROF_PERIOD": ("no", "sampling period of the live kernel timing (64)"),
    "FG_FD_NO_FFT": ("bits", "1: the x basis change of the FD preconditioner as dense GEMM instead of the row FFT (tests)"),
    "FG_MB_BICG_VEC4": ("no", "bit per multi-block BiCGStab kernel: four-cell form (31 = all)"),
    "FG_MB_BICG_FUSE": ("bits", "multi-block BiCGStab: 0 five kernels, 1 s/t fused, 2 (default) also p/v"),
    "FG_MB_ML_FUSE": ("bits", "multilevel BiCGStab forms p / s inside the restriction: 0 never, 1 up to 32 systems, 2 always"),
    "FG_MB_ML_TRY_CAP": ("policy", "iteration cap of an attempt of the multilevel trial (200; tests force 2)"),
    "FG_MB_TRACE": ("no", "residual / verification trace of the pressure BiCGStab on stderr"),
    "FG_MB_TRACE_FAIL": ("no", "recurrence words of a system that ends non-finite"),
    "FG_MB_COMPACT": ("no", "0: every multi-block Krylov launch covers all systems of the batch"),
    "FG_MB_OC_RTG_NT": ("bits", "register-resident on-chip CG with a global residual copy on 16-24 k-cell meshes instead of k_mbc_l2"),
    "FG_MB_ONCHIP": ("bits", "0: no whole-solve on-chip CG (chunked CG kernels)"),
    "FG_MB_OC_AGG": ("bits", "0: cell-ordered on-chip CG instead of the aggregate-owned one"),
    "FG_MB_CLUSTER": ("bits", "pressure CG of an env by a cluster of four workgroups (fg_mb_cluster.hip): 0 never (the one-workgroup kernels), 1 (default) meshes beyond 8 k cells, 2 every mesh its tables fit (tests)"),
    "FG_MB_CL_JACOBI": ("bits", "0: the velocity sweeps of the meshes the cluster CG takes stay one launch per sweep (k_mbj_sweep_env) instead of one launch per solve by the clusters (k_mbj_cluster; A/B runs: 2 552 against 3 045 env-steps/s on the cylinder mesh)"),
    "FG_MB_CL_HALF": ("bits", "0: meshes whose rows of the coarse inverse do not fit LDS as fp32 stream them from L2 instead of holding them as fp16 (A/B runs: 19.7 against 16.8 us per iteration on 23 k cells)"),
    "FG_MB_CL_MAXCL": ("no", "cap on the clusters of one launch of the cluster CG (tests: envs beyond it queue inside the kernel; same bits)"),
    "FG_MB_CL_NEAR": ("no", "0: granule stores of the cluster CG always write through (sc1), also when a cluster's workgroups reported one XCD (A/B runs: 10.0 against 8.6 us per iteration)"),
    "FG_MB_OC_VARIANT": ("no", "on-chip CG variant bits (fences / coefficient layout)"),
    "FG_MB_RUNG_ILU": ("bits", "0: column-scaled preconditioned rung instead of ILU(0)"),
    "FLUIDGYM_AMD_LIB": ("no", "path of libfluidgym_hip.so (sanitizer build: tests/run_sanitizer_suite.sh)"),
    "FLUIDGYM_AMD_LIB_F64": ("no", "path of libfluidgym_hip_f64.so"),
    "FLUIDGYM_AMD_ADVECTION_FD_PRECONDITIONER": ("bits", "policy advection_fd_preconditioner: auto (2-D periodic-x grids) / always / never"),
    "FLUIDGYM_AMD_ADVECTION_LINE_PRECONDITIONER": ("bits", "policy advection_line_preconditioner (off)"),
    "FLUIDGYM_AMD_ADVECTION_RUNG_PRECONDITIONER": ("bits", "preconditioner of the BiCG_precondition_fallback rung: line / ilu"),
    "FLUIDGYM_AMD_ADVECTION_WARM_START": ("policy", "1: velocity solve starts from the current velocity in both branches (reference: branch rule)"),
    "FLUIDGYM_AMD_PRESSURE_WARM_START": ("policy", "1: pressure solves start from the previous pressure (reference: zero)"),
    "FLUIDGYM_AMD_PRESSURE_STALL_ACCEPT": ("policy", "accept a stalled pressure solve within a factor of the tolerance (off)"),
    "FLUIDGYM_AMD_PRESSURE_MULTILEVEL": ("bits", "multilevel preconditioner of the multi-block pressure CG"),
    "FLUIDGYM_AMD_PRESSURE_MULTILEVEL_BICGSTAB": ("bits", "multilevel trial of the airfoil's refined BiCGStab"),
    "FLUIDGYM_AMD_PRESSURE_MULTILEVEL_FP64": ("bits", "policy pressure_multilevel_fp64 (default 0): float64 cylinder / airfoil envs on 2-D meshes install the multilevel preconditioner in the fp64 build (kernel-form preconditioned CG, unfused BiCGStab trial) instead of the plain recurrences"),
    "FG_MB_PCG_KERNEL": ("bits", "1 (fp32 build, debugging): the multilevel-preconditioned pressure CG as the kernel-form loop of mb_cg (five launches per iteration, `k_mbc_ap<.., MBC_PRE>` / `k_mbc_update<.., true>`: what the fp64 build runs) instead of the on-chip / cluster kernels; 0 (default)"),
    "FLUIDGYM_AMD_PRESSURE_BICGSTAB_LARGE_MESHES": ("bits", "3-D multi-block ids take the refined BiCGStab"),
    "FLUIDGYM_AMD_NATIVE_WALL_FORCING": ("bits", "policy native_wall_forcing: the TCF forcing hook runs inside the library"),
    "FLUIDGYM_COLLECTIVE_TIMEOUT_S": ("no", "timeout of ParallelFluidEnv's process group (600 s)"),
    "FLUIDGYM_FORCE_COLLECTIVES": ("no", "ParallelFluidEnv issues its collectives at world size 1 too (tests)"),
    "FLUIDGYM_MASTER_PORT": ("no", "rendezvous port of the reference-style ParallelFluidEnv(cuda_ids=...) entry"),
    "FLUIDGYM_DATA_PATH": ("no", "local data path (initial domains), as config.update('local_data_path', ...)"),
}
IGNORE = {"RANK", "WORLD_SIZE", "LOCAL_RANK", "MASTER_ADDR", "MASTER_PORT", "HSA_ENABLE_IPC_MODE_LEGACY", "PYTHONPATH", "OMP_NUM_THREADS",
          "OPENBLAS_NUM_THREADS", "MKL_NUM_THREADS", "TMPDIR", "GRAFT_REPO_ROOT"}


def scan():
    found = {}
    for base, _, files in os.walk(os.path.join(ROOT, "fluidgym_amd")):
        if "_san" in base or "_f64" in base or "_var" in base or "__pycache__" in base:
            continue
        for fn in files:
            if not fn.endswith((".hip", ".h", ".py")):
                continue
            path = os.path.join(base, fn)
            rel = os.path.relpath(path, ROOT)
            for no, line in enumerate(open(path, errors="replace"), 1):
                for m in re.finditer(r'getenv\("([A-Z][A-Z0-9_]+)"\)', line):
                    found.setdefault(m.group(1), []).append(f"{rel}:{no}")
                for m in re.finditer(r'environ(?:\.get)?[\[(]\s*"([A-Z][A-Z0-9_]+)"', line):
                    found.setdefault(m.group(1), []).append(f"{rel}:{no}")
    return {k: v for k, v in found.items() if k not in IGNORE}


def render(found):
    lines = ["# Environment switches of fluidgym_amd", "",
             "Generated by `python profiles/gen_switch_table.py` from the `getenv` / `os.environ` sites of the source; `tests/test_switch_table.py`",
             "fails when this file is stale.  The native library reads its variables ONCE, at `fg_create` / `fg_mb_create` (never on a step",
             "path); `fg_config_dump` / `fg_mb_config_dump` report the values a handle runs under and `bench.py` stores them with every leg",
             "(`profiles/bench_detail.json`).  None is needed in normal operation.", "",
             "*results*: **no** = timing / diagnosis only; **bits** = the same converged answer through another kernel form (rounding and",
             "iteration trajectories differ); **policy** = a documented departure from (or return to) the reference's solver policy.", "",
             "| variable | results | read at | what |", "|---|---|---|---|"]
# ... 31 lines not shown
```

Before: 10570 env-steps/s.

## Keep lazy first-iterate envs unstored when pressure CG has stragglers

When the fast-diagonalisation CG's first-iterate poll finds only some envs converged, the envs that stopped at the first iterate now stay in lazy form. Their pressure is not written during the update and is materialised only when needed. The corrector reruns with those envs masked out, and a second speculative corrector launch is issued behind the iteration-1 verdict kernel. The poll schedule now uses a four-solve history to decide whether to poll the first iterate. This adds extra kernel paths, a materialise pass on failure or reset, and more state bookkeeping.

```diff
diff --git a/fluidgym_amd/_lib.py b/fluidgym_amd/_lib.py
--- a/fluidgym_amd/_lib.py
+++ b/fluidgym_amd/_lib.py
@@ -185,6 +185,7 @@
     "fg_make_divergence_free": (c_int, [c_void_p, c_float, c_int, POINTER(FgSolveInfo), c_void_p]),
     "fg_reset_solver_state": (c_int, [c_void_p, c_void_p]),
     "fg_solver_hints": (c_int, [c_void_p, POINTER(c_int32), c_int32]),
+    "fg_debug_cg_poll_rule": (c_int, [POINTER(c_int32), c_int, POINTER(c_int32)]),
     "fg_env_restore_field": (c_int, [c_void_p, c_int, c_void_p, c_int32, POINTER(FgEnvSel), c_int32, c_int32, c_void_p]),
     "fg_env_reset_solver_state": (c_int, [c_void_p, POINTER(FgEnvSel), c_int32, c_void_p]),
     "fg_mb_env_restore_field": (c_int, [c_void_p, c_int, c_void_p, c_int32, POINTER(FgEnvSel), c_int32, c_int32, c_void_p]),
diff --git a/fluidgym_amd/csrc/fg_api.hip b/fluidgym_amd/csrc/fg_api.hip
--- a/fluidgym_amd/csrc/fg_api.hip
+++ b/fluidgym_amd/csrc/fg_api.hip
@@ -8,6 +8,7 @@
 #include <stdlib.h>
 
 #include "fg_internal.h"
+#include "fg_fftcg.h"
 
 static thread_local std::string g_last_error;
 void fg_set_error(const std::string& msg) { g_last_error = msg; }
@@ -112,7 +113,7 @@
     FG_HIP_CHECK(hipMemset(s->t_rem_dev, 0, sizeof(double) * g.B));
 #endif
     if (int rc = fg_poll_create(&s->poll, (int)(nsys > 2 * (size_t)g.B ? nsys : 2 * (size_t)g.B))) return rc;
-    for (int k = 0; k < 4; ++k) { s->pred_bicg[k] = 2; s->pred_cg[k] = 1; }
+    for (int k = 0; k < 4; ++k) { s->pred_bicg[k] = 2; s->pred_cg[k] = 1; s->cg_hist_n[k] = 0; }
     s->wall_forcing_axis = -1;
     s->ref64_inner = 1e-4f;
     s->cg_wgs_per_slot = 256;
@@ -146,6 +147,7 @@
     { const char* e = getenv("FG_FCG_FIRST"); s->fcg_first = (e && atoi(e) == 0) ? 0 : 1; }
     { const char* e = getenv("FG_JAC_SPEC"); s->jac_spec = (e && atoi(e) == 0) ? 0 : 1; }
     { const char* e = getenv("FG_FCG_SPEC"); s->fcg_spec = (e && atoi(e) == 0) ? 0 : 1; }
+    { const char* e = getenv("FG_FCG_TRIM"); s->fcg_trim = (e && atoi(e) == 0) ? 0 : 1; }
     { const char* e = getenv("FG_JAC_PREFACTOR"); s->jac_prefactor = (e && atoi(e) == 0) ? 0 : 1; }
     { const char* e = getenv("FG_JAC_WARM"); s->jac_warm = e ? (atoi(e) != 0 ? 1 : 0) : -1; }
     s->cg_return_best = 1;
@@ -579,7 +581,7 @@
     if (last && !mean_folded)
         if (int rc = fg_launch_mean_sub(s, dt, s->p_result, s->pressure, st)) return rc;
     const FgMeanRef mean = {s->fcg_xsum, s->info_dev, s->pressure, o.marks_valid ? s->fcg_lazy : nullptr, s->fcg_alpha};
-    const FgLazyRef lazy = {s->fcg_lazy, s->fcg_alpha, last ? s->p_result : nullptr};
+    const FgLazyRef lazy = {s->fcg_lazy, s->fcg_alpha, last ? s->p_result : nullptr, o.lazy_mixed ? s->p_result : nullptr, o.skip_lazy ? 1 : 0};
     const fg_real* p = o.lazy_z ? o.lazy_z : ((last && !mean_folded) ? s->pressure : s->p_result);
     return fg_launch_correct(s, dt, s->rA, s->hvec, p, s->vel_result, st, last ? s->velocity : nullptr, mean_folded ? &mean : nullptr, o.lazy_z ? &lazy : nullptr);
 }
@@ -618,6 +620,9 @@
             fg_solve_info* info = info_host;
             if (!info) { tmp.assign(s->info_pinned, s->info_pinned + s->grid.B); info = tmp.data(); }
             s->rung_count[2] += 1;
+            if (out->lazy_mixed) {
+                if (int rc2 = fg_fcg_materialise(s, out->lazy_z, a.x, st)) return rc2;
+            }
             rc = fg_rung64_cg(s, a, info, (s->ladder_force & 2) != 0, st, out);
         }
 #endif
@@ -777,8 +782,10 @@
                                          info.data(), st, false, c == 0 ? 0 : 1, &outcome, FgCgSpec{spec_correct, &spec_ctx})))
             return rc;
         if (c < 2) { stats[2 + c] = max_iters(info.data(), B); s->ctr.add(2 + c, info.data(), B); }
-        if (!outcome.spec_done)
+        if (!outcome.spec_done) {
+            if (outcome.skip_lazy) s->fcg_masked_reruns += 1;
             if (int rc = launch_corrector(s, dt_B, outcome, last, st)) return rc;
+        }
     }
     if (opt->corrector_steps <= 0)
         if (int rc = fg_launch_copy_active(s, dt_B, s->vel_result, s->velocity, d, st)) return rc;
@@ -795,11 +802,13 @@
         "\"FG_BICG3_BXL\": %d, \"FG_BICG3_MIX\": %d, \"FG_REDUCE_WGS\": %d, \"FG_CG_WGS_PER_SLOT\": %d, \"FG_TRIDIAG_CB\": %d, \"FG_HELM_CB\": %d, "
         "\"FG_HELM_ROWFORM\": %d, \"FG_FD_ROWMEAN\": %d, \"FG_POLL_SPIN\": %d, \"FG_PROF_PERIOD\": %d, \"fast_transform_x\": %d, \"fd_preconditioner\": %d, "
         "\"helmholtz\": %d, \"advection_preconditioner\": %d, \"advection_from_result\": %d, \"return_best\": %d, \"cg_reset_steps\": %d, "
-        "\"double_fallback\": %d, \"wall_forcing_axis\": %d, \"FG_ADV_JACOBI\": %d, \"FG_FCG_FIRST\": %d, \"FG_JAC_WARM\": %d, \"first_iterate_polls\": %ld, \"unstored_pressure_solves\": %ld, \"FG_JAC_SPEC\": %d, \"FG_FCG_SPEC\": %d, \"jacobi_speculation_misses\": %ld, \"jacobi_floor_released\": %ld, \"pressure_refinement_corrections\": %ld}",
+        "\"double_fallback\": %d, \"wall_forcing_axis\": %d, \"FG_ADV_JACOBI\": %d, \"FG_FCG_FIRST\": %d, \"FG_JAC_WARM\": %d, \"first_iterate_polls\": %ld, \"unstored_pressure_solves\": %ld, \"FG_JAC_SPEC\": %d, \"FG_FCG_SPEC\": %d, \"jacobi_speculation_misses\": %ld, \"jacobi_floor_released\": %ld, \"pressure_refinement_corrections\": %ld, "
+        "\"FG_FCG_TRIM\": %d, \"mixed_pressure_solves\": %ld, \"masked_corrector_reruns\": %ld, \"second_verdict_speculations\": %ld}",
         FG_F64 ? "f64" : "f32", s->cg_fused, s->bicg_pfused, s->bicg_fused, s->bicg_sub, s->bicg3_force, s->bicg3_bxl, s->bicg3_mix, s->reduce_wgs,
         s->cg_wgs_per_slot, s->tridiag_cb, s->helm_cb_pref, s->helm_rowform_off ? 0 : 1, s->fd_rowmean, s->poll.spin, s->prof.period, s->fd_dct_x, s->fd_Qx ? 1 : 0,
         s->fd_lam ? 1 : 0, s->adv_precond, s->adv_from_result, s->cg_return_best, s->cg_reset_steps, s->double_fallback, s->wall_forcing_axis, s->adv_jacobi, s->fcg_first, s->jac_warm,
-        s->fcg_first_polls, s->fcg_unstored, s->jac_spec, s->fcg_spec, s->jac_spec_missed, s->jac_floor_released, s->ref64_corrections);
+        s->fcg_first_polls, s->fcg_unstored, s->jac_spec, s->fcg_spec, s->jac_spec_missed, s->jac_floor_released, s->ref64_corrections,
+        s->fcg_trim, s->fcg_mixed, s->fcg_masked_reruns, s->fcg_spec2);
     if (len >= n) return len + 1;
     memcpy(buf, tmp, (size_t)len + 1);
     return FG_OK;
@@ -977,6 +986,7 @@
 extern "C" int fg_reset_solver_state(fg_handle s, void* stream) {
     FG_REQUIRE(s && s->velocity, FG_ERR_NOT_BOUND, "velocity not bound");
     for (int k = 0; k < 4; ++k) s->jac_hist[k] = FgJacHist{0, 0, 0};
+    for (int k = 0; k < 4; ++k) s->cg_hist_n[k] = 0;
     FG_HIP_CHECK(hipMemsetAsync(s->p_result, 0, sizeof(fg_real) * (size_t)s->grid.B * s->grid.n, (hipStream_t)stream));
     return fg_launch_copy_active(s, nullptr, s->velocity, s->vel_result, s->grid.dims, (hipStream_t)stream);
 }
diff --git a/fluidgym_amd/csrc/fg_fftcg.h b/fluidgym_amd/csrc/fg_fftcg.h
--- a/fluidgym_amd/csrc/fg_fftcg.h
+++ b/fluidgym_amd/csrc/fg_fftcg.h
@@ -17,7 +17,9 @@
     int ns, rows, it, first; long env_stride;
     const float* r0; int x_zero;
     const int32_t* lazy;
+    int lazy_mode;
 };
+enum { FCG_LAZY_WRITE = 0, FCG_LAZY_KEEP = 1, FCG_LAZY_ONLY = 2 };
 struct FcgInvArgs {
     const float* u; const float* r; const float* rA; float* z; float* w;
     const float2* tw; const float2* rot; float is0, is;
@@ -37,7 +39,9 @@
 #if !FG_F64
 int fg_fcg_div_fwd(fg_state* s, const FgBounds& bnd, const fg_real* dt, const fg_real* hvec, fg_real* div, int ns, hipStream_t st);
 bool fg_fcg_ok(const fg_state* s);
-int fg_fcg_update_fwd(fg_state* s, const FcgVectors& v, int it, int first, int ns, hipStream_t st, bool marks_valid, const fg_real* r0 = nullptr);
+int fg_fcg_update_fwd(fg_state* s, const FcgVectors& v, int it, int first, int ns, hipStream_t st, bool marks_valid, const fg_real* r0 = nullptr,
+                      int lazy_mode = FCG_LAZY_WRITE);
+int fg_fcg_materialise(fg_state* s, const fg_real* z, fg_real* x, hipStream_t st);
 int fg_fcg_inv_apply(fg_state* s, const FcgVectors& v, const fg_real* rA, int it, int ns, hipStream_t st, int extras = 0);
 int fg_fcg_check0(fg_state* s, fg_real tol, int ns, hipStream_t st, FgPollOut poll, bool* marks_valid);
 #endif
diff --git a/fluidgym_amd/csrc/fg_fftcg.hip b/fluidgym_amd/csrc/fg_fftcg.hip
--- a/fluidgym_amd/csrc/fg_fftcg.hip
+++ b/fluidgym_amd/csrc/fg_fftcg.hip
@@ -16,8 +16,9 @@
     __shared__ float red[8];
     const int b = blockIdx.y;
     const int lane = threadIdx.x & 63, wave = threadIdx.x >> 6;
-    if (a.flags[b] != 0) {
+    if (a.flags[b] != 0 || a.lazy_mode == FCG_LAZY_ONLY) {
         if (a.lazy && a.lazy[b] == 1) {
+            if (a.lazy_mode == FCG_LAZY_KEEP) return;
             const float alpha = (float)a.alpha[b * 2];
             const int row0 = 2 * (blockIdx.x * 4 + wave);
 #pragma unroll
@@ -37,7 +38,7 @@
                 for (int e = 0; e < EPL; ++e) xv[e] += alpha * zv[e];
                 fgfft::store_row<N>(a.x + o, lane, xv);
             }
-        } else if (a.x_zero && (a.flags[b] == 1 || a.flags[b] == 2)) {
+        } else if (a.lazy_mode != FCG_LAZY_ONLY && a.x_zero && (a.flags[b] == 1 || a.flags[b] == 2)) {
             float z0[EPL];
 #pragma unroll
             for (int e = 0; e < EPL; ++e) z0[e] = 0.f;
@@ -433,11 +434,12 @@
            s->fcg_alpha != nullptr;
 }
 
-int fg_fcg_update_fwd(fg_state* s, const FcgVectors& v, int it, int first, int ns, hipStream_t st, bool marks_valid, const fg_real* r0) {
+int fg_fcg_update_fwd(fg_state* s, const FcgVectors& v, int it, int first, int ns, hipStream_t st, bool marks_valid, const fg_real* r0, int lazy_mode) {
     const FgGrid& G = s->grid;
     FcgUpdArgs a = {};
     a.r0 = r0; a.x_zero = r0 ? 1 : 0;
     a.lazy = (it == 0 && marks_valid) ? s->fcg_lazy : nullptr;
+    a.lazy_mode = a.lazy ? lazy_mode : FCG_LAZY_WRITE;
     a.z = v.z; a.w = v.w; a.p = v.p; a.s = v.s; a.x = v.x; a.r = v.r; a.t1 = v.t1;
     a.tw = s->fd_dct_tw; a.rot = s->fd_dct_rot; a.fs0 = s->fd_dct_fwd[0]; a.fs = s->fd_dct_fwd[1];
     a.flags = s->flags; a.acc = s->cg_acc; a.alpha = s->fcg_alpha; a.xsum = s->fcg_xsum; a.best = s->cg_best;
@@ -445,6 +447,18 @@
     const dim3 grid((G.ny + 7) / 8, G.B);
     const int slot = fg_prof_slot(s, FG_PK_FCG_UPD, s->flags, G.B, (first ? (r0 ? 24.0 : 28.0) : 44.0) * G.n, (10.0 + 5.0 * log2((double)G.nx)) * G.n, st);
     if (int rc = (s->fd_dct_x == 2 ? launch_upd<true>(s, slot, G.nx, a, grid, st) : launch_upd<false>(s, slot, G.nx, a, grid, st))) return rc;
+    FG_HIP_CHECK(hipGetLastError());
+    return FG_OK;
+}
+
+int fg_fcg_materialise(fg_state* s, const fg_real* z, fg_real* x, hipStream_t st) {
+    const FgGrid& G = s->grid;
+    FcgUpdArgs a = {};
+    a.z = z; a.x = x; a.x_zero = 1;
+    a.lazy = s->fcg_lazy; a.lazy_mode = FCG_LAZY_ONLY;
+    a.flags = s->flags; a.alpha = s->fcg_alpha; a.rows = G.ny; a.env_stride = G.n;
+    const dim3 grid((G.ny + 7) / 8, G.B);
+    if (int rc = (s->fd_dct_x == 2 ? launch_upd<true>(s, -1, G.nx, a, grid, st) : launch_upd<false>(s, -1, G.nx, a, grid, st))) return rc;
     FG_HIP_CHECK(hipGetLastError());
     return FG_OK;
 }
diff --git a/fluidgym_amd/csrc/fg_internal.h b/fluidgym_amd/csrc/fg_internal.h
--- a/fluidgym_amd/csrc/fg_internal.h
+++ b/fluidgym_amd/csrc/fg_internal.h
@@ -639,6 +639,8 @@
     int cg_fused, bicg_pfused; double* fcg_alpha; FgDacc* fcg_xsum;
     int32_t* fcg_lazy; int fcg_first;
     int fcg_spec;
+    int fcg_trim;
+    long fcg_mixed, fcg_masked_reruns, fcg_spec2;
     int jac_spec; long jac_spec_missed;
     long jac_floor_released = 0;
     int jac_prefactor;
@@ -667,6 +669,7 @@
     double* t_rem_dev;
     int dev_dt;
     int pred_bicg[4], pred_cg[4];
+    int cg_hist[4][4], cg_hist_n[4];
     int adv_jacobi, adv_jacobi_env; FgJacHist jac_hist[4]; float* jac_prev;
     int adv_linesweep;
     long long jac_solves, jac_fallbacks;
@@ -762,7 +765,7 @@
                   bool cg_from_zero = false,
                   bool fused_fwd = false);
 struct FgMeanRef { const FgDacc* sums; const fg_solve_info* info; fg_real* p_copy; const int32_t* lazy; const double* alpha; };
-struct FgLazyRef { const int32_t* lazy; const double* alpha; fg_real* p_res; };
+struct FgLazyRef { const int32_t* lazy; const double* alpha; fg_real* p_res; const fg_real* stored; int skip; };
 int fg_launch_correct(const fg_state* s, const fg_real* dt, const fg_real* rA, const fg_real* hvec, const fg_real* p,
                       fg_real* vel_out, hipStream_t st, fg_real* vel_copy = nullptr, const FgMeanRef* mean = nullptr, const FgLazyRef* lazy = nullptr);
 struct FgDtRule { double* t_rem; fg_real* dt_out; float cfl; double time_step; int reset; };
@@ -787,9 +790,11 @@
                            hipStream_t st);
 struct FgCgOutcome {
     const fg_real* lazy_z = nullptr;
+    bool lazy_mixed = false;
     bool mean_ready = false;
     bool marks_valid = false;
     bool spec_done = false;
+    bool skip_lazy = false;
 };
 struct FgCgSpec { int (*fn)(void* ctx, const FgCgOutcome& o) = nullptr; void* ctx = nullptr; };
 struct FgCgArgs {
@@ -804,6 +809,7 @@
     FgCgSpec spec;
 };
 int fg_cg_solve(fg_state* s, const FgCgArgs& a, fg_solve_info* info_host, hipStream_t st, FgCgOutcome* out = nullptr);
+bool fg_cg_poll_first(const int32_t* used, int n);
 
 struct FgSpecHook { int (*fn)(void* ctx) = nullptr; void* ctx = nullptr; };
 struct FgBicgArgs {
diff --git a/fluidgym_amd/csrc/fg_piso.hip b/fluidgym_amd/csrc/fg_piso.hip
--- a/fluidgym_amd/csrc/fg_piso.hip
+++ b/fluidgym_amd/csrc/fg_piso.hip
@@ -299,12 +299,14 @@
                                                        fg_real* __restrict__ vel_copy, FgMeanRef mean, FgLazyRef lazy, int tiles_x, int tiles_y, int tiles) {
     const FgCtx<DIMS, VEC> c = fg_make_ctx<DIMS, VEC>(g, tiles_x, tiles_y, tiles);
     if ((dt && !(dt[c.b] > 0.f)) || !c.valid) return;
+    const bool on = lazy.lazy && lazy.lazy[c.b] == 1;
+    if (on && lazy.skip) return;
+    const bool from_stored = lazy.lazy && !on && lazy.stored;
     const size_t N = g.n;
     const FgMetric<DIMS, VEC> m = fg_metrics<DIMS, VEC>(g, c);
     const FgVec<VEC> rA = fg_load<VEC>(rA_ + (size_t)c.b * N + c.idx);
-    FgNbr<DIMS, VEC> P = fg_gather<DIMS, VEC>(p + (size_t)c.b * N, c);
-    if (lazy.lazy) {
-        const bool on = lazy.lazy[c.b] == 1;
+    FgNbr<DIMS, VEC> P = fg_gather<DIMS, VEC>((from_stored ? lazy.stored : p) + (size_t)c.b * N, c);
+    if (lazy.lazy && !from_stored) {
         const fg_real sc = on ? (fg_real)lazy.alpha[2 * c.b] : (fg_real)0;
         auto scale = [&](FgVec<VEC>& v) {
 #pragma unroll
@@ -949,7 +951,7 @@
                       fg_real* vel_out, hipStream_t st, fg_real* vel_copy, const FgMeanRef* mean, const FgLazyRef* lazy) {
     fg_htrace("correct_in");
     const FgMeanRef mr = mean ? *mean : FgMeanRef{nullptr, nullptr, nullptr, nullptr, nullptr};
-    const FgLazyRef lz = lazy ? *lazy : FgLazyRef{nullptr, nullptr, nullptr};
+    const FgLazyRef lz = lazy ? *lazy : FgLazyRef{nullptr, nullptr, nullptr, nullptr, 0};
     const double cb = (s->grid.dims == 3 ? 36.0 : 28.0) + (vel_copy ? 4.0 * s->grid.dims : 0.0) + ((mean && mean->sums) || (lazy && lazy->p_res) ? 4.0 : 0.0);
     const int slot_c = fg_prof_slot(s, FG_PK_CORRECT, nullptr, s->grid.B, cb * (double)s->grid.n, 5.0 * s->grid.dims * (double)s->grid.n, st);
     FG_DISPATCH(s, {
diff --git a/fluidgym_amd/csrc/fg_poisson.hip b/fluidgym_amd/csrc/fg_poisson.hip
--- a/fluidgym_amd/csrc/fg_poisson.hip
+++ b/fluidgym_amd/csrc/fg_poisson.hip
@@ -386,7 +386,26 @@
     bool start_ready = false;
     bool start_fwd = false;
     bool done = false, info_fresh = false;
+    bool trim = false, spec0 = false, spec2 = false;
 };
+}
+
+bool fg_cg_poll_first(const int32_t* used, int n) {
+    if (n < 4) return true;
+    for (int i = n - 4; i < n; ++i)
+        if (used[i] < 1) return true;
+    return false;
+}
+
+extern "C" int fg_debug_cg_poll_rule(const int32_t* used_history, int n, int32_t* polls_out) {
+    FG_REQUIRE(n >= 0 && (n == 0 || (used_history && polls_out)), FG_ERR_INVALID_ARG, "fg_debug_cg_poll_rule: bad argument");
+    int32_t last[4]; int have = 0;
+    for (int i = 0; i < n; ++i) {
+        polls_out[i] = fg_cg_poll_first(last, have) ? 1 : 0;
+        if (have == 4) { for (int k = 0; k < 3; ++k) last[k] = last[k + 1]; have = 3; }
+        last[have++] = used_history[i];
+    }
+    return FG_OK;
 }
 
 static int cg_begin(fg_state* s, const FgCgArgs& a, CgRun& c, hipStream_t st) {
@@ -423,6 +442,7 @@
         if (int rc = fg_fd_apply(s, a.r, c.zvec, s->cg_acc + (size_t)(c.nb + 0) * FG_CG_SLOTS, FG_CG_NAMES * FG_CG_SLOTS, ns, B, st, &c.judge)) return rc;
     }
     c.next_poll = a.precond ? (s->pred_cg[a.kind & 3] + 1 > 1 ? s->pred_cg[a.kind & 3] + 1 : 1) : c.check_every;
+    if (a.precond && s->fcg_trim) c.next_poll = fg_cg_poll_first(s->cg_hist[a.kind & 3], s->cg_hist_n[a.kind & 3]) ? 1 : (c.next_poll > 2 ? c.next_poll : 2);
     c.mean_sums = (!a.use_x0 && a.x == s->p_result && s->fcg_xsum) ? s->fcg_xsum : nullptr;
     return FG_OK;
 }
@@ -460,7 +480,8 @@
         if (poll0) fg_prof_prefetch(s, st);
         if (int rc = fg_fcg_check0(s, a.tol, ns, st, po, &o.marks_valid)) return rc;
         bool spec = false;
-        if (poll0 && s->fcg_spec && a.spec.fn && a.lazy_ok && r0 && c.mean_sums) {
+        const bool unstored_ok = a.lazy_ok && r0 && c.mean_sums;
+        if (poll0 && s->fcg_spec && a.spec.fn && unstored_ok) {
             FgCgOutcome ahead;
             ahead.lazy_z = v.z; ahead.mean_ready = true; ahead.marks_valid = true;
             if (int rc = a.spec.fn(a.spec.ctx, ahead)) return rc;
@@ -472,13 +493,16 @@
             fg_htrace("cg_poll_done");
             c.info_fresh = true;
             s->fcg_first_polls += 1;
-            bool all = true, all_ok = true;
+            bool all = true, all_ok = true, any_bad = false;
+            int n_lazy = 0;
             for (int b = 0; b < B; ++b) {
                 all = all && (s->info_pinned[b].converged || !s->info_pinned[b].is_finite);
                 all_ok = all_ok && s->info_pinned[b].converged && s->info_pinned[b].is_finite;
+                any_bad = any_bad || !s->info_pinned[b].is_finite;
+                n_lazy += (s->info_pinned[b].converged && s->info_pinned[b].is_finite && s->info_pinned[b].used_iterations == 0) ? 1 : 0;
             }
             if (all) {
-                if (a.lazy_ok && r0 && all_ok && c.mean_sums) {
+                if (unstored_ok && all_ok) {
                     o.lazy_z = v.z; s->fcg_unstored += 1; o.spec_done = spec;
                 } else {
                     if (int rc = fg_fcg_update_fwd(s, v, 0, 1, ns, st, o.marks_valid, r0)) return rc;
@@ -486,13 +510,22 @@
                 c.done = true;
             } else {
                 c.next_poll = 2;
+                if (s->fcg_trim && unstored_ok && !any_bad) {
+                    c.trim = true; c.spec0 = spec;
+                    if (n_lazy > 0) s->fcg_mixed += 1;
+                }
             }
         }
     }
+    auto materialise = [&]() -> int {
+        if (!c.trim) return FG_OK;
+        c.trim = false; c.spec0 = false;
+        return fg_fcg_materialise(s, c.zvec, a.x, st);
+    };
     int first = 1;
     const int fused_reset = (a.reset_steps > 0 && a.reset_steps < 10) ? a.reset_steps : 10;
     for (int it = 0; it < a.max_iterations && !c.done; ++it) {
-        if (int rc = fg_fcg_update_fwd(s, v, it, first, ns, st, o.marks_valid, it == 0 ? r0 : nullptr)) return rc;
+        if (int rc = fg_fcg_update_fwd(s, v, it, first, ns, st, o.marks_valid, it == 0 ? r0 : nullptr, c.trim ? FCG_LAZY_KEEP : FCG_LAZY_WRITE)) return rc;
         if (first) {
             fg_real* t = v.p; v.p = v.z; v.z = t;
             t = v.s; v.s = v.w; v.w = t;
@@ -507,16 +540,26 @@
             hipLaunchKernelGGL(k_cg_check, dim3((B + CG_CHECK_WAVES - 1) / CG_CHECK_WAVES), dim3(64 * CG_CHECK_WAVES), 0, st, s->cg_acc, s->flags, s->info_dev, s->info_pinned, a.tol, it,
                                n, B, final_pass, ns, po);
             fg_htrace("cg_check_launched");
+            bool spec2 = false;
+            if (c.trim && it == 1 && s->fcg_spec && a.spec.fn) {
+                FgCgOutcome ahead;
+                ahead.lazy_z = c.zvec; ahead.lazy_mixed = true; ahead.skip_lazy = c.spec0; ahead.mean_ready = true; ahead.marks_valid = true;
+                if (int rc = a.spec.fn(a.spec.ctx, ahead)) return rc;
+                s->fcg_spec2 += 1;
+                spec2 = true;
+            }
             if (int rc = fg_poll_wait_infos(&s->poll, po, 0, B, s->info_pinned, st)) return rc;
             fg_htrace("cg_poll_done");
             c.info_fresh = true;
             c.done = true;
             for (int b = 0; b < B; ++b) c.done = c.done && (s->info_pinned[b].converged || !s->info_pinned[b].is_finite);
+            c.spec2 = spec2 && c.done;
             if (c.done) break;
         }
         if (it + 1 < a.max_iterations) {
             judge.it = it;
             if ((it + 2) % fused_reset == 0) {
+                if (int rc = materialise()) return rc;
                 hipLaunchKernelGGL(k_zero_name, dim3(B), dim3(64), 0, st, s->cg_acc, (it + 1) % 3, B);
                 FG_DISPATCH(s, {
                     const FgLaunch L = fg_launch_geometry<DIMS, VEC>(s->grid);
@@ -532,6 +575,7 @@
         }
     }
     o.mean_ready = !a.use_x0;
+    if (c.trim) { o.lazy_z = c.zvec; o.lazy_mixed = true; o.skip_lazy = c.spec0; o.spec_done = c.spec2; }
     return FG_OK;
 }
 #endif
@@ -615,6 +659,12 @@
     if (int prc = fg_prof_collect(s, st)) return prc;
     bool failed = false;
     for (int b = 0; b < B; ++b) failed = failed || !s->info_pinned[b].converged;
+#if !FG_F64
+    if (failed && o.lazy_mixed) {
+        if (int rc = fg_fcg_materialise(s, o.lazy_z, a.x, st)) return rc;
+        o.lazy_z = nullptr; o.lazy_mixed = false; o.skip_lazy = false; o.spec_done = false;
+    }
+#endif
     if (failed) {
         o.mean_ready = false;
         hipLaunchKernelGGL(k_cg_restore_best, dim3(32, B), dim3(FG_BLOCK), 0, st, a.x, s->info_dev, s->info_pinned, s->cg_best, n);
@@ -625,6 +675,9 @@
         int used_max = 0;
         for (int b = 0; b < B; ++b) used_max = s->info_pinned[b].used_iterations > used_max ? s->info_pinned[b].used_iterations : used_max;
         s->pred_cg[a.kind & 3] = used_max;
+        int* H = s->cg_hist[a.kind & 3]; int& hn = s->cg_hist_n[a.kind & 3];
+        if (hn == 4) { for (int k = 0; k < 3; ++k) H[k] = H[k + 1]; hn = 3; }
+        H[hn++] = used_max;
     }
     for (int b = 0; b < B; ++b) {
         if (info_host) info_host[b] = s->info_pinned[b];
diff --git a/include/fluidgym_hip.h b/include/fluidgym_hip.h
--- a/include/fluidgym_hip.h
+++ b/include/fluidgym_hip.h
@@ -199,6 +199,7 @@
 };
 int fg_reset_solver_state(fg_handle h, void* stream);
 int fg_solver_hints(fg_handle h, int32_t* hints12, int32_t set);
+int fg_debug_cg_poll_rule(const int32_t* used_history, int n, int32_t* polls_out);
 
 typedef struct fg_env_sel {
     int32_t env, src;
diff --git a/profiles/gen_switch_table.py b/profiles/gen_switch_table.py
--- a/profiles/gen_switch_table.py
+++ b/profiles/gen_switch_table.py
@@ -25,6 +25,7 @@
     "FG_JAC_WARM": ("bits", "start vector of the Jacobi sweeps of a step's velocity systems: 1 the block velocity, 0 the BiCGStab start vector (zero on the non-orthogonal branch); unset: the block velocity on on-chip grids of 2^17 cells and more (where it saves a pass)"),
     "FG_JAC_PREFACTOR": ("no", "0: the row-mean factors of the pressure preconditioner are made in front of the first tridiagonal solve instead of behind the sweeps' check kernel (A/B runs)"),
     "FG_FCG_SPEC": ("no", "0: the corrector waits for the verdict on the first iterate instead of being launched behind the verdict kernel (A/B runs)"),
+    "FG_FCG_TRIM": ("no", "0: the round-6 schedule of a pressure solve with stragglers -- the first iterate is polled only after a solve that ended there, every env is stored when the solve goes on and the whole corrector runs again (A/B runs)"),
     "FG_JAC_SPEC": ("no", "0: k_h and the divergence kernel of the first corrector wait for the verdict on the velocity sweeps instead of being launched behind the check kernel (A/B runs)"),
     "FG_JAC_XCD": ("no", "0: the on-chip Jacobi regions in launch order instead of one XCD per run of an env's regions (A/B runs)"),
     "FG_JAC_SHAPE": ("bits", "A/B runs of the Jacobi sweeps: 1 full-row regions only, 2 bands only (unset: the cheaper of the two for the grid)"),
```

Result: slower. 10380 env-steps/s (-1.9%).
